# BlaineHeffron/WaveformML

Measured on AMD Instinct MI355X. Metric: waveforms/sec (LitPSD sparse-conv training step), higher is better.
Workload: dtype bf16; 1 GPU; SubMConv3d PSD net, 14x11 PMT grid x 256 samples, Cin=2 Cout=32, 256 events/rank/step, rulebook rebuilt every step; active_voxels_per_rank=84164, global_batch=256, parallelism=dp1, execution=hipgraph

## Files before the change

include/wfsparse.h:

```cpp
#ifndef WFSPARSE_H
#define WFSPARSE_H

#include <stddef.h>
#include <stdint.h>

#ifdef __cplusplus
extern "C" {
#endif

#define WFS_OK 0
#define WFS_EINVAL 1
#define WFS_EOVERFLOW 2
#define WFS_EHIP 3
#define WFS_EWORKSPACE 4

#define WFS_F32 0
#define WFS_BF16 1
#define WFS_F16 2

#define WFS_MAX_DIM 4

#define WFS_ABI_VERSION 6
int wfs_abi_version(void);
const char *wfs_last_error(void);
// ... 250 lines not shown
                   const float *momentum, const float *eps, const float *dropout_p, const int64_t *seed_dev,
                   int32_t training, float *saved, void *Y, int32_t dtype, void *stream);
int wfs_conv2d_bwd(const void *X, const void *dY, int64_t B, int32_t H, int32_t W, int32_t c0, const int32_t *channels,
                   const int32_t *fs, const int32_t *st, const int32_t *pd, const int32_t *dil, int32_t layers,
                   const void *param_ptrs, const float *dropout_p, const int64_t *seed_dev, int32_t training,
                   const float *saved, void *dX, float *workspace, int32_t dtype, void *stream);
int wfs_densify_rows(const void *rows, const int32_t *coords, int64_t n_cap, int32_t C, int64_t B, int32_t H, int32_t W,
                     const int64_t *n_valid_dev, void *out, int32_t dtype, void *stream);

#define WFS_RNN_MAX_INPUT 32
#define WFS_RNN_MAX_HIDDEN 32
#define WFS_RNN_MAX_LAYERS 8
#define WFS_RNN_MAX_T 4096
#define WFS_RNN_RELU 0
#define WFS_RNN_TANH 1
int wfs_rnn_ok(int32_t I, int32_t H, int32_t layers, int32_t dirs, int32_t nonlinearity, int32_t T, int32_t dtype);
int wfs_rnn_n_params(int32_t layers, int32_t dirs);
size_t wfs_rnn_saved_floats(int64_t N, int32_t T, int32_t I, int32_t H, int32_t layers, int32_t dirs);
size_t wfs_rnn_bwd_workspace_floats(int64_t N, int32_t T, int32_t I, int32_t H, int32_t layers, int32_t dirs);
int wfs_rnn_fwd(const void *X, int64_t N, int32_t T, int32_t I, int32_t H, int32_t layers, int32_t dirs,
                int32_t nonlinearity, const void *param_ptrs, float *saved, void *Y, void *hidden, int32_t dtype,
                float dropout_p, const int64_t *seed_dev, void *stream);
int wfs_rnn_bwd(const void *dY, int64_t N, int32_t T, int32_t I, int32_t H, int32_t layers, int32_t dirs,
                int32_t nonlinearity, const void *param_ptrs, const float *saved, void *dX, float *workspace,
                int32_t dtype, float dropout_p, const int64_t *seed_dev, void *stream);

#define WFS_VOXELIZE_MAX_SAMPLES 4096
size_t wfs_voxelize_offsets_ints(int64_t n_cap, int32_t T);
int wfs_voxelize_plan(const void *rows, const int32_t *coords, int64_t n_cap, int32_t T, const int64_t *n_dev,
                      float threshold, int32_t batch_size, int64_t V_cap, int32_t *row_offsets, int64_t *v_dev,
                      int32_t *event_offsets, int32_t *overflow_dev, int32_t dtype, void *stream);
int wfs_voxelize_emit(const void *rows, const void *values, const int32_t *coords, int64_t n_cap, int32_t T,
                      float threshold, const int32_t *row_offsets, int64_t V_cap, int32_t *indices, void *feats,
                      int32_t dtype, void *stream);
int wfs_voxelize_bwd(const void *dfeat, const int32_t *indices, const int32_t *row_offsets, int64_t n_cap, int32_t T,
                     int64_t V_cap, void *dY, int32_t dtype, void *stream);

int wfs_xent_mean_fwd_bwd(const float *logits, const int64_t *target, int64_t B, int32_t C,
                          int64_t ignore_index, float *loss, float *dlogits, void *stream);

int wfs_sgd_step(float *param, const float *grad, float *momentum_buf, int64_t n, const float *lr_dev,
                 float momentum, float dampening, float weight_decay, int32_t nesterov, int32_t first_step,
                 void *stream);

#define WFS_ADAM_COEF_FLOATS 16
int wfs_adam_step(float *param, const float *grad, float *exp_avg, float *exp_avg_sq, float *max_exp_avg_sq,
                  int64_t n, const double *hyper_dev, float *step_dev, float *coef_dev, int32_t amsgrad,
                  int32_t maximize, int32_t decoupled, void *stream);

int wfs_load_batch(const int32_t *coords, int64_t n, int32_t cols, const int32_t *perm_host, int32_t *coords_dst,
                   int32_t *indices_dst, const void *feats, void *feats_dst, int64_t feat_bytes,
                   const int64_t *labels, int64_t *labels_dst, int64_t B, int64_t *n_valid_dst,
                   int32_t *event_offsets, int32_t events, void *stream);

#define WFS_EVAL_MAX_SAMPLES 512
size_t wfs_eval_table_ints(int32_t n_bins, int32_t n_mult, int32_t n_confusion, int32_t n_se_max, int32_t nx,
                           int32_t ny, int32_t n_classes);
int wfs_event_pulse_stats(const int32_t *coords, const void *rows, int64_t n_cap, int32_t T, int32_t dtype,
                          const int64_t *n_dev, int32_t E, const double *gains, const float *seg_status, int32_t nx,
                          int32_t ny, int32_t fix_last_n_se, int32_t *offsets, double *rowstats, double *avg_coo,
                          float *summed, float *stats, int32_t *multiplicity, int32_t *n_se, float *psdl, float *psdr,
                          float *energy, float *features, int32_t *flags, void *stream);
int wfs_eval_accumulate(int32_t E, int32_t T, int32_t n_classes, const double *avg_coo, const float *summed,
                        const int32_t *multiplicity, const int32_t *n_se, const float *psdl, const float *psdr,
                        const float *energy, const int64_t *predictions, const int64_t *labels, int32_t n_bins,
                        int32_t n_mult, int32_t n_confusion, int32_t n_se_max, int32_t nx, int32_t ny, double emin,
                        double emax, double psd_min, double psd_max, int64_t *tables, double *sum_wf,
                        double *sum_labelled, int32_t *flags, void *stream);

size_t wfs_phys_table_ints(int32_t n_bins, int32_t n_mult, int32_t n_confusion, int32_t nx, int32_t ny,
                           int32_t n_classes);
size_t wfs_phys_spectra_ints(int32_t n_classes, const int32_t *spec_bins);
int wfs_phys_event_stats(const int32_t *coords, const void *rows, int64_t n_cap, int32_t dtype, const int64_t *n_dev,
                         int32_t E, int32_t *offsets, double *avg_coo, float *features, int32_t *multiplicity,
                         int32_t *flags, void *stream);
int wfs_phys_accumulate(int32_t E, int32_t n_classes, const double *avg_coo, const float *features,
                        const int32_t *multiplicity, const int64_t *predictions, const int64_t *labels, int32_t n_bins,
                        int32_t n_mult, int32_t n_confusion, int32_t nx, int32_t ny, double emin, double emax,
                        double psd_min, double psd_max, int64_t *tables, const double *spec_ranges,
                        const int32_t *spec_bins, int64_t *spectra, int32_t *flags, void *stream);

#define WFS_SEG_FIXED_ONE 4294967296.0
size_t wfs_seg_z_table_ints(int32_t nx, int32_t ny, int32_t nmult, int32_t nz, int32_t n_err, int32_t n_sample);
size_t wfs_seg_energy_table_ints(int32_t nx, int32_t ny, int32_t nmult, int32_t nE);
int wfs_seg_z_accumulate(const int32_t *coords, int64_t n_cap, const int64_t *n_dev, int32_t B, const void *pred,
                         int32_t pred_dtype, int64_t pred_bs, int64_t pred_ps, int32_t pred_plane, const void *targ,
                         int32_t targ_dtype, int64_t targ_bs, int64_t targ_ps, int32_t targ_plane, const void *energy,
                         int32_t e_dtype, int64_t e_bs, int64_t e_ps, int32_t e_plane, const float *seg_status,
                         int32_t nx, int32_t ny, const int32_t *sample_segs, int32_t n_sample, int32_t nmult,
                         int32_t nz, double zrange, int32_t n_err, double err_low, double err_high, double E_low,
                         double E_high, double E_scale, int32_t *offsets, int64_t *tables, int32_t *flags,
                         void *stream);
int wfs_seg_energy_accumulate(const int32_t *coords, int64_t n_cap, const int64_t *n_dev, int32_t B, const void *pred,
                              int32_t pred_dtype, int64_t pred_bs, int64_t pred_ps, int32_t pred_plane,
                              const void *targ, int32_t targ_dtype, int64_t targ_bs, int64_t targ_ps,
                              int32_t targ_plane, const float *seg_status, int32_t nx, int32_t ny, int32_t nmult,
                              int32_t nE, double E_low, double E_high, double E_scale, int32_t *offsets,
                              int64_t *tables, int32_t *flags, void *stream);

#define WFS_METRIC_PAIRS_MAX 16
#define WFS_PID_CLASSES 5
size_t wfs_metric_pairs_table_ints(int32_t P, const int32_t *nbins, int32_t n_classes);
int wfs_metric_pairs_accumulate(const float *params, const int32_t *result, const int32_t *category, int64_t M,
                                const int64_t *n_dev, int32_t P, const double *lo, const double *hi,
                                const int32_t *nbins, int32_t n_classes, int64_t *tables, int32_t *flags, void *stream);
int wfs_match_categories(const int64_t *predictions, const int64_t *labels, int64_t M, int32_t *result,
// ... 133 lines not shown
```

waveformml_amd/_lib.py:

```python
import ctypes
import os

import torch

_HERE = os.path.dirname(os.path.abspath(__file__))
LIB_PATH = os.environ.get("WFS_LIB") or os.path.join(_HERE, "lib", "libwfsparse.so")

WFS_OK, WFS_EINVAL, WFS_EOVERFLOW, WFS_EHIP, WFS_EWORKSPACE = 0, 1, 2, 3, 4
WFS_F32, WFS_BF16, WFS_F16 = 0, 1, 2
WFS_TENSOR_TARGET_I64 = 3
WFS_MAX_DIM = 4
WFS_RNN_RELU, WFS_RNN_TANH = 0, 1
WFS_LOSS_L1, WFS_LOSS_MSE = 0, 1
WFS_PREDICT_ROWS_PER_BLOCK = 256
WFS_PREDICT_WAVEFORM, WFS_PREDICT_PULSE = 0, 1
WFS_PREDICT_DENSE, WFS_PREDICT_EVENT, WFS_PREDICT_ROWS = 0, 1, 2
WFS_ABI_VERSION = 6
TIMER_GATHER_CONV, TIMER_GATHER_DW, TIMER_RULEBOOK, TIMER_CONV_BACKWARD = 0, 1, 2, 3

c_i32p = ctypes.POINTER(ctypes.c_int32)
c_i64p = ctypes.POINTER(ctypes.c_int64)
c_f32p = ctypes.POINTER(ctypes.c_float)
_vp, _i32, _i64, _sz = ctypes.c_void_p, ctypes.c_int32, ctypes.c_int64, ctypes.c_size_t
_dbl = ctypes.c_double


class Geometry(ctypes.Structure):
    _fields_ = [("ndim", _i32), ("batch_size", _i32), ("subm", _i32), ("K", _i32),
                ("spatial", _i32 * WFS_MAX_DIM), ("out_shape", _i32 * WFS_MAX_DIM),
                ("ksize", _i32 * WFS_MAX_DIM), ("stride", _i32 * WFS_MAX_DIM),
                ("padding", _i32 * WFS_MAX_DIM), ("dilation", _i32 * WFS_MAX_DIM),
                ("transposed", _i32), ("output_padding", _i32 * WFS_MAX_DIM)]


class DwJob(ctypes.Structure):
    _fields_ = [("part", _vp), ("nslabs", _i64), ("per", _i64), ("K", _i32), ("A", _i32), ("B", _i32),
                ("transpose", _i32), ("dW", _vp)]


SIGNATURES = {
    "wfs_abi_version": (ctypes.c_int, []),
    "wfs_last_error": (ctypes.c_char_p, []),
    "wfs_geometry_init": (ctypes.c_int, [ctypes.POINTER(Geometry)]),
    "wfs_rulebook_workspace_bytes": (_sz, [ctypes.POINTER(Geometry), _i64]),
    "wfs_rulebook_plan": (ctypes.c_int, [ctypes.POINTER(Geometry), _vp, _i64, _vp, _vp, _sz, c_i64p, _vp, _vp, _i64,
                                         _vp]),
    "wfs_rulebook_emit": (ctypes.c_int, [ctypes.POINTER(Geometry), _vp, _i64, _i64, _vp, _vp, _vp, _vp, _vp,
                                         _vp, _sz, _vp, _vp, _vp]),
    "wfs_indices_check": (ctypes.c_int, [ctypes.POINTER(Geometry), _vp, _i64, _vp, _sz, c_i64p, _vp]),
    "wfs_gather_conv": (ctypes.c_int, [_vp, c_i32p, _i32, _i32, _i64, _vp, _i64, _i32, _vp, _i32, _i32, _i32,
                                       _vp, _vp, _i32, _vp, _i32, _vp]),
    "wfs_gather_packed_ok": (ctypes.c_int, [_i32, _i32, _i32, _i32, _i32, _i32]),
    "wfs_unpack_table": (ctypes.c_int, [_vp, _i32, _i32, _i64, _vp, _vp, _vp]),
    "wfs_event_rulebook_conv_ok": (ctypes.c_int, [ctypes.POINTER(Geometry)]),
    "wfs_event_rulebook_conv_packed_kl": (ctypes.c_int, [ctypes.POINTER(Geometry)]),
    "wfs_event_rulebook_conv_state_bytes": (_sz, [_i32]),
    "wfs_event_rulebook_conv": (ctypes.c_int, [ctypes.POINTER(Geometry), _vp, _i64, _vp, _vp, _i64, _vp, _vp, _vp, _vp,
                                               _i32, _vp, _vp, _vp, _vp, _vp, _vp]),
    "wfs_wide_conv_ok": (ctypes.c_int, [_i32, _i64, _i64, _i32, _i32, _i32]),
    "wfs_wide_enable": (ctypes.c_int, [_i32]),
    "wfs_wide_conv_workspace_bytes": (_sz, [_i32, _i64, _i64, _i32, _i32, _i32, _i32]),
    "wfs_wide_filters_bytes": (_sz, [_i32, _i32, _i32, _i32]),
    "wfs_wide_filters": (ctypes.c_int, [_vp, _i32, _i32, _i32, _i32, _vp, _vp]),
    "wfs_wide_gather_conv": (ctypes.c_int, [_vp, c_i32p, _i32, _i32, _i64, _vp, _i64, _i32, _vp, _vp, _i32, _i32, _i32,
                                            _vp, _vp, _i32, _vp, _vp, _sz, _vp]),
    "wfs_wide_linear_ok": (ctypes.c_int, [_i64, _i32, _i32, _i32]),
    "wfs_wide_linear_workspace_bytes": (_sz, [_i64, _i32, _i32, _i32]),
    "wfs_wide_linear_fwd": (ctypes.c_int, [_vp, _i64, _i32, _vp, _vp, _i32, _vp, _i32, _vp, _sz, _vp]),
    "wfs_wide_linear_bwd": (ctypes.c_int, [_vp, _vp, _i64, _i32, _vp, _i32, _vp, _vp, _vp, _i32, _vp, _sz, _vp]),
    "wfs_event_offsets_ints": (_sz, [_i32]),
    "wfs_event_offsets": (ctypes.c_int, [_vp, _i64, _i32, _i32, _vp, _vp, _vp]),
    "wfs_event_rulebook_ok": (ctypes.c_int, [ctypes.POINTER(Geometry)]),
    "wfs_event_rulebook_flag_ints": (_sz, [_i32]),
    "wfs_event_rulebook_subm": (ctypes.c_int, [ctypes.POINTER(Geometry), _vp, _i64, _vp, _vp, _vp, _vp, _vp, _vp]),
    "wfs_gather_dw_workspace_bytes": (_sz, [_i32, _i64, _i32, _i32]),
    "wfs_gather_dw": (ctypes.c_int, [_vp, c_i32p, _i32, _i32, _i64, _vp, _i32, _vp, _i64, _i32, _i32, _vp, _i32, _vp,
                                     _sz, _vp, ctypes.POINTER(DwJob), _i32, _vp]),
    "wfs_conv_backward": (ctypes.c_int, [_vp, _i32, _i32, _i64, _vp, _vp, _i64, _i32, _i32, _vp, _vp, _vp, _i32, _vp, _sz,
                                         _vp, ctypes.POINTER(DwJob), _i32, _vp]),
    "wfs_dw_reduce_jobs": (ctypes.c_int, [ctypes.POINTER(DwJob), _i32, _vp]),
    "wfs_first_conv_bn_backward_workspace_bytes": (_sz, [_i32, _i64]),
    "wfs_first_conv_bn_backward": (ctypes.c_int, [_vp, c_i32p, _i32, _i32, _i64, _vp, _vp, _vp, _i64, _vp, _vp, _vp, _vp,
                                                  _i32, _vp, _vp, _vp, _i32, _vp, _sz, _vp, ctypes.POINTER(DwJob), _vp]),
    "wfs_scatter_conv": (ctypes.c_int, [_vp, _i32, _i32, _i64, _vp, _i32, _vp, _i32, _i32, _i32, _vp, _i32, _vp]),
    "wfs_maxpool_fwd": (ctypes.c_int, [_vp, c_i32p, _i32, _i64, _vp, _i64, _i32, _vp, _i32, _vp, _vp]),
    "wfs_maxpool_packed_ok": (ctypes.c_int, [_i32, _i32, _i32, _i32]),
    "wfs_maxpool_bwd": (ctypes.c_int, [_vp, _i32, _i32, _i64, _vp, _vp, _vp, _i64, _i32, _vp, _i32, _vp, _vp]),
    "wfs_bn_workspace_bytes": (_sz, [_i64, _i32]),
    "wfs_column_sum_workspace_bytes": (_sz, [_i32]),
    "wfs_column_sum": (ctypes.c_int, [_vp, _i64, _i32, _vp, _vp, _sz, _i32, _vp, _vp]),
    "wfs_bn_relu_fwd": (ctypes.c_int, [_vp, _i64, _i32, _vp, _vp, _vp, _vp, _vp, ctypes.c_float, ctypes.c_float, _i32,
# ... 18 lines not shown
    "wfs_head_bwd": (ctypes.c_int, [_vp, _vp, _i64, _i64, _vp, _i32, _vp, _vp, _vp, _i32, _vp, _sz, ctypes.POINTER(DwJob),
                                    _vp]),
    "wfs_tcn_lds_bytes": (_sz, [_i32, _i32, _i32]),
    "wfs_tcn_taps_fwd": (ctypes.c_int, [_vp, _i32, _i32, _vp, _vp, _vp]),
    "wfs_tcn_taps_bwd": (ctypes.c_int, [_vp, _i32, _i32, _vp, _i64, _vp]),
    "wfs_tcn_fwd": (ctypes.c_int, [_vp, _i64, _i32, _vp, _vp, _i32, _i32, _vp, _i32, ctypes.c_float, _vp, _vp]),
    "wfs_tcn_bwd": (ctypes.c_int, [_vp, _vp, _i64, _i32, _vp, _vp, _i32, _i32, _vp, _vp, _i32, ctypes.c_float, _vp,
                                    _vp]),
    "wfs_tcnc_ok": (ctypes.c_int, [_i32, c_i32p, _i32, _i32, _i32, _i32]),
    "wfs_tcnc_n_conv": (ctypes.c_int, [_i32, c_i32p, _i32, _i32]),
    "wfs_tcnc_weights_floats": (_sz, [_i32, c_i32p, _i32, _i32]),
    "wfs_tcnc_saved_floats": (_sz, [_i64, _i32, _i32, c_i32p, _i32]),
    "wfs_tcnc_bwd_workspace_floats": (_sz, [_i64, _i32, _i32, c_i32p, _i32, _i32]),
    "wfs_tcnc_taps_fwd": (ctypes.c_int, [_vp, _i32, c_i32p, _i32, _i32, _vp, _vp]),
    "wfs_tcnc_fwd": (ctypes.c_int, [_vp, _i64, _i32, _i32, c_i32p, _i32, _i32, _vp, _vp, _vp, _i32, ctypes.c_float, _vp,
                                    _vp]),
    "wfs_tcnc_bwd": (ctypes.c_int, [_vp, _vp, _i64, _i32, _i32, c_i32p, _i32, _i32, _vp, _vp, _vp, _vp, _vp, _i32,
                                    ctypes.c_float, _vp, _vp]),
    "wfs_conv1d_ok": (ctypes.c_int, [_i32, c_i32p, c_i32p, c_i32p, c_i32p, _i32, _i32, _i32]),
    "wfs_conv1d_saved_floats": (_sz, [_i64, _i32, _i32, c_i32p, c_i32p, c_i32p, c_i32p, _i32]),
    "wfs_conv1d_bwd_workspace_floats": (_sz, [_i64, _i32, _i32, c_i32p, c_i32p, c_i32p, c_i32p, _i32]),
    "wfs_conv1d_fwd": (ctypes.c_int, [_vp, _i64, _i32, _i32, c_i32p, c_i32p, c_i32p, c_i32p, _i32, _vp, c_f32p, c_f32p,
                                      _i32, _vp, _vp, _i32, _vp, _vp]),
    "wfs_conv1d_bwd": (ctypes.c_int, [_vp, _vp, _i64, _i32, _i32, c_i32p, c_i32p, c_i32p, c_i32p, _i32, _vp, _i32, _vp,
                                      _vp, _vp, _i32, _vp, _vp]),
    "wfs_conv2d_ok": (ctypes.c_int, [_i32, c_i32p, c_i32p, c_i32p, c_i32p, c_i32p, _i32, _i64, _i32, _i32, _i32, _i32]),
    "wfs_conv2d_saved_floats": (_sz, [_i64, _i32, _i32, _i32, c_i32p, c_i32p, c_i32p, c_i32p, c_i32p, _i32, _i32]),
    "wfs_conv2d_bwd_workspace_floats": (_sz, [_i64, _i32, _i32, _i32, c_i32p, c_i32p, c_i32p, c_i32p, c_i32p, _i32,
                                              _i32]),
    "wfs_conv2d_fwd": (ctypes.c_int, [_vp, _i64, _i32, _i32, _i32, c_i32p, c_i32p, c_i32p, c_i32p, c_i32p, _i32, _vp,
                                      c_f32p, c_f32p, c_f32p, _vp, _i32, _vp, _vp, _i32, _vp]),
    "wfs_conv2d_bwd": (ctypes.c_int, [_vp, _vp, _i64, _i32, _i32, _i32, c_i32p, c_i32p, c_i32p, c_i32p, c_i32p, _i32, _vp,
                                      c_f32p, _vp, _i32, _vp, _vp, _vp, _i32, _vp]),
    "wfs_densify_rows": (ctypes.c_int, [_vp, _vp, _i64, _i32, _i64, _i32, _i32, _vp, _vp, _i32, _vp]),
    "wfs_rnn_ok": (ctypes.c_int, [_i32, _i32, _i32, _i32, _i32, _i32, _i32]),
    "wfs_rnn_n_params": (ctypes.c_int, [_i32, _i32]),
    "wfs_rnn_saved_floats": (_sz, [_i64, _i32, _i32, _i32, _i32, _i32]),
    "wfs_rnn_bwd_workspace_floats": (_sz, [_i64, _i32, _i32, _i32, _i32, _i32]),
    "wfs_rnn_fwd": (ctypes.c_int, [_vp, _i64, _i32, _i32, _i32, _i32, _i32, _i32, _vp, _vp, _vp, _vp, _i32, ctypes.c_float,
                                   _vp, _vp]),
    "wfs_rnn_bwd": (ctypes.c_int, [_vp, _i64, _i32, _i32, _i32, _i32, _i32, _i32, _vp, _vp, _vp, _vp, _i32, ctypes.c_float,
                                   _vp, _vp]),
    "wfs_voxelize_offsets_ints": (_sz, [_i64, _i32]),
    "wfs_voxelize_plan": (ctypes.c_int, [_vp, _vp, _i64, _i32, _vp, ctypes.c_float, _i32, _i64, _vp, _vp, _vp, _vp, _i32,
                                         _vp]),
    "wfs_voxelize_emit": (ctypes.c_int, [_vp, _vp, _vp, _i64, _i32, ctypes.c_float, _vp, _i64, _vp, _vp, _i32, _vp]),
    "wfs_voxelize_bwd": (ctypes.c_int, [_vp, _vp, _vp, _i64, _i32, _i64, _vp, _i32, _vp]),
    "wfs_xent_mean_fwd_bwd": (ctypes.c_int, [_vp, _vp, _i64, _i32, _i64, _vp, _vp, _vp]),
    "wfs_sgd_step": (ctypes.c_int, [_vp, _vp, _vp, _i64, _vp, ctypes.c_float, ctypes.c_float, ctypes.c_float, _i32, _i32,
                                    _vp]),
    "wfs_adam_step": (ctypes.c_int, [_vp, _vp, _vp, _vp, _vp, _i64, _vp, _vp, _vp, _i32, _i32, _i32, _vp]),
    "wfs_load_batch": (ctypes.c_int, [_vp, _i64, _i32, c_i32p, _vp, _vp, _vp, _vp, _i64, _vp, _vp, _i64, _vp, _vp, _i32,
                                      _vp]),
    "wfs_eval_table_ints": (_sz, [_i32, _i32, _i32, _i32, _i32, _i32, _i32]),
    "wfs_event_pulse_stats": (ctypes.c_int, [_vp, _vp, _i64, _i32, _i32, _vp, _i32, _vp, _vp, _i32, _i32, _i32, _vp, _vp,
                                             _vp, _vp, _vp, _vp, _vp, _vp, _vp, _vp, _vp, _vp, _vp]),
    "wfs_eval_accumulate": (ctypes.c_int, [_i32, _i32, _i32, _vp, _vp, _vp, _vp, _vp, _vp, _vp, _vp, _vp, _i32, _i32,
                                           _i32, _i32, _i32, _i32, ctypes.c_double, ctypes.c_double, ctypes.c_double,
                                           ctypes.c_double, _vp, _vp, _vp, _vp, _vp]),
    "wfs_phys_table_ints": (_sz, [_i32, _i32, _i32, _i32, _i32, _i32]),
    "wfs_phys_spectra_ints": (_sz, [_i32, c_i32p]),
    "wfs_phys_event_stats": (ctypes.c_int, [_vp, _vp, _i64, _i32, _vp, _i32, _vp, _vp, _vp, _vp, _vp, _vp]),
    "wfs_phys_accumulate": (ctypes.c_int, [_i32, _i32, _vp, _vp, _vp, _vp, _vp, _i32, _i32, _i32, _i32, _i32, _dbl, _dbl,
                                           _dbl, _dbl, _vp, ctypes.POINTER(_dbl), c_i32p, _vp, _vp, _vp]),
    "wfs_seg_z_table_ints": (_sz, [_i32, _i32, _i32, _i32, _i32, _i32]),
    "wfs_seg_energy_table_ints": (_sz, [_i32, _i32, _i32, _i32]),
    "wfs_seg_z_accumulate": (ctypes.c_int, [_vp, _i64, _vp, _i32] + [_vp, _i32, _i64, _i64, _i32] * 3 +
                             [_vp, _i32, _i32, _vp, _i32, _i32, _i32, _dbl, _i32, _dbl, _dbl, _dbl, _dbl, _dbl, _vp, _vp,
                              _vp, _vp]),
    "wfs_seg_energy_accumulate": (ctypes.c_int, [_vp, _i64, _vp, _i32] + [_vp, _i32, _i64, _i64, _i32] * 2 +
                                  [_vp, _i32, _i32, _i32, _i32, _dbl, _dbl, _dbl, _vp, _vp, _vp, _vp]),
    "wfs_metric_pairs_table_ints": (_sz, [_i32, c_i32p, _i32]),
    "wfs_metric_pairs_accumulate": (ctypes.c_int, [_vp, _vp, _vp, _i64, _vp, _i32, ctypes.POINTER(_dbl),
                                                   ctypes.POINTER(_dbl), c_i32p, _i32, _vp, _vp, _vp]),
    "wfs_match_categories": (ctypes.c_int, [_vp, _vp, _i64, _vp, _vp, _vp]),
    "wfs_pid_table_ints": (_sz, [_i32, _i32]),
    "wfs_pid_row_stats": (ctypes.c_int, [_vp, _vp, _vp, _vp, _i32, _i32, _i64, _vp, _i32, _vp, _i32, _i32, _i32, _i32,
                                         _i32, _i32, _i32, _dbl] + [_vp] * 10),
    "wfs_metric_pairs_real_table_ints": (_sz, [_i32, c_i32p, _i32]),
    "wfs_metric_pairs_accumulate_real": (ctypes.c_int, [_vp, _vp, _vp, _i64, _vp, _i32, ctypes.POINTER(_dbl),
                                                        ctypes.POINTER(_dbl), c_i32p, _i32, _vp, _vp, _vp]),
    "wfs_tensor_rows": (ctypes.c_int, [_vp, _i32, _i32, _vp, _i32, _i32, _vp, _i64, _vp, _i32, _i32, _vp, _vp, _vp, _vp,
                                       _vp]),
    "wfs_masked_regression_loss_workspace_bytes": (_sz, [_i64]),
    "wfs_masked_regression_loss": (ctypes.c_int, [_vp, _i32, _vp, _i32, _i32, _i32, _vp, _vp, _i32, _i32, _i64, _vp, _i32,
                                                  _i32, _vp, _sz, _vp, _vp, _vp]),
    "wfs_masked_regression_loss_backward": (ctypes.c_int, [_vp, _i32, _vp, _i32, _i32, _i32, _vp, _vp, _i32, _i32, _i64,
                                                           _vp, _i32, _vp, _vp, _vp, _vp]),
    "wfs_error_edges": (ctypes.c_int, [_dbl, _i32, ctypes.POINTER(_dbl)]),
    "wfs_segq_row_stats": (ctypes.c_int, [_vp, _vp, _i32, _vp, _i32, _i32, _vp, _i32, _i64, _vp, _i32, _vp, _i32, _i32,
                                          _i32, _i32, _i32, _i32] + [_vp] * 11),
    "wfs_segq_error_accumulate": (ctypes.c_int, [_vp, _i32, _vp, _i32, _i32, _i32, _vp, _vp, _i64, _vp, _i32, _i32, _i32]
                                  + [_vp] * 7),
    "wfs_align_pulses": (ctypes.c_int, [_vp, _i32, _i64, _vp, _i32, _i32, _vp, _vp, _vp]),
    "wfs_zreal_row_stats": (ctypes.c_int, [_vp, _vp, _i32, _i64, _i64, _i32, _vp, _i32, _i64, _i64, _i32, _i32, _i32, _vp,
                                           _i32, _i64, _vp, _i32, _vp, _i32, _i32, _i32, _dbl] + [_vp] * 12),
    "wfs_zreal_baseline": (ctypes.c_int, [_vp, _i64, _vp, _i32, _vp, _vp, _vp, _i32, _i32, _vp, _vp]),
    "wfs_zreal_table_ints": (_sz, [_i32, _i32, _i32, _i32, _i32]),
    "wfs_zreal_accumulate": (ctypes.c_int, [_vp, _i64, _vp, _i32, _vp, _vp, _vp, _vp, _vp, _vp, _i32, _i32, _i32, _i32,
                                            _dbl, _dbl, _dbl, _i32, _vp, _vp, _vp]),
    "wfs_seg_z_accumulate_cal": (ctypes.c_int, [_vp, _i64, _vp, _i32] + [_vp, _i32, _i64, _i64, _i32] * 3 +
                                 [_vp, _vp, _i32, _vp, _vp, _i32, _i32, _vp, _i32, _i32, _i32, _dbl, _i32, _dbl, _dbl, _dbl, _dbl,
                                  _dbl, _vp, _vp, _vp, _vp]),
    "wfs_seg_energy_cal_table_ints": (_sz, [_i32, _i32, _i32, _i32, _i32]),
    "wfs_seg_energy_accumulate_cal": (ctypes.c_int, [_vp, _i64, _vp, _i32] + [_vp, _i32, _i64, _i64, _i32] * 2 +
                                      [_vp, _vp, _vp, _i32, _i32, _i32, _i32, _i32, _dbl, _dbl, _dbl, _dbl, _vp, _vp, _vp,
# ... 107 lines not shown
```

waveformml_amd/csrc/conv_mfma.hip:

```cpp
#include <stdlib.h>

#include "wfs_common.h"

namespace {

typedef float f32x16 __attribute__((ext_vector_type(16)));
typedef float f32x4 __attribute__((ext_vector_type(4)));
constexpr int F32_GROUP = 4;

struct KMap {
    int v[128];
};


__device__ __forceinline__ int packed_entry(int e, int o) { return (e >= 0 && (e & 7) == o) ? (e >> 3) : -1; }
__device__ __forceinline__ void table_row_of(int pk, int k, int *trow, int *osel) {
    const int kq = pk ? k / pk : k;
    *trow = kq;
    *osel = pk ? k - kq * pk : -1;
}
__device__ __forceinline__ int table_value(int e, int osel) { return osel < 0 ? e : packed_entry(e, osel); }

typedef __bf16 bf16x8e __attribute__((ext_vector_type(8)));
typedef float f32x2 __attribute__((ext_vector_type(2)));
// ... 286 lines not shown
                                                       const float *__restrict__ X, const float *__restrict__ W,
                                                       const float *__restrict__ bias, float *__restrict__ Y) {
    extern __shared__ __attribute__((aligned(16))) float sW_dyn[];
    __shared__ int sNext;
    gconv16_f32_body<TRANSPOSE_W, PK, true>(sW_dyn, &sNext, (int)blockIdx.x, (int)gridDim.x, (int)blockDim.x, table, mirror,
                                            K, identity_k, R, r_dev, X, W, bias, Y);
}

template <bool TRANSPOSE_W, int PK = 0>
__global__ void __launch_bounds__(1024) k_gconv16_f32(const int *__restrict__ table, int mirror, int K, int identity_k,
                                                      long long R, const long long *__restrict__ r_dev,
                                                      const float *__restrict__ X, const float *__restrict__ W,
                                                      const float *__restrict__ bias, float *__restrict__ Y) {
    extern __shared__ __attribute__((aligned(16))) float sW_dyn[];
    __shared__ int sNext;
    gconv16_f32_body<TRANSPOSE_W, PK>(sW_dyn, &sNext, (int)blockIdx.x, (int)gridDim.x, (int)blockDim.x, table, mirror, K,
                                      identity_k, R, r_dev, X, W, bias, Y);
}

typedef short s16x8 __attribute__((ext_vector_type(8)));
typedef __bf16 bf16x8 __attribute__((ext_vector_type(8)));
constexpr int BF_GROUP = 6;

typedef _Float16 f16x8 __attribute__((ext_vector_type(8)));

template <typename H, typename V>
__device__ __forceinline__ f32x16 mfma16(V a, V b, f32x16 acc) {
    static_assert(sizeof(V) == 16, "8 x 16-bit operands");
    if constexpr (sizeof(H) == 2 && __is_same(H, wfs_f16))
        return __builtin_amdgcn_mfma_f32_32x32x16_f16(__builtin_bit_cast(f16x8, a), __builtin_bit_cast(f16x8, b), acc, 0,
                                                      0, 0);
    else
        return __builtin_amdgcn_mfma_f32_32x32x16_bf16(__builtin_bit_cast(bf16x8, a), __builtin_bit_cast(bf16x8, b), acc,
                                                       0, 0, 0);
}

__device__ __forceinline__ uint4 keep_if(uint4 v, bool ok) {
    v.x = ok ? v.x : 0u;
    v.y = ok ? v.y : 0u;
    v.z = ok ? v.z : 0u;
    v.w = ok ? v.w : 0u;
    return v;
}

#ifndef WFS_KNOCK
#define WFS_KNOCK 0
#endif
template <typename H, bool TRANSPOSE_W, int PK = 0>
__device__ __forceinline__ void gconv32_bf16_body(unsigned char *smem, int vbid, int vgrid, int nthreads,
                                                  const int *__restrict__ table, int mirror, int K, int identity_k,
                                                  long long R, const long long *__restrict__ r_dev,
                                                  const H *__restrict__ X, const float *__restrict__ W,
                                                  const float *__restrict__ bias, H *__restrict__ Y, long long ntiles,
                                                  long long tiles_per_xcd) {
    uint4 *sWb = reinterpret_cast<uint4 *>(smem);
    int *sNb = reinterpret_cast<int *>(smem + (size_t)K * 2048);
    constexpr int WSB = 5;
    const int nfrag = K * 128;
    if (!(WFS_KNOCK & 1))
    for (int u0 = threadIdx.x; u0 < nfrag; u0 += nthreads * WSB) {
        float w[WSB][8];
#pragma unroll
        for (int b = 0; b < WSB; ++b) {
            int u = u0 + b * nthreads;
            u = u < nfrag ? u : nfrag - 1;
            int k = u >> 7, s = (u >> 6) & 1, h = (u >> 5) & 1, col = u & 31;
            int c0 = 16 * h + 8 * s;
            if (!TRANSPOSE_W) {
#pragma unroll
                for (int j = 0; j < 8; ++j) w[b][j] = W[((long long)k * 32 + c0 + j) * 32 + col];
            } else {
                const f32x4 *src = (const f32x4 *)(W + ((long long)k * 32 + col) * 32 + c0);
                f32x4 lo = src[0], hi = src[1];
                w[b][0] = lo.x; w[b][1] = lo.y; w[b][2] = lo.z; w[b][3] = lo.w;
                w[b][4] = hi.x; w[b][5] = hi.y; w[b][6] = hi.z; w[b][7] = hi.w;
            }
        }
#pragma unroll
        for (int b = 0; b < WSB; ++b) {
            int u = u0 + b * nthreads;
            uint4 v;
            v.x = wfs_pack2<H>(w[b][0], w[b][1]);
            v.y = wfs_pack2<H>(w[b][2], w[b][3]);
            v.z = wfs_pack2<H>(w[b][4], w[b][5]);
            v.w = wfs_pack2<H>(w[b][6], w[b][7]);
            if (u < nfrag) sWb[u] = v;
        }
    }
    __syncthreads();

    const int lane = threadIdx.x & 63, wid = threadIdx.x >> 6, nw = nthreads >> 6;
    const int r = lane & 31, h = lane >> 5;
    int *myNb = sNb + (size_t)wid * K * 32;
    const int xcd = vbid & 7, bi = vbid >> 3, bpx = vgrid >> 3;
    const long long Rv = wfs_valid_rows(R, r_dev);
    const long long nt_v = (Rv + 31) >> 5, tpx_v = (nt_v + 7) >> 3;
    (void)ntiles;
    (void)tiles_per_xcd;
    const long long t_begin = (long long)xcd * tpx_v;
    const long long t_end = t_begin + tpx_v < nt_v ? t_begin + tpx_v : nt_v;
    const float bj = bias ? bias[r] : 0.f;
    const __amdgpu_buffer_rsrc_t rsrcX = __builtin_amdgcn_make_buffer_rsrc((void *)X, 0, 0x7FFFFFFF, 0x00020000);
    for (long long tile = t_begin + (long long)wid * bpx + bi; tile < t_end; tile += (long long)bpx * nw) {
        if (tile * 32 >= Rv) break;
        const long long row = tile * 32 + r;
        const bool live = row < Rv;
        const long long rowc = live ? row : 0;
        int v[32];
        if constexpr (PK == 0) {
#pragma unroll
            for (int k = 0; k < 32; ++k) {
                int kk = k < K ? k : K - 1;
// ... 29 lines not shown
            int nbs[BF_GROUP];
#pragma unroll
            for (int g = 0; g < BF_GROUP; ++g) {
                ks[g] = mask ? __builtin_ctz(mask) : -1;
                mask = mask ? (mask & (mask - 1)) : 0u;
            }
#pragma unroll
            for (int g = 0; g < BF_GROUP; ++g)
                if (ks[g] >= 0) {
                    nbs[g] = myNb[ks[g] * 32 + r];
                    const int src = (WFS_KNOCK & 16) ? (int)rowc : nbs[g];
                    int voff = src >= 0 ? (int)((unsigned)src * 64u + (unsigned)h * 32u) : (int)0x80000000;
                    asm volatile("" : "+v"(voff));
                    if ((WFS_KNOCK & 32) && (ks[g] % 3) != 1) {
                        a_lo[g] = uint4{0x3f803f80u, 0x3f803f80u, 0x3f803f80u, 0x3f803f80u};
                        a_hi[g] = a_lo[g];
                    } else {
                        a_lo[g] = __builtin_bit_cast(uint4, __builtin_amdgcn_raw_buffer_load_b128(rsrcX, voff, 0, 0));
                        a_hi[g] = __builtin_bit_cast(uint4, __builtin_amdgcn_raw_buffer_load_b128(rsrcX, voff + 16, 0, 0));
                    }
                }
#pragma unroll
            for (int g = 0; g < BF_GROUP; ++g)
                if (ks[g] >= 0) {
                    const uint4 lo = a_lo[g], hi = a_hi[g];
                    const uint4 *bp = sWb + (size_t)ks[g] * 128 + h * 32 + r;
                    uint4 b0 = bp[0], b1 = bp[64];
                    acc = mfma16<H>(lo, b0, acc);
                    acc = mfma16<H>(hi, b1, acc);
                }
        }
        unsigned *Yw = reinterpret_cast<unsigned *>(Y);
#pragma unroll
        for (int i = 0; i < 16; i += 2) {
            float mine0 = acc[i], mine1 = acc[i + 1];
            float send = (lane & 1) ? mine0 : mine1;
            float got = __shfl_xor(send, 1, 64);
            unsigned packed = (lane & 1) ? wfs_pack2<H>(got, mine1) : wfs_pack2<H>(mine0, got);
            int ri = (lane & 1) ? i + 1 : i;
            long long orow = tile * 32 + (ri & 3) + 8 * (ri >> 2) + 4 * h;
            if (!(WFS_KNOCK & 8) || packed == 0x12345678u)
                if (orow < Rv) Yw[orow * 16 + (r >> 1)] = packed;
        }
    }
}

template <typename H, bool TRANSPOSE_W, int PK = 0>
__global__ void __launch_bounds__(1024) k_gconv32_bf16(const int *__restrict__ table, int mirror, int K,
                                                       int identity_k,
                                                       long long R, const long long *__restrict__ r_dev,
                                                       const H *__restrict__ X,
                                                       const float *__restrict__ W, const float *__restrict__ bias,
                                                       H *__restrict__ Y, long long ntiles,
                                                       long long tiles_per_xcd) {
    extern __shared__ __attribute__((aligned(16))) unsigned char smem[];
    gconv32_bf16_body<H, TRANSPOSE_W, PK>(smem, (int)blockIdx.x, (int)gridDim.x, (int)blockDim.x, table, mirror, K,
                                          identity_k, R, r_dev, X, W, bias, Y, ntiles, tiles_per_xcd);
}

template <typename T>
__global__ void __launch_bounds__(256) k_gconv_c2c32(const int *__restrict__ table, KMap kmap, int K, int identity_k,
                                                     long long R, const long long *__restrict__ r_dev,
                                                     const T *__restrict__ X,
                                                     const float *__restrict__ W, const float *__restrict__ bias,
                                                     T *__restrict__ Y) {
    __shared__ __attribute__((aligned(16))) float sW[128 * 64];
    for (int e = threadIdx.x; e < K * 64; e += 256) sW[e] = W[e];
    __syncthreads();
    const int rsub = threadIdx.x >> 3, cq = threadIdx.x & 7;
    f32x4 bv = {0.f, 0.f, 0.f, 0.f};
    if (bias) bv = *(const f32x4 *)(bias + cq * 4);
    const long long Rv = wfs_valid_rows(R, r_dev);
    for (long long row = (long long)blockIdx.x * 32 + rsub; row < Rv; row += (long long)gridDim.x * 32) {
        f32x4 acc = bv;
        for (int k = 0; k < K; ++k) {
            int nb = (k == identity_k) ? (int)row : table[(long long)kmap.v[k] * R + row];
            if (nb < 0) continue;
            float x0 = wfs_ld(X + (long long)nb * 2), x1 = wfs_ld(X + (long long)nb * 2 + 1);
            f32x4 w0 = *(const f32x4 *)(sW + k * 64 + cq * 4);
            f32x4 w1 = *(const f32x4 *)(sW + k * 64 + 32 + cq * 4);
            acc.x = fmaf(x0, w0.x, acc.x);
            acc.y = fmaf(x0, w0.y, acc.y);
            acc.z = fmaf(x0, w0.z, acc.z);
            acc.w = fmaf(x0, w0.w, acc.w);
            acc.x = fmaf(x1, w1.x, acc.x);
            acc.y = fmaf(x1, w1.y, acc.y);
            acc.z = fmaf(x1, w1.z, acc.z);
            acc.w = fmaf(x1, w1.w, acc.w);
        }
        T *y = Y + row * 32 + cq * 4;
        if constexpr (sizeof(T) == 4) {
            *reinterpret_cast<f32x4 *>(y) = acc;
        } else {
            uint2 pk;
            pk.x = wfs_pack2<T>(acc.x, acc.y);
            pk.y = wfs_pack2<T>(acc.z, acc.w);
            *reinterpret_cast<uint2 *>(y) = pk;
        }
    }
}

constexpr int DW_KG = 4;
constexpr int DW_WAVES = 8;

constexpr int DW_LDS = DW_WAVES * 1024 * 4;
template <typename T>
__device__ __forceinline__ void gdw32_body(float *sRed, int bx, int by, int nbx, const int *__restrict__ table, int pk, int K,
                                           int identity_k, long long Rcap, const long long *__restrict__ r_dev,
                                           const T *__restrict__ S, const T *__restrict__ G, float *__restrict__ part,
                                           int ngroups) {
// ... 459 lines not shown
#pragma unroll
    for (int q = 0; q < DWS_KG; ++q) {
        __syncthreads();
#pragma unroll
        for (int i = 0; i < 16; ++i) {
            int arow = (i & 3) + 8 * (i >> 2) + 4 * h;
            sRed[wid * 1024 + arow * 32 + c] = acc[q][i];
        }
        __syncthreads();
        const int k = g + q * ngroups;
        for (int e = threadIdx.x; e < 1024; e += DWS_WAVES * 64) {
            float v = 0.f;
#pragma unroll
            for (int w = 0; w < DWS_WAVES; ++w) v += sRed[w * 1024 + e];
            if (k < K) part[((long long)bx * K + k) * 1024 + e] = v;
        }
    }
}

__global__ void __launch_bounds__(DWS_WAVES * 64) k_gdw32_split(const int *__restrict__ table, int pk, int K, int identity_k,
                                                               long long Rcap, const long long *__restrict__ r_dev,
                                                               const float *__restrict__ S, const float *__restrict__ G,
                                                               float *__restrict__ part, int ngroups) {
    extern __shared__ __attribute__((aligned(16))) unsigned char smem[];
    gdw32_split_body(smem, (int)blockIdx.x, (int)blockIdx.y, (int)gridDim.x, table, pk, K, identity_k, Rcap, r_dev, S, G, part,
                     ngroups);
}

template <int PK>
__global__ void __launch_bounds__(DWS_WAVES * 64) k_bwd32_split(const int *__restrict__ table, int K, int identity_k,
                                                               long long Rcap, const long long *__restrict__ r_dev,
                                                               const float *__restrict__ S, const float *__restrict__ G,
                                                               const float *__restrict__ W, float *__restrict__ dX,
                                                               float *__restrict__ part, int ngroups, int nbx_dw,
                                                               int n_dw_pad, int n_dx, int dx_threads) {
    extern __shared__ __attribute__((aligned(16))) unsigned char smem[];
    __shared__ int sNext;
    const int bid = (int)blockIdx.x;
    if (bid < n_dw_pad) {
        if (bid >= nbx_dw * ngroups) return;
        gdw32_split_body(smem, bid % nbx_dw, bid / nbx_dw, nbx_dw, table, PK, K, identity_k, Rcap, r_dev, S, G, part, ngroups);
    } else {
        if ((int)threadIdx.x >= dx_threads) return;
        gconv16_f32_body<true, PK, true>(reinterpret_cast<float *>(smem), &sNext, bid - n_dw_pad, n_dx, dx_threads, table, 0,
                                         K, identity_k, Rcap, r_dev, G, W, nullptr, dX);
    }
}

template <typename H, int PK>
__global__ void __launch_bounds__(1024) k_bwd32_bf16(const int *__restrict__ table, int K, int identity_k, long long Rcap,
                                                     const long long *__restrict__ r_dev, const H *__restrict__ S,
                                                     const H *__restrict__ G, const float *__restrict__ W,
                                                     H *__restrict__ dX, float *__restrict__ part, int ngroups,
                                                     int nbx_dw, int n_dw_pad, int n_dx, int dx_threads) {
    extern __shared__ __attribute__((aligned(16))) unsigned char smem[];
    const int bid = (int)blockIdx.x;
    if (bid < n_dw_pad) {
        if (bid >= nbx_dw * ngroups) return;
        gdw32_bf16_body<H>(smem, bid % nbx_dw, bid / nbx_dw, nbx_dw, table, PK, K, identity_k, Rcap, r_dev, S, G, part,
                           ngroups);
    } else {
        if ((int)threadIdx.x >= dx_threads) return;
        gconv32_bf16_body<H, true, PK>(smem, bid - n_dw_pad, n_dx, dx_threads, table, 0, K, identity_k, Rcap, r_dev, G, W,
                                       nullptr, dX, 0, 0);
    }
}


constexpr int C2_WAVES = 8;

__device__ __forceinline__ void c2_fetch(const int *__restrict__ table, int mirror, int K, long long Rcap, long long trow,
                                         int h, int (&nb)[14]) {
#pragma unroll
    for (int t = 0; t < 14; ++t) {
        int k = 2 * t + h;
        int kk = k < K ? k : K - 1;
        nb[t] = table[(long long)(mirror ? K - 1 - kk : kk) * Rcap + trow];
    }
}

__device__ __forceinline__ void c2_resolve(int K, int identity_k, long long trow, bool tlive, int h, int (&nb)[14]) {
#pragma unroll
    for (int t = 0; t < 14; ++t) {
        int k = 2 * t + h;
        int n = (k == identity_k) ? (int)trow : nb[t];
        nb[t] = (tlive && k < K && n >= 0) ? n : -1;
    }
}

__device__ __forceinline__ void c2_fill_a(unsigned *myA, int c, int h, const int (&nb)[14], const unsigned (&xv)[14]) {
#pragma unroll
    for (int t = 0; t < 14; ++t) {
        int k = 2 * t + h;
        myA[c * 33 + k] = nb[t] >= 0 ? xv[t] : 0u;
    }
    if (h == 0) {
#pragma unroll
        for (int k = 28; k < 32; ++k) myA[c * 33 + k] = 0u;
    }
}

template <typename H>
__device__ __forceinline__ void c2_product(const unsigned *myA, const unsigned short *myB, int c, int h, f32x16 &acc0,
                                           f32x16 &acc1) {
    const unsigned short *A16 = reinterpret_cast<const unsigned short *>(myA);
    unsigned wa[2][2][4], wb[2][4];
#pragma unroll
    for (int st = 0; st < 2; ++st)
#pragma unroll
        for (int m = 0; m < 4; ++m) {
            int r0 = 16 * st + 8 * h + 2 * m;
            wa[0][st][m] = (unsigned)A16[r0 * 66 + c] | ((unsigned)A16[(r0 + 1) * 66 + c] << 16);
            wa[1][st][m] = (unsigned)A16[r0 * 66 + 32 + c] | ((unsigned)A16[(r0 + 1) * 66 + 32 + c] << 16);
            wb[st][m] = (unsigned)myB[r0 * 32 + c] | ((unsigned)myB[(r0 + 1) * 32 + c] << 16);
        }
#pragma unroll
    for (int st = 0; st < 2; ++st) {
// ... 401 lines not shown
    nb = (nb + 7) / 8 * 8;
    *wpb = w;
    *nblk = nb;
    *tiles_per_xcd = (*ntiles + 7) / 8;
}

int wfs_launch_gconv32_f32(const int *table, int mirror, int K, int identity_k, long long R, const long long *r_dev,
                           const float *X, const float *W, int transpose_w, const float *bias, float *Y,
                           hipStream_t stream, int packed_kl) {
    const size_t lds = (size_t)K * 4096;
    WFS_REQUIRE(packed_kl == 0 || (packed_kl == 3 && transpose_w && !mirror && identity_k < 0), WFS_EINVAL,
                "packed tables: kl = 3, dX products only");
    static bool attr16[2] = {false, false};
    const long long nt16 = (R + 15) >> 4;
    const long long expect = r_dev ? (nt16 * 7 + 7) / 8 : nt16;
    int w = (int)((expect + 255) / 256);
    w = w < 4 ? 4 : (w > 16 ? 16 : (w + 3) / 4 * 4);
    long long nb = (expect + w - 1) / w;
    nb = nb > 256 ? 256 : (nb + 7) / 8 * 8;
    if (nb < 8) nb = 8;
    if (wfs_split_bf16() && K <= 27) {
        int ws = w > 12 ? 12 : w;
        long long nbs = (expect + ws - 1) / ws;
        nbs = nbs > 256 ? 256 : (nbs + 7) / 8 * 8;
        if (nbs < 8) nbs = 8;
        const dim3 gs((unsigned)nbs), bs(ws * 64);
        const size_t lds_s = (size_t)(K - 1) * 6144;
        static bool attrs[3] = {false, false, false};
        if (packed_kl)
            return launch_big_lds(k_gconv16_split<true, 3>, &attrs[2], gs, bs, lds_s, stream, table, mirror, K, identity_k, R,
                                  r_dev, X, W, bias, Y);
        if (transpose_w)
            return launch_big_lds(k_gconv16_split<true>, &attrs[0], gs, bs, lds_s, stream, table, mirror, K, identity_k, R,
                                  r_dev, X, W, bias, Y);
        return launch_big_lds(k_gconv16_split<false>, &attrs[1], gs, bs, lds_s, stream, table, mirror, K, identity_k, R, r_dev,
                              X, W, bias, Y);
    }
    const dim3 g16((unsigned)nb), b16(w * 64);
    if (packed_kl) {
        static bool attr16p = false;
        return launch_big_lds(k_gconv16_f32<true, 3>, &attr16p, g16, b16, lds, stream, table, mirror, K, identity_k, R,
                              r_dev, X, W, bias, Y);
    }
    if (transpose_w)
        return launch_big_lds(k_gconv16_f32<true>, &attr16[0], g16, b16, lds, stream, table, mirror, K, identity_k, R,
                              r_dev, X, W, bias, Y);
    return launch_big_lds(k_gconv16_f32<false>, &attr16[1], g16, b16, lds, stream, table, mirror, K, identity_k, R,
                          r_dev, X, W, bias, Y);
}

template <typename H>
static int launch_gconv32_h16(const int *table, int mirror, int K, int identity_k, long long R, const long long *r_dev,
                              const H *Xb, const float *W, int transpose_w, const float *bias, H *Yb,
                              hipStream_t stream, int packed_kl) {
    long long ntiles, nblk, tiles_per_xcd;
    int wpb;
    gconv32_grid(R, r_dev != nullptr, &ntiles, &wpb, &nblk, &tiles_per_xcd, 16);
    const size_t lds = (size_t)K * 2048 + (size_t)wpb * K * 32 * sizeof(int);
    static bool attr[2] = {false, false};
    const dim3 grid((unsigned)nblk), block(wpb * 64);
    WFS_REQUIRE(packed_kl == 0 || (packed_kl == 3 && transpose_w && !mirror && identity_k < 0), WFS_EINVAL,
                "packed tables: kl = 3, dX products only");
    if (packed_kl) {
        static bool attr_p = false;
        return launch_big_lds(k_gconv32_bf16<H, true, 3>, &attr_p, grid, block, lds, stream, table, mirror, K, identity_k, R,
                              r_dev, Xb, W, bias, Yb, ntiles, tiles_per_xcd);
    }
    if (transpose_w)
        return launch_big_lds(k_gconv32_bf16<H, true>, &attr[0], grid, block, lds, stream, table, mirror, K, identity_k, R,
                              r_dev, Xb, W, bias, Yb, ntiles, tiles_per_xcd);
    return launch_big_lds(k_gconv32_bf16<H, false>, &attr[1], grid, block, lds, stream, table, mirror, K, identity_k, R,
                          r_dev, Xb, W, bias, Yb, ntiles, tiles_per_xcd);
}

int wfs_launch_gconv32_h16(const int *table, int mirror, int K, int identity_k, long long R, const long long *r_dev,
                           const void *X, const float *W, int transpose_w, const float *bias, void *Y, int dtype,
                           hipStream_t stream, int packed_kl) {
    if (dtype == WFS_F16)
        return launch_gconv32_h16<wfs_f16>(table, mirror, K, identity_k, R, r_dev, (const wfs_f16 *)X, W, transpose_w,
                                           bias, (wfs_f16 *)Y, stream, packed_kl);
    return launch_gconv32_h16<wfs_bf16>(table, mirror, K, identity_k, R, r_dev, (const wfs_bf16 *)X, W, transpose_w, bias,
                                        (wfs_bf16 *)Y, stream, packed_kl);
}

int wfs_launch_gconv_c2c32(const int *table, const int *kmap, int K, int identity_k, long long R,
                           const long long *r_dev, const void *X, const float *W, const float *bias, void *Y, int dtype,
                           hipStream_t stream) {
    KMap km;
    for (int k = 0; k < K; ++k) km.v[k] = kmap ? kmap[k] : k;
    const int kind = wfs_kmap_kind(kmap, K);
    const int mir = kind == WFS_KMAP_MIRROR;
    if (dtype != WFS_F32 && K <= 32 && kind != WFS_KMAP_OTHER) {
        long long nb = ((R + 31) / 32 + 3) / 4;
        if (nb > 4096) nb = 4096;
        const dim3 grid((unsigned)nb), block(256);
        if (dtype == WFS_F16)
            k_gconv_c2c32_bf16<wfs_f16><<<grid, block, 0, stream>>>(table, mir, K, identity_k, R, r_dev, (const wfs_f16 *)X, W,
                                                                    bias, (wfs_f16 *)Y);
        else
            k_gconv_c2c32_bf16<wfs_bf16><<<grid, block, 0, stream>>>(table, mir, K, identity_k, R, r_dev, (const wfs_bf16 *)X,
                                                                     W, bias, (wfs_bf16 *)Y);
        WFS_LAUNCH_CHECK();
        return WFS_OK;
    }
    if (dtype == WFS_F32 && K <= 27 && kind != WFS_KMAP_OTHER) {
        long long nb = ((R + 31) / 32 + 3) / 4;
        if (nb > 4096) nb = 4096;
        k_gconv_c2c32_f32<<<dim3((unsigned)nb), dim3(256), 0, stream>>>(table, mir, K, identity_k, R, r_dev, (const float *)X,
                                                                        W, bias, (float *)Y);
        WFS_LAUNCH_CHECK();
        return WFS_OK;
    }
    long long nblk = (R + 31) / 32;
    if (nblk > 8192) nblk = 8192;
    return wfs_with_dtype(dtype, [&](auto t) -> int {
        using T = decltype(t);
        k_gconv_c2c32<T><<<dim3((unsigned)nblk), dim3(256), 0, stream>>>(table, km, K, identity_k, R, r_dev, (const T *)X, W,
                                                                        bias, (T *)Y);
        WFS_LAUNCH_CHECK();
        return WFS_OK;
    });
}

static long long dw32_blocks(long long R, bool two_per_cu = false) {
    long long ntiles = (R + 31) >> 5;
    long long nblk = (ntiles + (two_per_cu ? 19 : 39)) / (two_per_cu ? 20 : 40);
    if (nblk < 1) nblk = 1;
    const long long cap = two_per_cu ? 72 : 36;
    if (nblk > cap) nblk = cap;
    return nblk;
}
static long long c2_slabs(long long R) {
    const long long ntiles = (R + 31) >> 5;
    const long long slabs = (ntiles + C2_WAVES - 1) / C2_WAVES;
    return slabs > 512 ? 512 : (slabs < 1 ? 1 : slabs);
// ... 3 lines not shown
    if (Cs == 32 && Cg == 32) return (size_t)dw32_blocks(R, true) * K * 1024 * sizeof(float);
    if (Cs == 32 && Cg == 2) {
        const long long bound = (R + 127) / 128;
        return (size_t)(bound > 512 ? 512 : (bound < 1 ? 1 : bound)) * K * 64 * sizeof(float);
    }
    return 0;
}

static int dw_reduce_or_defer(float *part, long long nslabs, long long per, int K, int A, int B, int transpose, float *dW,
                              wfs_dw_job *defer, hipStream_t stream) {
    if (defer) {
        *defer = wfs_dw_job{part, nslabs, per, K, A, B, transpose, dW};
        return WFS_OK;
    }
    k_slab_reduce<<<dim3((unsigned)((per + 31) / 32)), dim3(nslabs > 64 ? 1024 : 256), 0, stream>>>(part, nslabs, per, K, A, B,
                                                                                                  transpose, dW);
    WFS_LAUNCH_CHECK();
    return WFS_OK;
}

int wfs_launch_gdw32(const int *table, int K, int identity_k, long long R, const long long *r_dev, const void *S,
                     const void *G, int swap, float *dW, float *part, int dtype, wfs_dw_job *defer, hipStream_t stream,
                     int packed_kl) {
    WFS_REQUIRE(packed_kl == 0 || (packed_kl >= 1 && packed_kl <= 8 && K % packed_kl == 0 && identity_k < 0), WFS_EINVAL,
                "packed tables: K must be a multiple of kl <= 8, no identity offset");
    const long long nblk = dw32_blocks(R, dtype == WFS_F32 && !wfs_split_bf16());
    const long long ntiles = (R + 31) >> 5;
    const long long tiles_per_block = (ntiles + nblk - 1) / nblk;
    const int ngroups = (K + DW_KG - 1) / DW_KG;
    const dim3 grid((unsigned)nblk, (unsigned)ngroups);
    if (dtype == WFS_F32 && wfs_split_bf16()) {
        static bool attr = false;
        const int rc = launch_big_lds(k_gdw32_split, &attr, grid, dim3(DWS_WAVES * 64), DWS_LDS, stream, table, packed_kl, K, identity_k, R,
                                      r_dev, (const float *)S, (const float *)G, part, ngroups);
        if (rc != WFS_OK) return rc;
    } else if (dtype == WFS_F32) {
        k_gdw32<float><<<grid, dim3(512), 0, stream>>>(table, packed_kl, K, identity_k, R, r_dev, (const float *)S,
                                                       (const float *)G, part, ngroups, tiles_per_block);
        WFS_LAUNCH_CHECK();
    } else {
        const int rc = wfs_with_h16(dtype, [&](auto t) -> int {
            using H = decltype(t);
            static bool attr = false;
            return launch_big_lds(k_gdw32_bf16<H>, &attr, grid, dim3(1024), DWB_LDS, stream, table, packed_kl, K, identity_k,
                                  R, r_dev, (const H *)S, (const H *)G, part, ngroups, tiles_per_block);
        });
        if (rc != WFS_OK) return rc;
    }
    return dw_reduce_or_defer(part, nblk, (long long)K * 1024, K, 32, 32, swap, dW, defer, stream);
}

template <typename H>
static int launch_bwd32_h16(const int *table, int packed_kl, int K, int identity_k, long long R, const long long *r_dev,
                            const H *S, const H *G, const float *W, H *dX, float *part, hipStream_t stream) {
    const long long nbx_dw = dw32_blocks(R, false);
    const int ngroups = (K + DWB_KG - 1) / DWB_KG;
    const long long n_dw = nbx_dw * ngroups, n_dw_pad = (n_dw + 7) / 8 * 8;
    long long ntiles, n_dx, tiles_per_xcd;
    int wpb;
    gconv32_grid(R, r_dev != nullptr, &ntiles, &wpb, &n_dx, &tiles_per_xcd, 16);
    size_t lds = (size_t)K * 2048 + (size_t)wpb * K * 32 * sizeof(int);
    if (lds < (size_t)DWB_LDS) lds = DWB_LDS;
    const dim3 grid((unsigned)(n_dw_pad + n_dx)), block(1024);
    if (packed_kl) {
        static bool attr = false;
        return launch_big_lds(k_bwd32_bf16<H, 3>, &attr, grid, block, lds, stream, table, K, identity_k, R, r_dev, S, G, W, dX,
                              part, ngroups, (int)nbx_dw, (int)n_dw_pad, (int)n_dx, wpb * 64);
    }
    static bool attr0 = false;
    return launch_big_lds(k_bwd32_bf16<H, 0>, &attr0, grid, block, lds, stream, table, K, identity_k, R, r_dev, S, G, W, dX,
                          part, ngroups, (int)nbx_dw, (int)n_dw_pad, (int)n_dx, wpb * 64);
}

bool wfs_bwd32_fused_ok(int K, int packed_kl, int dtype) {
    const bool row_type = dtype == WFS_BF16 || dtype == WFS_F16 || (dtype == WFS_F32 && wfs_split_bf16());
    return row_type && K >= 1 && K <= 27 && (packed_kl == 0 || (packed_kl == 3 && K % 3 == 0));
}

static void gconv16_split_grid(long long R, bool padded, int *waves, long long *nblk) {
    const long long nt16 = (R + 15) >> 4;
    const long long expect = padded ? (nt16 * 7 + 7) / 8 : nt16;
    int w = (int)((expect + 255) / 256);
    w = w < 4 ? 4 : (w > 12 ? 12 : (w + 3) / 4 * 4);
    long long nb = (expect + w - 1) / w;
    nb = nb > 256 ? 256 : (nb + 7) / 8 * 8;
    if (nb < 8) nb = 8;
    *waves = w;
    *nblk = nb;
}

static int launch_bwd32_split(const int *table, int packed_kl, int K, int identity_k, long long R, const long long *r_dev,
                              const float *S, const float *G, const float *W, float *dX, float *part, hipStream_t stream) {
    const long long nbx_dw = dw32_blocks(R, false);
    const int ngroups = (K + DWS_KG - 1) / DWS_KG;
    const long long n_dw = nbx_dw * ngroups, n_dw_pad = (n_dw + 7) / 8 * 8;
    int ws;
    long long n_dx;
    gconv16_split_grid(R, r_dev != nullptr, &ws, &n_dx);
    size_t lds = (size_t)(K - 1) * 6144;
    if (lds < (size_t)DWS_LDS) lds = DWS_LDS;
    const dim3 grid((unsigned)(n_dw_pad + n_dx)), block(DWS_WAVES * 64);
    if (packed_kl) {
        static bool attr = false;
        return launch_big_lds(k_bwd32_split<3>, &attr, grid, block, lds, stream, table, K, identity_k, R, r_dev, S, G, W, dX,
                              part, ngroups, (int)nbx_dw, (int)n_dw_pad, (int)n_dx, ws * 64);
    }
    static bool attr0 = false;
    return launch_big_lds(k_bwd32_split<0>, &attr0, grid, block, lds, stream, table, K, identity_k, R, r_dev, S, G, W, dX,
                          part, ngroups, (int)nbx_dw, (int)n_dw_pad, (int)n_dx, ws * 64);
}

int wfs_launch_bwd32_h16(const int *table, int packed_kl, int K, int identity_k, long long R, const long long *r_dev,
                         const void *S, const void *G, const float *W, void *dX, int swap, float *dW, float *part, int dtype,
                         wfs_dw_job *defer, hipStream_t stream) {
    int rc;
    if (dtype == WFS_F32)
        rc = launch_bwd32_split(table, packed_kl, K, identity_k, R, r_dev, (const float *)S, (const float *)G, W, (float *)dX,
                                part, stream);
    else if (dtype == WFS_F16)
        rc = launch_bwd32_h16<wfs_f16>(table, packed_kl, K, identity_k, R, r_dev, (const wfs_f16 *)S, (const wfs_f16 *)G, W,
                                       (wfs_f16 *)dX, part, stream);
    else
        rc = launch_bwd32_h16<wfs_bf16>(table, packed_kl, K, identity_k, R, r_dev, (const wfs_bf16 *)S, (const wfs_bf16 *)G,
                                        W, (wfs_bf16 *)dX, part, stream);
    if (rc != WFS_OK) return rc;
    return dw_reduce_or_defer(part, dw32_blocks(R, false), (long long)K * 1024, K, 32, 32, swap, dW, defer, stream);
}

int wfs_launch_gdw_c32c2(const int *table, int mirror, int K, int identity_k, long long R, const long long *r_dev,
                         const void *S, const void *G, int swap, float *dW, float *part, int dtype,
                         wfs_dw_job *defer, hipStream_t stream) {
    const long long slabs = c2_slabs(R);
    if (dtype == WFS_F32)
        k_gdw_c32c2_f32<<<dim3((unsigned)slabs), dim3(512), 0, stream>>>(table, mirror, K, identity_k, R, r_dev,
                                                                         (const float *)S, (const float *)G, part);
    else
        wfs_with_h16(dtype, [&](auto t) -> int {
            using H = decltype(t);
            k_gdw_c32c2_bf16<H><<<dim3((unsigned)slabs), dim3(512), 0, stream>>>(table, mirror, K, identity_k, R, r_dev,
                                                                                (const H *)S, (const H *)G, part);
            return WFS_OK;
        });
    WFS_LAUNCH_CHECK();
    return dw_reduce_or_defer(part, slabs, (long long)K * 64, K, 2, 32, swap ? 0 : 1, dW, defer, stream);
}

long long wfs_first_bn_slabs(long long R) { return c2_slabs(R); }

int wfs_launch_first_bn_bwd(const int *table, int mirror, int K, int identity_k, long long R, const long long *r_dev,
                            const void *Z, const void *dY, const void *X, const float *gamma, const float *beta,
                            const float *mean, const float *invstd, int relu, const float *partial, int nblk, float *dW,
                            float *dgamma, float *dbeta, float *part, int dtype, wfs_dw_job *defer, hipStream_t stream) {
    const long long slabs = c2_slabs(R);
    const int rc = wfs_with_h16(dtype, [&](auto t) -> int {
        using H = decltype(t);
        k_gdw_bnapply_c32c2<H><<<dim3((unsigned)slabs), dim3(512), 0, stream>>>(
            table, mirror, K, identity_k, R, r_dev, (const H *)Z, (const H *)dY, (const H *)X, partial, nblk, mean, invstd,
            gamma, beta, relu, dgamma, dbeta, part);
        WFS_LAUNCH_CHECK();
        return WFS_OK;
    });
    if (rc != WFS_OK) return rc;
    return dw_reduce_or_defer(part, slabs, (long long)K * 64, K, 2, 32, 0, dW, defer, stream);
}
```

waveformml_amd/csrc/gather_conv.hip:

```cpp
#include "wfs_common.h"

namespace {

constexpr int TB = 256;
constexpr int CT = 8;

struct KMap {
    int v[128];
};


template <typename T, bool TRANSPOSE_W>
__global__ void __launch_bounds__(TB) k_gather_conv(const int *__restrict__ table, KMap kmap, int K, int identity_k,
                                                    long long R, const long long *__restrict__ r_dev,
                                                    const T *__restrict__ X, int Cx,
                                                    const float *__restrict__ W, int Cw_in, int Cw_out,
                                                    const float *__restrict__ bias, T *__restrict__ Y, int Cy) {
    const int lane = threadIdx.x & 63;
    const int wid = __builtin_amdgcn_readfirstlane(threadIdx.x >> 6);
    const long long r = (long long)blockIdx.x * 64 + lane;
    const int c0 = blockIdx.y * (4 * CT) + wid * CT;
    if (c0 >= Cy) return;
    const bool live = r < wfs_valid_rows(R, r_dev);
    float acc[CT];
// ... 273 lines not shown
            const int nb = h ? n1 : n0;
            const long long rr = base + 2 * s + h;
            const float a = wfs_ld(S + (nb >= 0 ? rr : r_begin) * Cs + ac);
            const float b = wfs_ld(G + (long long)(nb >= 0 ? nb : 0) * Cg + bc);
            A[s] = (nb >= 0 && a_ok) ? a : 0.f;
            B[s] = (nb >= 0 && b_ok) ? b : 0.f;
        }
    };
    if (r_begin < r_end) fetch(r_begin, av, bv);
    for (long long base = r_begin; base < r_end; base += 64) {
        const bool more = base + 64 < r_end;
        if (more) fetch(base + 64, an, bn);
#pragma unroll
        for (int s = 0; s < 32; ++s) acc = __builtin_amdgcn_mfma_f32_32x32x2f32(av[s], bv[s], acc, 0, 0, 0);
        if (more) {
#pragma unroll
            for (int s = 0; s < 32; ++s) {
                av[s] = an[s];
                bv[s] = bn[s];
            }
        }
    }
    float *p = part + ((long long)chunk * K + k) * Cs * Cg;
#pragma unroll
    for (int i = 0; i < 16; ++i) {
        const int a = a0 + (i & 3) + 8 * (i >> 2) + 4 * h;
        if (a < Cs && b_ok) p[(long long)a * Cg + b0 + j] = acc[i];
    }
}

inline bool gm_shape(int Ca, int Cb) { return Ca >= 8 && Cb >= 8 && (long long)Ca * Cb >= 256; }

long long dw_chunks(long long R) {
    long long chunks = wfs_cdiv(R, 4096);
    if (chunks < 1) chunks = 1;
    if (chunks > 512) chunks = 512;
    return chunks;
}
long long dw_chunks_mfma(long long R, int K, int Cs, int Cg) {
    long long chunks = wfs_cdiv(R, 256);
    const long long per = (long long)K * Cs * Cg * 4;
    const long long cap = per > 0 ? (32ll << 20) / per : 1;
    if (chunks > 64) chunks = 64;
    if (chunks > cap) chunks = cap;
    const long long base = dw_chunks(R);
    return chunks < base ? base : chunks;
}

}

static int gather_conv_impl(const int32_t *table, const int32_t *kmap_host, int32_t K, int32_t identity_k,
                            int64_t R, const void *X, int64_t X_rows, int32_t Cx, const float *W, int32_t Cw_in,
                            int32_t Cw_out, int32_t transpose_w, const float *bias, void *Y, int32_t dtype,
                            const int64_t *r_dev_, void *stream_, int packed_kl = 0) {
    hipStream_t stream = (hipStream_t)stream_;
    WFS_REQUIRE(packed_kl == 0 || wfs_gather_packed_ok(packed_kl, K, Cx, transpose_w ? Cw_in : Cw_out, dtype, transpose_w ? 1 : 2),
                WFS_EINVAL, "a packed table (kl %d) is not taken by this product (wfs_gather_packed_ok): expand it with "
                "wfs_unpack_table", packed_kl);
    const long long *r_dev = (const long long *)r_dev_;
    (void)X_rows;
    WFS_REQUIRE(K >= 1 && K <= 128, WFS_EINVAL, "kernel volume %d not in [1,128]", K);
    WFS_REQUIRE(wfs_dtype_ok(dtype), WFS_EINVAL, "bad dtype %d", dtype);
    const int Cy = transpose_w ? Cw_in : Cw_out;
    WFS_REQUIRE(Cx == (transpose_w ? Cw_out : Cw_in), WFS_EINVAL, "channel mismatch: X has %d, filter wants %d", Cx,
                transpose_w ? Cw_out : Cw_in);
    if (R == 0) return WFS_OK;
    WFS_REQUIRE((table || (K == 1 && identity_k == 0)) && X && W && Y, WFS_EINVAL, "NULL device pointer");
    KMap km;
    for (int k = 0; k < K; ++k) {
        km.v[k] = kmap_host ? kmap_host[k] : k;
        WFS_REQUIRE(km.v[k] >= 0 && km.v[k] < K, WFS_EINVAL, "kmap[%d] out of range", k);
    }
    WfsTimerScope timer(WFS_TIMER_GATHER_CONV, stream);
    const int kind = wfs_kmap_kind(kmap_host, K);
    const int mirror = kind == WFS_KMAP_MIRROR;
    if (dtype == WFS_F32 && Cx == 32 && Cy == 32 && wfs_mfma_gconv32_ok(K) && table && kind != WFS_KMAP_OTHER &&
        X_rows < (1ll << 24)) {
        return wfs_launch_gconv32_f32(table, mirror, K, identity_k, R, r_dev, (const float *)X, W, transpose_w, bias,
                                      (float *)Y, stream, packed_kl);
    }
    if (dtype != WFS_F32 && Cx == 32 && Cy == 32 && K <= 27 && table && kind != WFS_KMAP_OTHER && X_rows < (1ll << 25)) {
        return wfs_launch_gconv32_h16(table, mirror, K, identity_k, R, r_dev, X, W, transpose_w, bias, Y, dtype, stream,
                                      packed_kl);
    }
    WFS_REQUIRE(packed_kl == 0, WFS_EINVAL, "a packed table reached a kernel that reads dense ones");
    if (Cx == 2 && Cy == 32 && !transpose_w && table)
        return wfs_launch_gconv_c2c32(table, kmap_host, K, identity_k, R, r_dev, X, W, bias, Y, dtype, stream);
    if (gm_shape(Cx, Cy) && table) {
        const dim3 g((unsigned)wfs_cdiv(R, 32), (unsigned)wfs_cdiv(Cy, 32)), b(64 * GM_WAVES);
        return wfs_with_dtype(dtype, [&](auto t) -> int {
            using T = decltype(t);
            if (transpose_w)
                k_gconv_mfma<T, true><<<g, b, 0, stream>>>(table, km, K, identity_k, R, r_dev, (const T *)X, Cx, W, Cw_in,
                                                           Cw_out, bias, (T *)Y, Cy);
            else
                k_gconv_mfma<T, false><<<g, b, 0, stream>>>(table, km, K, identity_k, R, r_dev, (const T *)X, Cx, W, Cw_in,
                                                            Cw_out, bias, (T *)Y, Cy);
            WFS_LAUNCH_CHECK();
            return WFS_OK;
        });
    }
    dim3 grid((unsigned)wfs_cdiv(R, 64), (unsigned)wfs_cdiv(Cy, 4 * CT)), block(TB);
    return wfs_with_dtype(dtype, [&](auto t) -> int {
        using T = decltype(t);
        if (transpose_w)
            k_gather_conv<T, true><<<grid, block, 0, stream>>>(table, km, K, identity_k, R, r_dev, (const T *)X, Cx, W, Cw_in,
                                                               Cw_out, bias, (T *)Y, Cy);
        else
            k_gather_conv<T, false><<<grid, block, 0, stream>>>(table, km, K, identity_k, R, r_dev, (const T *)X, Cx, W, Cw_in,
                                                                Cw_out, bias, (T *)Y, Cy);
        WFS_LAUNCH_CHECK();
        return WFS_OK;
    });
}

extern "C" int wfs_gather_conv(const int32_t *table, const int32_t *kmap_host, int32_t K, int32_t identity_k,
                               int64_t R, const void *X, int64_t X_rows, int32_t Cx, const float *W, int32_t Cw_in,
                               int32_t Cw_out, int32_t transpose_w, const float *bias, void *Y, int32_t dtype,
                               const int64_t *r_dev, int32_t packed_kl, void *stream) {
    WFS_REQUIRE(packed_kl == 0 || !kmap_host, WFS_EINVAL, "a packed table takes no column map");
    return gather_conv_impl(table, kmap_host, K, identity_k, R, X, X_rows, Cx, W, Cw_in, Cw_out, transpose_w, bias, Y,
                            dtype, r_dev, stream, packed_kl);
}

extern "C" int wfs_gather_packed_ok(int32_t packed_kl, int32_t K, int32_t Ca, int32_t Cb, int32_t dtype, int32_t which) {
    if (packed_kl < 1 || packed_kl > 8 || K < 1 || K > 32 || K % packed_kl != 0 || Ca != 32 || Cb != 32 || !wfs_dtype_ok(dtype))
        return 0;
    if (which == 3) return 1;
    return which == 1 && packed_kl == 3 && K <= 27;
}

extern "C" int wfs_scatter_conv(const int32_t *table, int32_t K, int32_t identity_k, int64_t R, const void *X,
                                int32_t Cx, const float *W, int32_t Cw_in, int32_t Cw_out, int32_t transpose_w,
                                float *Y_accum, int32_t dtype, void *stream_) {
    hipStream_t stream = (hipStream_t)stream_;
    WFS_REQUIRE(K >= 1, WFS_EINVAL, "bad K");
    WFS_REQUIRE(wfs_dtype_ok(dtype), WFS_EINVAL, "bad dtype %d", dtype);
    const int Cy = transpose_w ? Cw_in : Cw_out;
    WFS_REQUIRE(Cx == (transpose_w ? Cw_out : Cw_in), WFS_EINVAL, "channel mismatch");
    if (R == 0) return WFS_OK;
    WFS_REQUIRE(table && X && W && Y_accum, WFS_EINVAL, "NULL device pointer");
    dim3 grid((unsigned)wfs_cdiv(R, 64), (unsigned)wfs_cdiv(Cy, 4 * CT)), block(TB);
    return wfs_with_dtype(dtype, [&](auto t) -> int {
        using T = decltype(t);
        if (transpose_w)
            k_scatter_conv<T, true><<<grid, block, 0, stream>>>(table, K, identity_k, R, (const T *)X, Cx, W, Cw_in, Cw_out,
                                                                Y_accum, Cy);
        else
            k_scatter_conv<T, false><<<grid, block, 0, stream>>>(table, K, identity_k, R, (const T *)X, Cx, W, Cw_in, Cw_out,
                                                                 Y_accum, Cy);
        WFS_LAUNCH_CHECK();
        return WFS_OK;
    });
}

extern "C" size_t wfs_gather_dw_workspace_bytes(int32_t K, int64_t R, int32_t Cs, int32_t Cg) {
    size_t generic = (size_t)(gm_shape(Cs, Cg) ? dw_chunks_mfma(R, K, Cs, Cg) : dw_chunks(R)) * K * Cs * Cg * sizeof(float);
    size_t fast = wfs_dw_fast_workspace(K, R, Cs, Cg);
    if (wfs_wide_dw_ok(K, R, Cs, Cg, WFS_F32)) {
        size_t wide = wfs_wide_dw_workspace(K, R, Cs, Cg, WFS_F32);
        generic = generic > wide ? generic : wide;
    }
    return generic > fast ? generic : fast;
}

static int gather_dw_impl(const int32_t *table, const int32_t *kmap_host, int32_t K, int32_t identity_k, int64_t R,
                          const void *S, int32_t Cs, const void *G, int64_t G_rows, int32_t Cg, int32_t swap, float *dW,
                          int32_t dtype, void *workspace, size_t workspace_bytes, const int64_t *r_dev_,
                          wfs_dw_job *defer, void *stream_, int packed_kl = 0) {
    hipStream_t stream = (hipStream_t)stream_;
    WFS_REQUIRE(packed_kl == 0 || (wfs_gather_packed_ok(packed_kl, K, Cs, Cg, dtype, 3) && !kmap_host), WFS_EINVAL,
                "a packed table (kl %d) is not taken by this product (wfs_gather_packed_ok): expand it with wfs_unpack_table",
                packed_kl);
    const long long *r_dev = (const long long *)r_dev_;
    WFS_REQUIRE(K >= 1 && K <= 65535, WFS_EINVAL, "bad K");
// ... 16 lines not shown
    }
    const bool rows_fit = dtype != WFS_F32 || (R < (1ll << 24) && G_rows < (1ll << 24));
    if (Cs == 32 && Cg == 32 && table && !kmap_host && rows_fit)
        return wfs_launch_gdw32(table, K, identity_k, R, r_dev, S, G, swap, dW, (float *)workspace, dtype, defer, stream,
                                packed_kl);
    WFS_REQUIRE(packed_kl == 0, WFS_EINVAL, "a packed table reached a kernel that reads dense ones");
    const int kind = wfs_kmap_kind(kmap_host, K);
    if (Cs == 32 && Cg == 2 && K <= 27 && table && kind != WFS_KMAP_OTHER)
        return wfs_launch_gdw_c32c2(table, kind == WFS_KMAP_MIRROR, K, identity_k, R, r_dev, S, G, swap, dW,
                                    (float *)workspace, dtype, defer, stream);
    WFS_REQUIRE(kind == WFS_KMAP_IDENTITY, WFS_EINVAL, "a column map is only supported by the 32 x 2 dW kernel");
    long long chunks = gm_shape(Cs, Cg) ? dw_chunks_mfma(R, K, Cs, Cg) : dw_chunks(R);
    long long rows_per_chunk = wfs_cdiv(wfs_cdiv(R, chunks), DW_ROWS) * DW_ROWS;
    int tiles_a = (int)wfs_cdiv(Cs, DW_TA), tiles_b = (int)wfs_cdiv(Cg, DW_TBB);
    WFS_REQUIRE((long long)tiles_a * tiles_b <= 65535, WFS_EINVAL, "channel tile grid too large");
    dim3 grid((unsigned)chunks, (unsigned)K, (unsigned)(tiles_a * tiles_b)), block(TB);
    float *part = (float *)workspace;
    int rc;
    if (gm_shape(Cs, Cg) && table)
        rc = wfs_with_dtype(dtype, [&](auto t) -> int {
            using T = decltype(t);
            k_gdw_mfma<T><<<grid, dim3(64), 0, stream>>>(table, K, identity_k, R, r_dev, rows_per_chunk, (const T *)S, Cs,
                                                         (const T *)G, Cg, part, tiles_b);
            WFS_LAUNCH_CHECK();
            return WFS_OK;
        });
    else
        rc = wfs_with_dtype(dtype, [&](auto t) -> int {
            using T = decltype(t);
            k_gather_dw<T><<<grid, block, 0, stream>>>(table, K, identity_k, R, r_dev, rows_per_chunk, (const T *)S, Cs,
                                                       (const T *)G, Cg, part, tiles_a, tiles_b);
            WFS_LAUNCH_CHECK();
            return WFS_OK;
        });
    if (rc != WFS_OK) return rc;
    long long per = (long long)K * Cs * Cg;
    k_dw_reduce<<<dim3((unsigned)wfs_cdiv(per, TB)), block, 0, stream>>>(part, chunks, K, Cs, Cg, swap, dW);
    WFS_LAUNCH_CHECK();
    return WFS_OK;
}

extern "C" int wfs_gather_dw(const int32_t *table, const int32_t *kmap_host, int32_t K, int32_t identity_k, int64_t R,
                             const void *S, int32_t Cs, const void *G, int64_t G_rows, int32_t Cg, int32_t swap, float *dW,
                             int32_t dtype, void *workspace, size_t workspace_bytes, const int64_t *r_dev,
                             wfs_dw_job *defer, int32_t packed_kl, void *stream) {
    return gather_dw_impl(table, kmap_host, K, identity_k, R, S, Cs, G, G_rows, Cg, swap, dW, dtype, workspace,
                          workspace_bytes, r_dev, defer, stream, packed_kl);
}

extern "C" int wfs_conv_backward(const int32_t *table, int32_t K, int32_t identity_k, int64_t R, const void *X,
                                 const void *dY, int64_t dY_rows, int32_t Cin, int32_t Cout, const float *W, void *dX,
                                 float *dW, int32_t dtype, void *workspace, size_t workspace_bytes, const int64_t *r_dev,
                                 wfs_dw_job *defer, int32_t packed_kl, void *stream_) {
    hipStream_t stream = (hipStream_t)stream_;
    WFS_REQUIRE(dX && dW, WFS_EINVAL, "wfs_conv_backward computes both gradients (use wfs_gather_conv / wfs_gather_dw for one)");
    const long long row_lim = dtype == WFS_F32 ? (1ll << 24) : (1ll << 25);
    const bool fused = Cin == 32 && Cout == 32 && table && wfs_bwd32_fused_ok(K, packed_kl, dtype) && R > 0 &&
                       R < row_lim && dY_rows < row_lim && (packed_kl == 0 || identity_k < 0);
    if (!fused) {
        int rc = gather_dw_impl(table, nullptr, K, identity_k, R, X, Cin, dY, dY_rows, Cout, 0, dW, dtype, workspace,
                                workspace_bytes, r_dev, defer, stream_, packed_kl);
        if (rc != WFS_OK) return rc;
        return gather_conv_impl(table, nullptr, K, identity_k, R, dY, dY_rows, Cout, W, Cin, Cout, 1, nullptr, dX, dtype, r_dev,
                                stream_, packed_kl);
    }
    WFS_REQUIRE(X && dY && W && workspace, WFS_EINVAL, "NULL device pointer");
    const size_t need = wfs_gather_dw_workspace_bytes(K, R, Cin, Cout);
    WFS_REQUIRE(workspace_bytes >= need, WFS_EWORKSPACE, "workspace %zu < %zu", workspace_bytes, need);
    if (defer) *defer = wfs_dw_job_none();
    WfsTimerScope timer(WFS_TIMER_CONV_BACKWARD, stream);
    return wfs_launch_bwd32_h16(table, packed_kl, K, identity_k, R, (const long long *)r_dev, X, dY, W, dX, 0, dW,
                                (float *)workspace, dtype, defer, stream);
}

static size_t first_bn_slab_bytes(int32_t K, int64_t R) {
    return wfs_align_up((size_t)wfs_first_bn_slabs(R) * (size_t)K * 64 * sizeof(float), 256);
}
extern "C" size_t wfs_first_conv_bn_backward_workspace_bytes(int32_t K, int64_t R) {
    return first_bn_slab_bytes(K, R) + wfs_bn_workspace_bytes(R, 32);
}

extern "C" int wfs_first_conv_bn_backward(const int32_t *table, const int32_t *kmap_host, int32_t K, int32_t identity_k,
                                          int64_t R, const void *Z, const void *dY, const void *X, int64_t X_rows,
                                          const float *gamma, const float *beta, const float *save_mean,
                                          const float *save_invstd, int32_t relu, float *dW, float *dgamma, float *dbeta,
                                          int32_t dtype, void *workspace, size_t workspace_bytes, const int64_t *r_dev,
                                          wfs_dw_job *defer, void *stream_) {
    hipStream_t stream = (hipStream_t)stream_;
    WFS_REQUIRE(K >= 1 && K <= 27, WFS_EINVAL, "K = %d (1 .. 27)", K);
    WFS_REQUIRE(dtype == WFS_BF16 || dtype == WFS_F16, WFS_EINVAL, "16-bit rows only (dtype %d)", dtype);
    WFS_REQUIRE(dW, WFS_EINVAL, "NULL dW");
    WFS_REQUIRE(R >= 0 && R < (1ll << 31) && X_rows < (1ll << 31), WFS_EINVAL, "too many rows");
    if (defer) *defer = wfs_dw_job_none();
    if (R == 0) {
        WFS_HIP_CHECK(hipMemsetAsync(dW, 0, (size_t)K * 64 * sizeof(float), stream));
        if (dgamma) WFS_HIP_CHECK(hipMemsetAsync(dgamma, 0, 32 * sizeof(float), stream));
        if (dbeta) WFS_HIP_CHECK(hipMemsetAsync(dbeta, 0, 32 * sizeof(float), stream));
        return WFS_OK;
    }
    WFS_REQUIRE(table && Z && dY && X && save_mean && save_invstd && workspace, WFS_EINVAL, "NULL device pointer");
    WFS_REQUIRE(((uintptr_t)workspace & 15) == 0, WFS_EINVAL, "the workspace must be 16-byte aligned");
    WFS_REQUIRE(workspace_bytes >= wfs_first_conv_bn_backward_workspace_bytes(K, R), WFS_EWORKSPACE, "workspace too small");
    const int kind = wfs_kmap_kind(kmap_host, K);
    WFS_REQUIRE(kind != WFS_KMAP_OTHER, WFS_EINVAL, "the column map must be the identity or the SubM mirror");
    float *part = (float *)workspace;
    float *partial = (float *)((char *)workspace + first_bn_slab_bytes(K, R));
    int nblk = 0;
    int rc = wfs_launch_bn_bwd_reduce(Z, dY, R, 32, gamma, beta, save_mean, save_invstd, relu ? 1 : 0, partial, dtype,
                                      (const long long *)r_dev, stream, &nblk);
    if (rc != WFS_OK) return rc;
    WfsTimerScope timer(WFS_TIMER_GATHER_DW, stream);
    return wfs_launch_first_bn_bwd(table, kind == WFS_KMAP_MIRROR, K, identity_k, R, (const long long *)r_dev, Z, dY, X, gamma,
                                   beta, save_mean, save_invstd, relu ? 1 : 0, partial, nblk, dW, dgamma, dbeta, part, dtype,
                                   defer, stream);
}

extern "C" int wfs_dw_reduce_jobs(const wfs_dw_job *jobs, int32_t n, void *stream) {
    WFS_REQUIRE(n >= 0 && n <= 16 && (n == 0 || jobs), WFS_EINVAL, "%d jobs (0 .. 16)", n);
    wfs_dw_job live[16];
    int m = 0;
    for (int i = 0; i < n; ++i) {
        if (jobs[i].nslabs <= 0) continue;
        WFS_REQUIRE(jobs[i].part && jobs[i].dW && jobs[i].per > 0 && jobs[i].A > 0 && jobs[i].B > 0, WFS_EINVAL,
                    "job %d is incomplete", i);
        live[m++] = jobs[i];
// ... 64 lines not shown
```

waveformml_amd/csrc/optim.hip:

```cpp
#include "wfs_common.h"

namespace {

__global__ void __launch_bounds__(256) k_sgd_step(float *__restrict__ P, const float *__restrict__ G,
                                                  float *__restrict__ M, long long n, const float *__restrict__ lr_dev,
                                                  float momentum, float dampening, float weight_decay, int nesterov,
                                                  int first_step) {
    const float lr = *lr_dev;
    for (long long i = (long long)blockIdx.x * 256 + threadIdx.x; i < n; i += (long long)gridDim.x * 256) {
        float p = P[i];
        float g = G[i];
        if (weight_decay != 0.f) g = fmaf(weight_decay, p, g);
        if (M) {
            float b = first_step ? g : fmaf(1.f - dampening, g, M[i] * momentum);
            M[i] = b;
            g = nesterov ? fmaf(momentum, b, g) : b;
        }
        P[i] = fmaf(-lr, g, p);
    }
}

}

extern "C" int wfs_sgd_step(float *param, const float *grad, float *momentum_buf, int64_t n, const float *lr_dev,
                            float momentum, float dampening, float weight_decay, int32_t nesterov, int32_t first_step,
                            void *stream_) {
    hipStream_t stream = (hipStream_t)stream_;
    if (n == 0) return WFS_OK;
    WFS_REQUIRE(param && grad && lr_dev, WFS_EINVAL, "NULL device pointer");
    WFS_REQUIRE(momentum_buf || momentum == 0.f, WFS_EINVAL, "momentum needs a buffer");
    long long blocks = wfs_cdiv(n, 256);
    if (blocks > 2048) blocks = 2048;
    k_sgd_step<<<dim3((unsigned)blocks), dim3(256), 0, stream>>>(param, grad, momentum != 0.f ? momentum_buf : nullptr, n,
                                                                 lr_dev, momentum, dampening, weight_decay, nesterov,
                                                                 first_step);
    WFS_LAUNCH_CHECK();
    return WFS_OK;
}

namespace {

struct AdamCoef {
    float decay, wd, w1, omw1, b2, omb2, bc2s, eps, neg_step;
    int has_wd;
};
static_assert(sizeof(AdamCoef) <= WFS_ADAM_COEF_FLOATS * sizeof(float), "coefficient workspace");

__global__ void __launch_bounds__(64) k_adam_prologue(const double *__restrict__ hp, float *__restrict__ step,
                                                      AdamCoef *__restrict__ coef) {
    if (threadIdx.x != 0) return;
    const float t = *step + 1.f;
    *step = t;
    const double lr = hp[0], beta1 = hp[1], beta2 = hp[2], eps = hp[3], wd = hp[4];
// ... 63 lines not shown
    for (long long i = done + tid; i < n; i += nth) {
        float p = P[i], m = M[i], v = V[i], vm = AMS ? VM[i] : 0.f;
        adam1<AMS>(p, G[i], m, v, vm, c, maximize, decoupled);
        P[i] = p;
        M[i] = m;
        V[i] = v;
        if (AMS) VM[i] = vm;
    }
}

}

extern "C" int wfs_adam_step(float *param, const float *grad, float *exp_avg, float *exp_avg_sq, float *max_exp_avg_sq,
                             int64_t n, const double *hyper_dev, float *step_dev, float *coef_dev, int32_t amsgrad,
                             int32_t maximize, int32_t decoupled, void *stream_) {
    hipStream_t stream = (hipStream_t)stream_;
    WFS_REQUIRE(n >= 0, WFS_EINVAL, "negative size");
    WFS_REQUIRE(param && grad && exp_avg && exp_avg_sq && hyper_dev && step_dev && coef_dev, WFS_EINVAL,
                "NULL device pointer");
    WFS_REQUIRE(max_exp_avg_sq || !amsgrad, WFS_EINVAL, "amsgrad needs max_exp_avg_sq");
    WFS_REQUIRE((uintptr_t)coef_dev % 4 == 0, WFS_EINVAL, "unaligned coefficient workspace");
    AdamCoef *coef = reinterpret_cast<AdamCoef *>(coef_dev);
    k_adam_prologue<<<dim3(1), dim3(64), 0, stream>>>(hyper_dev, step_dev, coef);
    WFS_LAUNCH_CHECK();
    if (n == 0) return WFS_OK;
    float *vm = amsgrad ? max_exp_avg_sq : nullptr;
    const bool vec4 = (((uintptr_t)param | (uintptr_t)grad | (uintptr_t)exp_avg | (uintptr_t)exp_avg_sq |
                        (uintptr_t)vm) & 15) == 0;
    long long blocks = wfs_cdiv(vec4 ? wfs_cdiv(n, 4) : n, 256);
    if (blocks > 512) blocks = 512;
    if (amsgrad)
        k_adam_step<true><<<dim3((unsigned)blocks), dim3(256), 0, stream>>>(param, grad, exp_avg, exp_avg_sq, vm, n,
                                                                            vec4 ? 1 : 0, coef, maximize, decoupled);
    else
        k_adam_step<false><<<dim3((unsigned)blocks), dim3(256), 0, stream>>>(param, grad, exp_avg, exp_avg_sq, nullptr, n,
                                                                             vec4 ? 1 : 0, coef, maximize, decoupled);
    WFS_LAUNCH_CHECK();
    return WFS_OK;
}

namespace {

struct Perm {
    int v[8];
};

__global__ void __launch_bounds__(256) k_load_batch(const int *__restrict__ coords, long long n, int cols, Perm perm,
                                                    int *__restrict__ coords_dst, int *__restrict__ indices_dst,
                                                    const uint4 *__restrict__ feats, uint4 *__restrict__ feats_dst,
                                                    long long feat_words, const unsigned char *__restrict__ feats_tail,
                                                    unsigned char *__restrict__ feats_tail_dst, int tail_bytes,
                                                    const long long *__restrict__ labels, long long *__restrict__ labels_dst,
                                                    long long B, long long *__restrict__ n_valid_dst,
                                                    int *__restrict__ ev_off, int ev_B, int ev_col) {
    const long long tid = (long long)blockIdx.x * 256 + threadIdx.x, nth = (long long)gridDim.x * 256;
    if (tid == 0 && n_valid_dst) *n_valid_dst = n;
    if (ev_off && blockIdx.x < WFS_EVENT_FLAG_WORDS) {
        int bad = 0;
        if (n == 0)
            for (int e = blockIdx.x * 256 + threadIdx.x; e <= ev_B; e += WFS_EVENT_FLAG_WORDS * 256) ev_off[e] = 0;
        for (long long j = (long long)blockIdx.x * 256 + threadIdx.x; j < n; j += (long long)WFS_EVENT_FLAG_WORDS * 256) {
            const int b = coords[j * cols + ev_col];
            const int bp = j > 0 ? coords[(j - 1) * cols + ev_col] : -1;
            const bool ok = b >= 0 && b < ev_B && b >= bp && bp >= -1 && bp < ev_B;
            bad |= ok ? 0 : 1;
            if (ok) {
                for (int e = bp + 1; e <= b; ++e) ev_off[e] = (int)j;
                if (j == n - 1)
                    for (int e = b + 1; e <= ev_B; ++e) ev_off[e] = (int)n;
            }
        }
        bad = __syncthreads_or(bad);
        if (threadIdx.x == 0) ev_off[ev_B + 1 + blockIdx.x] = bad;
    }
    if (cols == 4 && ((reinterpret_cast<uintptr_t>(coords) | reinterpret_cast<uintptr_t>(coords_dst) |
                       reinterpret_cast<uintptr_t>(indices_dst)) & 15) == 0) {
        const int4 *src = reinterpret_cast<const int4 *>(coords);
        int4 *dst = reinterpret_cast<int4 *>(coords_dst), *idx = reinterpret_cast<int4 *>(indices_dst);
        const int p0 = perm.v[0], p1 = perm.v[1], p2 = perm.v[2], p3 = perm.v[3];
        auto pick = [](const int4 &r, int p) { return p == 0 ? r.x : (p == 1 ? r.y : (p == 2 ? r.z : r.w)); };
        for (long long row = tid; row < n; row += nth) {
            const int4 r = src[row];
            if (dst) dst[row] = r;
            if (idx) idx[row] = int4{pick(r, p0), pick(r, p1), pick(r, p2), pick(r, p3)};
        }
    } else {
        for (long long i = tid; i < n * cols; i += nth) {
            const long long row = i / cols;
            const int col = (int)(i - row * cols);
            if (coords_dst) coords_dst[i] = coords[i];
            if (indices_dst) indices_dst[i] = coords[row * cols + perm.v[col]];
        }
    }
    for (long long i = tid; i < feat_words; i += nth) feats_dst[i] = feats[i];
    for (long long i = tid; i < tail_bytes; i += nth) feats_tail_dst[i] = feats_tail[i];
    for (long long i = tid; i < B; i += nth) labels_dst[i] = labels[i];
}

}

extern "C" int wfs_load_batch(const int32_t *coords, int64_t n, int32_t cols, const int32_t *perm_host,
                              int32_t *coords_dst, int32_t *indices_dst, const void *feats, void *feats_dst,
                              int64_t feat_bytes, const int64_t *labels, int64_t *labels_dst, int64_t B,
                              int64_t *n_valid_dst, int32_t *event_offsets, int32_t events, void *stream_) {
    hipStream_t stream = (hipStream_t)stream_;
    WFS_REQUIRE(cols >= 1 && cols <= 8, WFS_EINVAL, "bad coordinate width %d", cols);
    WFS_REQUIRE(n >= 0 && B >= 0 && feat_bytes >= 0, WFS_EINVAL, "negative size");
    WFS_REQUIRE((n == 0 || coords) && (feat_bytes == 0 || (feats && feats_dst)) && (B == 0 || (labels && labels_dst)),
                WFS_EINVAL, "NULL device pointer");
    Perm pm;
    for (int c = 0; c < 8; ++c) {
        pm.v[c] = (perm_host && c < cols) ? perm_host[c] : c;
        WFS_REQUIRE(pm.v[c] >= 0 && pm.v[c] < (c < cols ? cols : 8), WFS_EINVAL, "bad column permutation");
    }
    const bool aligned = ((uintptr_t)feats % 16 == 0) && ((uintptr_t)feats_dst % 16 == 0);
    const long long words = aligned ? feat_bytes / 16 : 0;
    const int tail = (int)(feat_bytes - words * 16 > (1 << 30) ? 0 : feat_bytes - words * 16);
    WFS_REQUIRE(aligned || feat_bytes < (1 << 30), WFS_EINVAL, "unaligned feature buffers");
    long long work = n * cols > words ? n * cols : words;
    long long blocks = wfs_cdiv(work > 0 ? work : 1, 256);
    if (blocks > 1024) blocks = 1024;
    WFS_REQUIRE(!event_offsets || events >= 1, WFS_EINVAL, "event offsets of %d events", events);
    if (event_offsets && blocks < WFS_EVENT_FLAG_WORDS) blocks = WFS_EVENT_FLAG_WORDS;
    k_load_batch<<<dim3((unsigned)blocks), dim3(256), 0, stream>>>(
        coords, n, cols, pm, coords_dst, indices_dst, (const uint4 *)feats, (uint4 *)feats_dst, words,
        (const unsigned char *)feats + words * 16, (unsigned char *)feats_dst + words * 16, tail, (const long long *)labels,
        (long long *)labels_dst, B, (long long *)n_valid_dst, event_offsets, events, pm.v[0]);
    WFS_LAUNCH_CHECK();
    return WFS_OK;
}
```

waveformml_amd/csrc/wfs_common.h:

```cpp
#pragma once
#include <hip/hip_runtime.h>
#include <stdint.h>
#include <stdio.h>

#include <type_traits>

#include "../../include/wfsparse.h"

#define WFS_WAVE 64

void wfs_set_error(const char *fmt, ...);

#define WFS_HIP_CHECK(expr)                                                                  \
    do {                                                                                     \
        hipError_t _e = (expr);                                                              \
        if (_e != hipSuccess) {                                                              \
            wfs_set_error("%s failed: %s (%s:%d)", #expr, hipGetErrorString(_e), __FILE__,   \
                          __LINE__);                                                         \
            return WFS_EHIP;                                                                 \
        }                                                                                    \
    } while (0)

#define WFS_LAUNCH_CHECK() WFS_HIP_CHECK(hipGetLastError())

// ... 71 lines not shown
    bool is_ident = true, is_mirror = true;
    for (int k = 0; k < K && kmap_host; ++k) {
        is_ident = is_ident && kmap_host[k] == k;
        is_mirror = is_mirror && kmap_host[k] == K - 1 - k;
    }
    return is_ident ? WFS_KMAP_IDENTITY : (is_mirror ? WFS_KMAP_MIRROR : WFS_KMAP_OTHER);
}

template <typename F>
static inline int wfs_with_dtype(int dtype, F &&f) {
    if (dtype == WFS_F32) return f(float{});
    if (dtype == WFS_BF16) return f(wfs_bf16{});
    return f(wfs_f16{});
}
template <typename F>
static inline int wfs_with_h16(int dtype, F &&f) {
    if (dtype == WFS_BF16) return f(wfs_bf16{});
    return f(wfs_f16{});
}
template <int V0, int... Vs, typename F>
static inline int wfs_with_int(int v, F &&f) {
    if constexpr (sizeof...(Vs) == 0) {
        return f(std::integral_constant<int, V0>{});
    } else {
        if (v == V0) return f(std::integral_constant<int, V0>{});
        return wfs_with_int<Vs...>(v, f);
    }
}

__device__ __forceinline__ long long wfs_valid_rows(long long cap, const long long *dev) {
    long long v = dev ? *dev : cap;
    return v < cap ? v : cap;
}
__device__ __forceinline__ long long wfs_valid_rows_nonneg(long long cap, const long long *dev) {
    long long v = dev ? *dev : cap;
    v = v < cap ? v : cap;
    return v > 0 ? v : 0;
}

struct WfsTimerScope {
    int timer;
    hipStream_t stream;
    void *rec;
    WfsTimerScope(int timer, hipStream_t stream);
    ~WfsTimerScope();
};

bool wfs_mfma_gconv32_ok(int K);
int wfs_launch_gconv32_f32(const int *table, int mirror, int K, int identity_k, long long R, const long long *r_dev,
                           const float *X, const float *W, int transpose_w, const float *bias, float *Y,
                           hipStream_t stream, int packed_kl = 0);
int wfs_launch_gconv32_h16(const int *table, int mirror, int K, int identity_k, long long R, const long long *r_dev,
                           const void *X, const float *W, int transpose_w, const float *bias, void *Y, int dtype,
                           hipStream_t stream, int packed_kl = 0);
int wfs_launch_gconv_c2c32(const int *table, const int *kmap, int K, int identity_k, long long R,
                           const long long *r_dev, const void *X, const float *W, const float *bias, void *Y, int dtype,
                           hipStream_t stream);
bool wfs_wide_dw_ok(int K, long long R, int Cs, int Cg, int dtype);
size_t wfs_wide_dw_workspace(int K, long long R, int Cs, int Cg, int dtype);
int wfs_launch_wide_dw(const int *table, const int *kmap_host, int K, int identity_k, long long R, const long long *r_dev,
                       const void *S, int Cs, const void *G, long long G_rows, int Cg, int swap, float *dW, int dtype,
                       void *workspace, size_t workspace_bytes, hipStream_t stream);
size_t wfs_dw_fast_workspace(int K, long long R, int Cs, int Cg);
int wfs_launch_gdw32(const int *table, int K, int identity_k, long long R, const long long *r_dev, const void *S,
                     const void *G, int swap, float *dW, float *part, int dtype, wfs_dw_job *defer, hipStream_t stream,
                     int packed_kl = 0);
bool wfs_bwd32_fused_ok(int K, int packed_kl, int dtype);
int wfs_launch_bwd32_h16(const int *table, int packed_kl, int K, int identity_k, long long R, const long long *r_dev,
                         const void *S, const void *G, const float *W, void *dX, int swap, float *dW, float *part, int dtype,
                         wfs_dw_job *defer, hipStream_t stream);
int wfs_launch_gdw_c32c2(const int *table, int mirror, int K, int identity_k, long long R, const long long *r_dev,
                         const void *S, const void *G, int swap, float *dW, float *part, int dtype,
                         wfs_dw_job *defer, hipStream_t stream);
int wfs_launch_dw_jobs(const wfs_dw_job *jobs, int n, hipStream_t stream);
int wfs_launch_bn_bwd_reduce(const void *X, const void *dY, long long N, int C, const float *gamma, const float *beta,
                             const float *save_mean, const float *save_invstd, int relu, float *partial, int dtype,
                             const long long *n_dev, hipStream_t stream, int *nblk_out);
long long wfs_first_bn_slabs(long long R);
int wfs_launch_first_bn_bwd(const int *table, int mirror, int K, int identity_k, long long R, const long long *r_dev,
                            const void *Z, const void *dY, const void *X, const float *gamma, const float *beta,
                            const float *mean, const float *invstd, int relu, const float *partial, int nblk, float *dW,
                            float *dgamma, float *dbeta, float *part, int dtype, wfs_dw_job *defer, hipStream_t stream);
```

waveformml_amd/psd/graph.py:

```python
import contextlib
import gc
import os
import sys

import torch
import torch.distributed as dist

from .. import _lib
from ..spconv import ops
from .voxel import Voxelizer


@contextlib.contextmanager
def _no_gc():
    was = gc.isenabled()
    gc.disable()
    try:
        yield
    finally:
        if was:
            gc.enable()


def _round_up(v, m):
    return int((int(v) + m - 1) // m * m)


def steps_in_graph(optimizer):
    if getattr(optimizer, "flat_device_step", False):
        return True
    return all(g.get("capturable", True) for g in optimizer.param_groups)


class _CapturedRunner(object):

    @staticmethod
    def _headroom_granule(rows, labels, headroom=None, granule=None):
        if headroom is None and os.environ.get("WFS_CAPTURE_HEADROOM"):
            headroom = float(os.environ["WFS_CAPTURE_HEADROOM"])
        if headroom is None:
            headroom = max(1.1, 1.0 + 3.0 / max(1.0, float(labels)) ** 0.5)
        if granule is None:
            granule = 512 if rows >= 32768 else (256 if rows >= 2048 else 64)
        return headroom, granule

    @classmethod
    def capacity_for(cls, rows, labels):
        headroom, granule = cls._headroom_granule(int(rows), int(labels))
        return _round_up(headroom * int(rows), granule)

    def _static_buffers(self, module, example_batch, headroom, granule, min_rows=0, per_row=False):
        (coords, feats), labels = example_batch
        assert coords.is_cuda and feats.is_cuda
        dev = coords.device
        self.module, self.per_row = module, per_row
        self.graph, self._graphs = None, []
        self.n_cap = max(_round_up(headroom * coords.shape[0], granule), _round_up(min_rows, granule))
        self.coords = torch.zeros((self.n_cap, coords.shape[1]), dtype=coords.dtype, device=dev)
        self.feats = torch.zeros((self.n_cap, feats.shape[1]), dtype=feats.dtype, device=dev)
        if per_row:
            self.labels = torch.full((self.n_cap,) + tuple(labels.shape[1:]), self.ignore_index, dtype=labels.dtype,
                                     device=dev)
        else:
            self.labels = torch.zeros_like(labels)
        self.n_valid = torch.zeros((1,), dtype=torch.int64, device=dev)
        self.n_events = int(self.n_cap if per_row else labels.shape[0])
        net = getattr(module, "model", None)
        perm = getattr(net, "permute_tensor", None)
        self._perm = [int(v) for v in perm.tolist()] if perm is not None else None
        self.indices = torch.zeros_like(self.coords) if self._perm is not None else None
        self.events = None
        return net

    def _own_stream(self, dev):
        if torch.cuda.current_stream(dev) == torch.cuda.default_stream(dev):
            st = torch.cuda.Stream(dev)
            st.wait_stream(torch.cuda.default_stream(dev))
            torch.cuda.set_stream(st)
        self.stream = torch.cuda.current_stream(dev)

    def _fresh_flags(self):
        self._owners = [m for m in self.module.modules() if isinstance(m, ops.StickyFlags)]
        for m in self._owners:
            m.fresh_sticky_flags()

    def _calibrate(self, factor, slack, granule):
        for m in self._owners:
            count = m.calibration_count()
            if count is not None:
                m.out_capacity = _round_up(slack * factor * count, granule)

    def _capture(self, fn):
        graph = torch.cuda.CUDAGraph()
        mode = "thread_local" if (dist.is_available() and dist.is_initialized()) else "global"
        with _no_gc(), torch.cuda.graph(graph, stream=self.stream, capture_error_mode=mode):
            out = fn()
        self._graphs.append(graph)
        return graph, out

    def _collect_flags(self):
        self._stores = [m._sticky_flags() for m in self._owners]
        self._overflow, self._voxel_overflow, self._event_flags = [], [], []
        for m, store in zip(self._owners, self._stores):
            if "overflow" in store:
                (self._voxel_overflow if isinstance(m, Voxelizer) else self._overflow).append(store["overflow"])
            self._event_flags += [store[k] for k in ("events", "conv_events") if k in store]
        for t in self._overflow + self._voxel_overflow + self._event_flags:
            t.zero_()

    def check(self):
        _check_flags(self._overflow, self._voxel_overflow, self._event_flags, self.coords.device)

    def close(self):
        if self.graph is None:
            return
        torch.cuda.synchronize(self.coords.device)
        for g in self._graphs:
            g.reset()
        self.graph, self._graphs = None, []
        net = getattr(self.module, "model", None)
        if net is not None:
            if getattr(net, "batch_events", None) is not None and net.batch_events[0] is self.coords:
                net.batch_events = None
            if getattr(net, "batch_first_indices", None) is not None and net.batch_first_indices[0] is self.coords:
                net.batch_first_indices = None
        torch.cuda.synchronize(self.coords.device)

    def fits(self, batch):
        (coords, _f), labels = batch
        if self.per_row:
            return coords.shape[0] <= self.n_cap and labels.shape[0] == coords.shape[0]
        return coords.shape[0] <= self.n_cap and tuple(labels.shape) == tuple(self.labels.shape)

    def _load(self, batch):
        if torch.cuda.current_stream(self.coords.device) == torch.cuda.default_stream(self.coords.device):
            torch.cuda.set_stream(self.stream)
        (coords, feats), labels = batch
        n = coords.shape[0]
        if n > self.n_cap:
            raise RuntimeError("batch has %d voxels, the captured step holds %d" % (n, self.n_cap))
        if self.per_row:
            self.coords[:n].copy_(coords, non_blocking=True)
            self.feats[:n].copy_(feats, non_blocking=True)
            self.labels.fill_(self.ignore_index)
            self.labels[:n].copy_(labels, non_blocking=True)
            self.n_valid.fill_(n)
            if self.indices is not None:
                self.indices[:n].copy_(coords[:, self._perm], non_blocking=True)
            self._event_offsets()
            return
        if (coords.is_cuda and coords.dtype == torch.int32 and coords.is_contiguous() and feats.is_cuda
                and feats.is_contiguous() and feats.dtype == self.feats.dtype and labels.is_cuda
                and labels.dtype == torch.int64 and labels.is_contiguous() and labels.shape == self.labels.shape):
            lib = _lib.load()
            perm = _lib.i32_array(self._perm) if self._perm is not None else None
            ev = self.events if (self.events is not None and perm is not None) else None
            _lib.check(lib.wfs_load_batch(_lib.ptr(coords), n, coords.shape[1], perm, _lib.ptr(self.coords),
                                          _lib.ptr(self.indices), _lib.ptr(feats), _lib.ptr(self.feats),
                                          feats.numel() * feats.element_size(), _lib.ptr(labels), _lib.ptr(self.labels),
                                          labels.numel(), _lib.ptr(self.n_valid), _lib.ptr(ev), self.n_events,
                                          _lib.stream_ptr()))
            if ev is None:
                self._event_offsets()
            return
        self.coords[:n].copy_(coords, non_blocking=True)
        self.feats[:n].copy_(feats, non_blocking=True)
        self.labels.copy_(labels, non_blocking=True)
        self.n_valid.fill_(n)
        if self.indices is not None:
            self.indices[:n].copy_(coords[:, self._perm], non_blocking=True)
        self._event_offsets()

    def _event_offsets(self):
        if self.events is None:
            return
        _lib.check(_lib.load().wfs_event_offsets(_lib.ptr(self.indices), self.indices.shape[0], self.indices.shape[1] - 1,
                                                 self.n_events, _lib.ptr(self.n_valid), _lib.ptr(self.events),
                                                 _lib.stream_ptr()))


class GraphedTrainStep(_CapturedRunner):
    def __init__(self, module, optimizer, reducer, example_batch, headroom=None, granule=None, warmup=2, min_rows=0):
        (coords, feats), labels = example_batch
        headroom, granule = self._headroom_granule(int(coords.shape[0]), int(labels.shape[0]), headroom, granule)
        assert labels.is_cuda
        per_row = bool(getattr(module, "per_row_targets", False)) and labels.shape[0] == coords.shape[0]
        if per_row:
            self.ignore_index = int(getattr(getattr(module, "criterion", None), "ignore_index", -100))
        net = self._static_buffers(module, example_batch, headroom, granule, min_rows, per_row)
        self.optimizer, self.reducer = optimizer, reducer
        dev = coords.device
        if per_row and net is not None and hasattr(net, "batch_size_hint"):
            net.batch_size_hint = self.n_cap
        if (ops.EVENT_LOCAL and self.indices is not None and 1 <= self.n_events <= ops.EVENT_LOCAL_MAX_BATCH
                and hasattr(net, "batch_events")):
            self.events = torch.zeros((int(_lib.load().wfs_event_offsets_ints(self.n_events)),), dtype=torch.int32,
                                      device=dev)
            net.batch_events = (self.coords, self.events)
        self.world = reducer.world
        exchange = bool(getattr(reducer, "exchange", self.world > 1))
        self.in_graph_exchange = (exchange and dist.is_available() and dist.is_initialized()
                                  and dist.get_backend(reducer.group) == "nccl"
                                  and os.environ.get("WFS_GRAPH_EXCHANGE", "1") != "0")
        if self.in_graph_exchange:
            self.in_graph_exchange = _collective_capture_works(reducer.group, dev)
        self.exchange_after = exchange and not self.in_graph_exchange
        self.in_graph_optimizer = not self.exchange_after and steps_in_graph(optimizer)
        self._own_stream(dev)
        self._fresh_flags()
        reducer.reset()
        loss = module.training_step(([coords, feats], labels), 0)
        loss.backward()
        reducer.finish()
        optimizer.step()
        del loss
        own = _round_up(headroom * coords.shape[0], granule)
        factor = headroom if self.n_cap <= own else self.n_cap / max(1.0, float(coords.shape[0]))
        slack = 1.06 if headroom < 1.05 else 1.0
        self._calibrate(factor, slack, granule)
        if self.exchange_after:
            reducer.remove()
        if self.indices is not None:
            net.batch_first_indices = (self.coords, self.indices)
        self._load(example_batch)
        failed, err = 0, None
        try:
            self._warm_and_capture(warmup)
        except Exception as e:
            if not self.in_graph_exchange:
                raise
            failed, err = 1, e
        if self.in_graph_exchange and self.world > 1:
            failed = _agree_max(failed, reducer.group)
        if failed:
            print("[waveformml_amd] in-graph gradient exchange could not be captured on some rank (%s); exchanging "
                  "after the replay" % (("%s: %s" % (type(err).__name__, err)) if err is not None else "another rank"),
                  file=sys.stderr, flush=True)
            torch.cuda.synchronize()
            self.in_graph_exchange, self.exchange_after, self.in_graph_optimizer = False, True, False
            reducer.remove()
            self._warm_and_capture(warmup)
        self._collect_flags()

    def _warm_and_capture(self, warmup):
        for _ in range(warmup):
            self._body()
            if not self.in_graph_optimizer:
                self._after()
        torch.cuda.synchronize()
        self.graph, self.loss = self._capture(self._body)

    def close(self, remove_hooks=True):
        if self.graph is not None and remove_hooks:
            self.reducer.remove()
        super().close()
        self.loss = None

    def _static_batch(self):
        return ([self.coords, self.feats, self.n_valid], self.labels)

    def _body(self):
        self.reducer.reset()
        from ..spconv import functional as Fsp
        loss = self.module.training_step(self._static_batch(), 0)
        Fsp.defer_dw(self.reducer.flat_param is not None)
        try:
            if loss.dtype == torch.float32 and loss.dim() == 0:
                torch.autograd.backward(loss, grad_tensors=Fsp.unit_loss_grad(loss.device))
            else:
                loss.backward()
            if self.in_graph_exchange:
                self.reducer.finish()
            else:
                self.reducer.pack_all()
        finally:
            Fsp.defer_dw(False)
        if self.in_graph_optimizer:
            self.optimizer.step()
        return loss.detach()

    def _after(self):
        if self.exchange_after:
            self.reducer.exchange_packed()
        self.optimizer.step()

    def eager_step(self, batch):
        self.reducer.reset()
        net = getattr(self.module, "model", None)
        hint = getattr(net, "batch_size_hint", None)
        if self.per_row and hint is not None:
            net.batch_size_hint = None
        try:
            loss = self.module.training_step(batch, 0)
        finally:
            if self.per_row and hint is not None:
                net.batch_size_hint = hint
        loss.backward()
        if self.exchange_after:
            self.reducer.pack_all()
            self.reducer.exchange_packed()
        else:
            self.reducer.finish()
        self.optimizer.step()
        return loss.detach()

    def fits_counts(self, rows_max, labels_min, labels_max, rows_ne_labels):
        if self.per_row:
            return rows_max <= self.n_cap and not rows_ne_labels
        return rows_max <= self.n_cap and labels_min == labels_max == int(self.labels.shape[0])

    def __call__(self, batch):
        self._load(batch)
        if hasattr(self.optimizer, "sync_hyperparameters"):
            self.optimizer.sync_hyperparameters()
# ... 86 lines not shown
        work.wait()
        r = t[self.FIELDS * i: self.FIELDS * (i + 1)].tolist()
        return int(r[0]), -int(r[2]), int(r[1]), bool(r[3])


_EVENTS_MESSAGE = ("a batch was not grouped by event (or an event exceeded the LDS tables of the event-local rulebook "
                   "build, or held duplicate coordinates); set WFS_EVENT_LOCAL=0 and re-capture")


def _check_flags(conv, voxels, events, dev, reduce=None):
    def any_set(flags):
        if not flags:
            return torch.zeros((), dtype=torch.bool, device=dev)
        return torch.stack([f.any() for f in flags]).any()
    words = torch.stack([any_set([f[: 2 * (f.numel() // 3)] for f in events]), any_set(conv),
                         any_set(voxels)]).to(torch.int32)
    if reduce is not None:
        reduce(words)
    bad_events, conv_over, voxel_over = (bool(w) for w in words.tolist())
    for t in conv + voxels + events:
        t.zero_()
    if bad_events:
        raise RuntimeError(_EVENTS_MESSAGE)
    if conv_over and voxel_over:
        raise RuntimeError("a batch exceeded the captured voxel capacity AND a sparse conv output exceeded its captured "
                           "capacity; re-capture with more headroom")
    if voxel_over:
        raise RuntimeError("a batch had more voxels than the captured voxel capacity (psd/voxel.Voxelizer); re-capture "
                           "with more headroom or on a busier batch")
    if conv_over:
        raise RuntimeError("a sparse conv output exceeded its captured capacity; re-capture with more headroom")


class GraphedEvalStep(_CapturedRunner):

    def __init__(self, module, example_batch, headroom=None, granule=None, sweep=False, min_rows=0):
        (coords, feats), labels = example_batch
        headroom, granule = self._headroom_granule(int(coords.shape[0]), int(labels.shape[0]), headroom, granule)
        net = self._static_buffers(module, example_batch, headroom, granule, min_rows=min_rows)
        self.feats_loaded = torch.zeros_like(self.feats) if sweep else None
        self._own_stream(coords.device)
        self._reuse, self.graph_fwd = None, None
        was_training = module.training
        module.eval()
        try:
            with torch.no_grad():
                self._fresh_flags()
                if hasattr(net, "batch_size_hint"):
                    net.batch_size_hint = self.n_events
                net([coords, feats])
                self._calibrate(headroom, 1.0, granule)
                if self.indices is not None:
                    net.batch_first_indices = (self.coords, self.indices)
                self._load(example_batch)
                if sweep:
                    self._reuse = ops.reuse_rulebooks()
                    self._reuse.__enter__()
                for _ in range(2):
                    self._forward()
                torch.cuda.synchronize()
                self.graph, self.logits = self._capture(self._forward)
                self._collect_flags()
                if sweep:
                    before = ops.BUILD_COUNT
                    self.graph_fwd, self.logits_fwd = self._capture(self._forward)
                    assert ops.BUILD_COUNT == before, "the forward-only capture rebuilt a rulebook"
        finally:
            module.train(was_training)

    def _forward(self):
        net = self.module.model
        if hasattr(net, "batch_size_hint"):
            net.batch_size_hint = self.n_events
        return net([self.coords, self.feats, self.n_valid]).float()

    def __call__(self, batch, occlude_index=None):
        self._load(batch)
        if self.feats_loaded is not None:
            self.feats_loaded.copy_(self.feats)
        if occlude_index:
            self.feats[:, occlude_index] = 0
        self.graph.replay()
        return self.logits

    def rerun(self, occlude_index=None):
        if self.graph_fwd is None:
            raise RuntimeError("GraphedEvalStep(..., sweep=True) captures the forward-only graph that rerun() replays")
        self.feats.copy_(self.feats_loaded)
        if occlude_index:
            self.feats[:, occlude_index] = 0
        self.graph_fwd.replay()
        return self.logits_fwd

    def close(self):
        if self._reuse is not None:
            self._reuse.__exit__(None, None, None)
            self._reuse = None
        super().close()
        self.graph_fwd = None
```

waveformml_amd/spconv/conv.py:

```python
import math

import numpy as np
import torch
from torch import nn
from torch.nn import init

from . import functional as Fsp
from . import ops
from .modules import SparseModule
from .tensor import IndiceData, SparseConvTensor


class SparseConvolution(SparseModule, ops.StickyFlags):
    def __init__(self, ndim, in_channels, out_channels, kernel_size=3, stride=1, padding=0, dilation=1,
                 groups=1, bias=True, subm=False, output_padding=0, transposed=False, inverse=False,
                 indice_key=None, fused_bn=False, use_hash=False, algo=None):
        super(SparseConvolution, self).__init__()
        assert groups == 1
        self.ndim = ndim
        self.in_channels = in_channels
        self.out_channels = out_channels
        self.kernel_size = ops._listify(kernel_size, ndim)
        self.conv1x1 = int(np.prod(self.kernel_size)) == 1
        self.stride = ops._listify(stride, ndim)
        self.padding = ops._listify(padding, ndim)
        self.dilation = ops._listify(dilation, ndim)
        self.transposed = transposed
        self.inverse = inverse
        self.output_padding = ops._listify(output_padding, ndim)
        self.groups = groups
        self.subm = subm
        self.indice_key = indice_key
        self.fused_bn = fused_bn
        self.use_hash = use_hash
        self.algo = algo
        for d, s in zip(self.dilation, self.stride):
            assert any([s == 1, d == 1]), "don't support this."
        self.weight = nn.Parameter(torch.Tensor(*self.kernel_size, in_channels, out_channels))
        if bias:
            self.bias = nn.Parameter(torch.Tensor(out_channels))
        else:
            self.register_parameter('bias', None)
        self.reset_parameters()

    def calibration_count(self):
        if self.subm or self.conv1x1 or self.inverse:
            return None
        return self.last_rulebook.M

    def reset_parameters(self):
        init.kaiming_uniform_(self.weight, a=math.sqrt(5))
        if self.bias is not None:
            fan_in, _ = init._calculate_fan_in_and_fan_out(self.weight)
            bound = 1 / math.sqrt(fan_in)
            init.uniform_(self.bias, -bound, bound)

    def forward(self, input, bn_tail=None):
        assert isinstance(input, SparseConvTensor)
        features = input.features
        indices = input.indices
        spatial_shape = input.spatial_shape
        batch_size = input.batch_size
        if self.transposed:
            out_spatial_shape = ops.get_deconv_output_size(spatial_shape, self.kernel_size, self.stride,
                                                           self.padding, self.dilation, self.output_padding)
        elif not self.subm:
            out_spatial_shape = ops.get_conv_output_size(spatial_shape, self.kernel_size, self.stride,
                                                         self.padding, self.dilation)
        else:
            out_spatial_shape = spatial_shape
        if self.conv1x1:
            features = Fsp.pointwise_conv(features, self.weight, self.bias, input.n_valid)
            out_tensor = SparseConvTensor(features, input.indices, input.spatial_shape, input.batch_size)
            out_tensor.indice_dict = input.indice_dict
            out_tensor.grid = input.grid
            out_tensor.unique = input.unique
            out_tensor.n_valid = input.n_valid
            out_tensor.prefetched = getattr(input, "prefetched", None)
            return out_tensor
        datas = input.find_indice_pair(self.indice_key)
        fused = False
        if self.inverse:
            assert datas is not None and self.indice_key is not None
            rb = datas.rulebook
            out_spatial_shape = datas.spatial_shape
            assert rb.K == np.prod(self.kernel_size), "inverse conv must have same kernel size as its couple conv"
            out_indices = rb.indices
            out_features = Fsp.indice_inverse_conv(features, self.weight, self.bias, rb)
            out_unique = None if rb.has_dup else True
            out_n_valid = rb.n_dev
        else:
            pre = getattr(input, "prefetched", None)
            if pre is not None and id(self) in pre:
                rb = pre[id(self)]
                if rb.ready is not None:
                    rb.ready.wait()
                self.last_rulebook = rb
                input.unique = not rb.has_dup
                if datas is None:
                    input.indice_dict[self.indice_key] = IndiceData(rb, spatial_shape)
            elif self.indice_key is not None and datas is not None:
                rb = datas.rulebook
            else:
                rb = ops.build_rulebook(indices, batch_size, spatial_shape, self.kernel_size, self.stride,
                                        self.padding, self.dilation, self.subm, known_unique=input.unique,
                                        n_dev=input.n_valid, out_capacity=getattr(self, "out_capacity", None),
                                        transposed=self.transposed, output_padding=self.output_padding,
                                        events=getattr(input, "events", None), flags=self._sticky_flags(),
                                        want_cell_map=getattr(input, "dense_follows", True))
                if getattr(rb, "events_in", None) is not None:
                    input.events = rb.events_in
                self.last_rulebook = rb
                input.unique = not rb.has_dup
                input.indice_dict[self.indice_key] = IndiceData(rb, spatial_shape)
            out_indices = rb.out_indices
            fused = (bn_tail is not None and not self.transposed
                     and Fsp.first_conv_bn_ok(features, self.weight, self.bias, rb, bn_tail[0]))
            if fused:
                out_features = features
                out_unique = input.unique if self.subm else True
            elif self.subm:
                out_features = Fsp.indice_subm_conv(features, self.weight, self.bias, rb)
                out_unique = input.unique
            else:
                out_features = Fsp.indice_conv(features, self.weight, self.bias, rb)
                out_unique = True
            out_n_valid = rb.m_dev
        out_tensor = SparseConvTensor(out_features, out_indices, out_spatial_shape, batch_size)
        out_tensor.indice_dict = input.indice_dict
        out_tensor.grid = input.grid
        out_tensor.unique = out_unique
        out_tensor.n_valid = out_n_valid
        out_tensor.prefetched = getattr(input, "prefetched", None)
        if self.subm:
            out_tensor.events = getattr(input, "events", None)
        elif not self.inverse and getattr(rb, "events_out", None) is not None:
            out_tensor.events = rb.events_out
        if not self.subm and not self.inverse:
            out_tensor.cell_map = getattr(rb, "cell_map", None)
        if not self.inverse and fused:
            bn, relu, between = bn_tail
            out_tensor.features = Fsp.first_conv_bn_relu(features, self.weight, rb, bn, relu,
                                                         None if between is None else (lambda: between(out_tensor)))
            out_tensor.bn_applied = True
        return out_tensor


def _conv_class(name, ndim, **fixed):
    def __init__(self, in_channels, out_channels, kernel_size, stride=1, padding=0, dilation=1, groups=1,
                 bias=True, indice_key=None, use_hash=False, algo=None):
        SparseConvolution.__init__(self, ndim, in_channels, out_channels, kernel_size, stride, padding, dilation,
                                   groups, bias, indice_key=indice_key, use_hash=use_hash, algo=algo, **fixed)
    return type(name, (SparseConvolution,), {"__init__": __init__, "__module__": __name__})


def _inverse_class(name, ndim):
    def __init__(self, in_channels, out_channels, kernel_size, indice_key=None, bias=True, algo=None):
        SparseConvolution.__init__(self, ndim, in_channels, out_channels, kernel_size, bias=bias, inverse=True,
                                   indice_key=indice_key, algo=algo)
    return type(name, (SparseConvolution,), {"__init__": __init__, "__module__": __name__})


def _transpose_class(name, ndim):
    def __init__(self, in_channels, out_channels, kernel_size, stride=1, padding=0, dilation=1, groups=1,
                 bias=True, indice_key=None, algo=None):
        SparseConvolution.__init__(self, ndim, in_channels, out_channels, kernel_size, stride, padding, dilation,
                                   groups, bias, transposed=True, indice_key=indice_key, algo=algo)
    return type(name, (SparseConvolution,), {"__init__": __init__, "__module__": __name__})


SparseConv1d = _conv_class("SparseConv1d", 1)
SparseConv2d = _conv_class("SparseConv2d", 2)
SparseConv3d = _conv_class("SparseConv3d", 3)
SparseConv4d = _conv_class("SparseConv4d", 4)
SubMConv1d = _conv_class("SubMConv1d", 1, subm=True)
SubMConv2d = _conv_class("SubMConv2d", 2, subm=True)
SubMConv3d = _conv_class("SubMConv3d", 3, subm=True)
SubMConv4d = _conv_class("SubMConv4d", 4, subm=True)
# ... 5 lines not shown
```

waveformml_amd/spconv/functional.py:

```python
import ctypes

import torch
from torch.autograd import Function

from .. import _lib

CONV, SUBM, INVERSE = 0, 1, 2

ACCOUNT = None


def _account(kind, table, R, rows_in, c_in, rows_out, c_out, K, cw_in, cw_out, esize):
    if ACCOUNT is None:
        return
    pairs = int((table >= 0).sum().item()) if table is not None else int(R)
    ACCOUNT.append(dict(kind=kind, pairs=pairs,
                        bytes=rows_in * c_in * esize + rows_out * c_out * esize + pairs * 8 + K * cw_in * cw_out * 4,
                        flops=2 * pairs * cw_in * cw_out))


def _features_ok(t):
    if not t.is_cuda:
        raise RuntimeError("waveformml_amd.spconv: features must be on the GPU (there is no CPU path)")
    return t.contiguous()
# ... 8 lines not shown
    return torch.empty(shape, dtype=like.dtype, device=like.device)


def _masked_column_sum(t, r_dev):
    lib = _lib.load()
    t = t.contiguous()
    R, C = int(t.shape[0]), int(t.shape[1])
    out = torch.empty((C,), dtype=torch.float32, device=t.device)
    ws = torch.empty((int(lib.wfs_column_sum_workspace_bytes(C)),), dtype=torch.uint8, device=t.device)
    _lib.check(lib.wfs_column_sum(_lib.ptr(t), R, C, _lib.ptr(out), _lib.ptr(ws), ws.numel(), _lib.dtype_code(t),
                                  _lib.ptr(r_dev), _lib.stream_ptr()))
    return out




def _fast_shape(Cx, Cy):
    return (Cx == 32 and Cy == 32) or (Cx == 2 and Cy == 32) or (Cx == 32 and Cy == 2)


def filters16(W, like):
    lib = _lib.load()
    K, Cw_in, Cw_out = int(W.shape[0]), int(W.shape[1]), int(W.shape[2])
    if like.dtype == torch.float32 and Cw_out % 4 == 0:
        return None
    code = _lib.dtype_code(like)
    out = torch.empty((int(lib.wfs_wide_filters_bytes(K, Cw_in, Cw_out, code)),), dtype=torch.uint8, device=W.device)
    _lib.check(lib.wfs_wide_filters(_lib.ptr(W), K, Cw_in, Cw_out, code, _lib.ptr(out), _lib.stream_ptr()))
    return out


def takes_wide_path(K, R, X, Cy):
    return bool(X.is_cuda and X.dtype in (torch.float32, torch.bfloat16, torch.float16)
                and _lib.load().wfs_wide_conv_ok(K, R, X.shape[0], int(X.shape[1]), int(Cy), _lib.dtype_code(X)))


def _wide_gather_conv(lib, table, kmap, K, identity_k, R, X, W, transpose_w, bias, r_dev, w16=None):
    Cw_in, Cw_out = int(W.shape[-2]), int(W.shape[-1])
    Cx, Cy = int(X.shape[1]), (Cw_in if transpose_w else Cw_out)
    assert W.dtype == torch.float32 and W.is_contiguous() and X.is_contiguous()
    assert Cx == (Cw_out if transpose_w else Cw_in), (X.shape, W.shape, transpose_w)
    assert table is None or (table.dtype == torch.int32 and table.shape == (K, R)), (None if table is None else table.shape, K, R)
    assert bias is None or (bias.dtype == torch.float32 and bias.numel() == Cy)
    Y = _rows((R, Cy), X, r_dev)
    nbytes = lib.wfs_wide_conv_workspace_bytes(K, R, X.shape[0], Cx, Cy, 0 if table is None else 1, _lib.dtype_code(X))
    ws = torch.empty((int(nbytes),), dtype=torch.uint8, device=X.device)
    _lib.check(lib.wfs_wide_gather_conv(_lib.ptr(table), kmap, K, identity_k, R, _lib.ptr(X), X.shape[0], Cx, _lib.ptr(W),
                                        _lib.ptr(w16), Cw_in, Cw_out, 1 if transpose_w else 0, _lib.ptr(bias), _lib.ptr(Y),
                                        _lib.dtype_code(X), _lib.ptr(r_dev), _lib.ptr(ws), ws.numel(), _lib.stream_ptr()))
    _account("gather_conv", table, R, X.shape[0], Cx, R, Cy, K, Cw_in, Cw_out, X.element_size())
    return Y


def gather_conv(table, kmap, K, identity_k, R, X, W, transpose_w, bias, r_dev=None, w16=None, packed_kl=0):
    lib = _lib.load()
    Cw_in, Cw_out = int(W.shape[-2]), int(W.shape[-1])
    if packed_kl:
        assert transpose_w and kmap is None and table.shape == (K // packed_kl, R), (table.shape, K, packed_kl, R)
        Y = _rows((R, Cw_in), X, r_dev)
        _lib.check(lib.wfs_gather_conv(_lib.ptr(table), None, K, identity_k, R, _lib.ptr(X), X.shape[0], X.shape[1],
                                       _lib.ptr(W), Cw_in, Cw_out, 1, None, _lib.ptr(Y), _lib.dtype_code(X),
                                       _lib.ptr(r_dev), packed_kl, _lib.stream_ptr()))
        if ACCOUNT is not None:
            _account("gather_conv", (table >> 3).clamp_(min=-1), R, X.shape[0], X.shape[1], R, Cw_in, K, Cw_in, Cw_out,
                     X.element_size())
        return Y
    if X.is_cuda and lib.wfs_wide_conv_ok(K, R, X.shape[0], int(X.shape[1]), Cw_in if transpose_w else Cw_out, _lib.dtype_code(X)):
        return _wide_gather_conv(lib, table, kmap, K, identity_k, R, X, W, transpose_w, bias, r_dev, w16)
    if transpose_w and not _fast_shape(Cw_out, Cw_in):
        W, transpose_w = W.transpose(1, 2).contiguous(), False
        Cw_in, Cw_out = Cw_out, Cw_in
    Cy = Cw_in if transpose_w else Cw_out
    Y = _rows((R, Cy), X, r_dev)
    assert W.dtype == torch.float32 and W.is_contiguous()
    assert X.dim() == 2 and X.shape[1] == (Cw_out if transpose_w else Cw_in), (X.shape, W.shape, transpose_w)
    assert table is None or (table.dtype == torch.int32 and table.shape == (K, R)), (None if table is None else table.shape, K, R)
    assert bias is None or (bias.dtype == torch.float32 and bias.numel() == Cy)
    _lib.check(lib.wfs_gather_conv(_lib.ptr(table), kmap, K, identity_k, R, _lib.ptr(X), X.shape[0], X.shape[1],
                                   _lib.ptr(W), Cw_in, Cw_out, 1 if transpose_w else 0, _lib.ptr(bias),
                                   _lib.ptr(Y), _lib.dtype_code(X), _lib.ptr(r_dev), 0, _lib.stream_ptr()))
    _account("gather_conv", table, R, X.shape[0], X.shape[1], R, Cy, K, Cw_in, Cw_out, X.element_size())
    return Y


def scatter_conv(table, K, identity_k, R, X, W, transpose_w, n_out, bias):
    lib = _lib.load()
    Cw_in, Cw_out = int(W.shape[-2]), int(W.shape[-1])
    Cy = Cw_in if transpose_w else Cw_out
    Y = torch.zeros((n_out, Cy), dtype=torch.float32, device=X.device)
    if bias is not None:
        Y += bias
    assert table.dtype == torch.int32 and table.shape == (K, R)
    _lib.check(lib.wfs_scatter_conv(_lib.ptr(table), K, identity_k, R, _lib.ptr(X), X.shape[1], _lib.ptr(W), Cw_in,
                                    Cw_out, 1 if transpose_w else 0, _lib.ptr(Y), _lib.dtype_code(X),
                                    _lib.stream_ptr()))
    return Y.to(X.dtype)


_GRAD_SLOTS = []


def register_grad_slots(flat_param, flat_grad):
    import weakref
    _GRAD_SLOTS[:] = [(p, g) for (p, g) in _GRAD_SLOTS if p() is not None and g() is not None]
    _GRAD_SLOTS.append((weakref.ref(flat_param), weakref.ref(flat_grad)))


_SLOTS_WRITTEN = set()


def reset_grad_slots():
    _SLOTS_WRITTEN.clear()


def grad_like(param, shape=None):
    shape = tuple(param.shape) if shape is None else tuple(shape)
    if (param is not None and param.is_cuda and param.dtype == torch.float32 and param.is_contiguous()
            and param.grad is None):
        for pref, gref in _GRAD_SLOTS:
            fp, fg = pref(), gref()
            if fp is None or fg is None or fp.device != param.device or fg.dtype != torch.float32:
                continue
            off = param.data_ptr() - fp.data_ptr()
            if 0 <= off and off + 4 * param.numel() <= 4 * fp.numel() and off % 4 == 0:
                slot = fg.data_ptr() + off
                if slot in _SLOTS_WRITTEN:
                    flush_deferred_dw()
                    _SHARED_SLOTS.add(slot)
                    break
                if not _SLOTS_WRITTEN:
                    try:
                        torch.autograd.Variable._execution_engine.queue_callback(reset_grad_slots)
                    except RuntimeError:
# ... 17 lines not shown

def was_deferred(slot_ptr):
    return slot_ptr in _DEFERRED_SLOTS and slot_ptr not in _SHARED_SLOTS


def flush_deferred_dw():
    if not _DEFERRED_DW:
        return
    lib = _lib.load()
    jobs = (_lib.DwJob * len(_DEFERRED_DW))(*[j for (j, _ws) in _DEFERRED_DW])
    for at in range(0, len(_DEFERRED_DW), 16):
        n = min(16, len(_DEFERRED_DW) - at)
        _lib.check(lib.wfs_dw_reduce_jobs(ctypes.cast(ctypes.byref(jobs, at * ctypes.sizeof(_lib.DwJob)),
                                                      ctypes.POINTER(_lib.DwJob)), n, _lib.stream_ptr()))
    for j, _ws in _DEFERRED_DW:
        _DEFERRED_SLOTS.add(int(j.dW))
    del _DEFERRED_DW[:]


def _dw_job(grad):
    if _DEFERRED_DW is not None and grad is not None and grad._base is not None:
        return _lib.DwJob()
    return None


def _queue_dw_job(job, ws):
    if job is not None and job.nslabs > 0:
        _DEFERRED_DW.append((job, ws))


def gather_dw(table, K, identity_k, R, S, G, swap, kmap=None, r_dev=None, like=None, packed_kl=0):
    lib = _lib.load()
    Cs, Cg = int(S.shape[1]), int(G.shape[1])
    shape = (K, Cg, Cs) if swap else (K, Cs, Cg)
    if like is not None and like.numel() == K * Cs * Cg:
        dW = grad_like(like, shape)
    else:
        dW = torch.empty(shape, dtype=torch.float32, device=S.device)
    assert S.dtype == G.dtype and S.shape[0] == R
    assert table is None or (table.dtype == torch.int32 and table.shape == ((K // packed_kl if packed_kl else K), R))
    nbytes = lib.wfs_gather_dw_workspace_bytes(K, R, Cs, Cg)
    ws = torch.empty((max(int(nbytes), 1),), dtype=torch.uint8, device=S.device)
    job = _dw_job(dW)
    _lib.check(lib.wfs_gather_dw(_lib.ptr(table), kmap, K, identity_k, R, _lib.ptr(S), Cs, _lib.ptr(G), G.shape[0],
                                 Cg, 1 if swap else 0, _lib.ptr(dW), _lib.dtype_code(S), _lib.ptr(ws), ws.numel(),
                                 _lib.ptr(r_dev), job, packed_kl, _lib.stream_ptr()))
    _queue_dw_job(job, ws)
    if ACCOUNT is not None:
        _account("gather_dw", (table >> 3).clamp_(min=-1) if packed_kl else table, R, R, Cs, G.shape[0], Cg, K, Cs, Cg,
                 S.element_size())
    return dW


def conv_backward(table, K, identity_k, R, X, dY, W, r_dev=None, like=None, packed_kl=0):
    lib = _lib.load()
    Cin, Cout = int(X.shape[1]), int(dY.shape[1])
    if like is not None and like.numel() == K * Cin * Cout:
        dW = grad_like(like, (K, Cin, Cout))
    else:
        dW = torch.empty((K, Cin, Cout), dtype=torch.float32, device=X.device)
    dX = _rows((R, Cin), dY, r_dev)
    ws = torch.empty((max(int(lib.wfs_gather_dw_workspace_bytes(K, R, Cin, Cout)), 1),), dtype=torch.uint8, device=X.device)
    job = _dw_job(dW)
    _lib.check(lib.wfs_conv_backward(_lib.ptr(table), K, identity_k, R, _lib.ptr(X), _lib.ptr(dY), dY.shape[0], Cin, Cout,
                                     _lib.ptr(W), _lib.ptr(dX), _lib.ptr(dW), _lib.dtype_code(X), _lib.ptr(ws), ws.numel(),
                                     _lib.ptr(r_dev), job, packed_kl, _lib.stream_ptr()))
    _queue_dw_job(job, ws)
    if ACCOUNT is not None:
        dense = (table >> 3).clamp_(min=-1) if packed_kl else table
        pairs = int((dense >= 0).sum().item())
        es = X.element_size()
        fused = Cin == 32 and Cout == 32 and _one_launch_rows(X.dtype) and K <= 27
        if fused:
            ACCOUNT.append(dict(kind="conv_backward", pairs=pairs,
                                bytes=2 * R * Cin * es + dY.shape[0] * Cout * es + 2 * pairs * 8 + 2 * K * Cin * Cout * 4,
                                flops=4 * pairs * Cin * Cout))
        else:
            _account("gather_dw", dense, R, R, Cin, dY.shape[0], Cout, K, Cin, Cout, es)
            _account("gather_conv", dense, R, dY.shape[0], Cout, R, Cin, K, Cin, Cout, es)
    return dX, dW


SPLIT_BF16 = __import__("os").environ.get("WFS_SPLIT_BF16", "1") != "0"


def _one_launch_rows(dtype):
    return dtype in (torch.bfloat16, torch.float16) or (dtype == torch.float32 and SPLIT_BF16)


class SparseConvFunction(Function):

    @staticmethod
    def forward(ctx, features, filters, bias, rulebook, mode):
        rb = rulebook
        features = _features_ok(features)
        K = rb.K
        W = filters.detach().reshape(K, filters.shape[-2], filters.shape[-1]).float().contiguous()
        b = None if bias is None else bias.detach().float().contiguous()
        ident = rb.centre_k if rb.subm else -1
        w16 = None
        if mode == INVERSE:
            assert features.shape[0] == rb.M, "inverse conv input must be the coupled conv's output set"
            w16 = filters16(W, features) if takes_wide_path(K, rb.N, features, W.shape[2]) else None
            out = gather_conv(rb.nbr_out, None, K, ident, rb.N, features, W, False, b, rb.n_dev, w16)
        elif rb.has_dup:
            out = scatter_conv(rb.nbr_out, K, ident, rb.N, features, W, False, rb.M, b)
        else:
            assert features.shape[0] == rb.N
            table, kmap = rb.table_by_out()
            w16 = filters16(W, features) if takes_wide_path(K, rb.M, features, W.shape[2]) else None
            out = gather_conv(table, kmap, K, ident, rb.M, features, W, False, b, rb.m_dev, w16)
        ctx.save_for_backward(features, filters, bias)
        ctx.rb, ctx.mode = rb, mode
        ctx.w16 = w16 if ctx.needs_input_grad[0] else None
        return out

    @staticmethod
    def backward(ctx, grad_output):
        features, filters, bias = ctx.saved_tensors
        rb, mode = ctx.rb, ctx.mode
        K = rb.K
        dY = as_grad(grad_output, features.dtype)
        W = filters.detach().reshape(K, filters.shape[-2], filters.shape[-1]).float().contiguous()
        ident = rb.centre_k if rb.subm else -1
        dX = dW = db = None
        if mode == INVERSE:
            if ctx.needs_input_grad[0]:
                if rb.has_dup:
                    dX = scatter_conv(rb.nbr_out, K, ident, rb.N, dY, W, True, rb.M, None)
                else:
                    dX = gather_conv(rb.nbr_in, None, K, ident, rb.M, dY, W, True, None, rb.m_dev, ctx.w16)
            if ctx.needs_input_grad[1]:
                dW = gather_dw(rb.nbr_out, K, ident, rb.N, dY, features, True, None, rb.n_dev, filters)
        elif (ctx.needs_input_grad[0] and ctx.needs_input_grad[1] and not rb.has_dup and features.shape[1] == 32
              and dY.shape[1] == 32 and features.is_cuda and _one_launch_rows(features.dtype)):
            table, pk = rb.table_by_in(32, 32, features, 3)
            if pk and rb.table_by_in(32, 32, dY, 1)[1] != pk:
                table, pk = rb.nbr_out, 0
            dX, dW = conv_backward(table, K, ident, rb.N, features, dY, W, rb.n_dev, filters, pk)
        else:
            if ctx.needs_input_grad[1]:
                if features.shape[1] == 2 and dY.shape[1] == 32 and K <= 27 and not rb.has_dup:
                    table, kmap = rb.table_by_out()
                    dW = gather_dw(table, K, ident, rb.M, dY, features, True, kmap, rb.m_dev, filters)
                else:
                    table, pk = rb.table_by_in(features.shape[1], dY.shape[1], features, 3)
                    dW = gather_dw(table, K, ident, rb.N, features, dY, False, None, rb.n_dev, filters, pk)
            if ctx.needs_input_grad[0]:
                table, pk = rb.table_by_in(dY.shape[1], W.shape[1], dY, 1)
                dX = gather_conv(table, None, K, ident, rb.N, dY, W, True, None, rb.n_dev, ctx.w16, pk)
        if dW is not None:
            dW = dW.reshape(filters.shape).to(filters.dtype)
        if bias is not None and ctx.needs_input_grad[2]:
            db = _masked_column_sum(dY, rb.n_dev if mode == INVERSE else rb.m_dev).to(bias.dtype)
        return dX, dW, db, None, None


def maxpool_fwd(table, kmap, K, R, X, r_dev=None):
    lib = _lib.load()
    C = int(X.shape[1])
    assert X.dim() == 2 and table.dtype == torch.int32 and table.shape == (K, R), (X.shape, table.shape, K, R)
    Y = _rows((R, C), X, r_dev)
    _lib.check(lib.wfs_maxpool_fwd(_lib.ptr(table), kmap, K, R, _lib.ptr(X), X.shape[0], C, _lib.ptr(Y),
                                   _lib.dtype_code(X), _lib.ptr(r_dev), _lib.stream_ptr()))
    _account("maxpool_fwd", table, R, X.shape[0], C, R, C, K, 0, 0, X.element_size())
    return Y


def maxpool_bwd(table, K, packed_kl, N, X, Y, dY, n_dev=None):
    lib = _lib.load()
    C = int(X.shape[1])
    assert X.shape[0] == N and Y.shape == dY.shape and Y.shape[1] == C and X.dtype == Y.dtype == dY.dtype
    assert table.dtype == torch.int32 and table.shape == ((K // packed_kl if packed_kl else K), N), (table.shape, K, N)
    dX = _rows((N, C), X, n_dev)
    _lib.check(lib.wfs_maxpool_bwd(_lib.ptr(table), K, packed_kl, N, _lib.ptr(X), _lib.ptr(Y), _lib.ptr(dY), Y.shape[0], C,
                                   _lib.ptr(dX), _lib.dtype_code(X), _lib.ptr(n_dev), _lib.stream_ptr()))
    if ACCOUNT is not None:
        pairs = int(((table >> 3).clamp_(min=-1) if packed_kl else table).ge(0).sum().item())
        ACCOUNT.append(dict(kind="maxpool_bwd", pairs=pairs, flops=0,
                            bytes=(2 * N + 2 * Y.shape[0]) * C * X.element_size() + pairs * 8))
    return dX


class SparseMaxPoolFunction(Function):

    @staticmethod
    def forward(ctx, features, rulebook):
        rb = rulebook
        features = _features_ok(features)
        if rb.has_dup:
            raise RuntimeError("waveformml_amd.spconv: SparseMaxPool needs distinct input coordinates")
        assert features.shape[0] == rb.N
        table, kmap = rb.table_by_out()
        out = maxpool_fwd(table, kmap, rb.K, rb.M, features, rb.m_dev)
        ctx.save_for_backward(features, out)
        ctx.rb = rb
        return out

    @staticmethod
    def backward(ctx, grad_output):
        features, out = ctx.saved_tensors
        rb = ctx.rb
        if not ctx.needs_input_grad[0]:
            return None, None
        dY = as_grad(grad_output, features.dtype)
        table, pk = rb.nbr_out_packed, rb.packed_kl
        if table is None or not _lib.load().wfs_maxpool_packed_ok(pk, rb.K, int(features.shape[1]), _lib.dtype_code(features)):
            table, pk = rb.nbr_out, 0
# ... 518 lines not shown
        grad = grad_loss if grad_loss.dtype == torch.float32 else grad_loss.float()
        dpred = torch.empty_like(pred)
        p = _lib.ptr
        _lib.check(_lib.load().wfs_masked_regression_loss_backward(
            p(pred), _lib.dtype_code(pred), p(target), _lib.dtype_code(target), n_cols, col, p(coords), p(se_mask), nx, ny,
            n_cap, p(n_valid), kind, p(count), p(grad.contiguous()), p(dpred), _lib.stream_ptr()))
        return dpred, None, None, None, None, None, None, None


def regression_loss_kind(criterion):
    if getattr(criterion, "reduction", None) != "mean":
        return None
    if type(criterion) is torch.nn.L1Loss:
        return _lib.WFS_LOSS_L1
    if type(criterion) is torch.nn.MSELoss:
        return _lib.WFS_LOSS_MSE
    return None


def can_fuse_regression_loss(criterion, pred, target):
    return (regression_loss_kind(criterion) is not None and pred.is_cuda and target.is_cuda and pred.dim() == 1
            and target.dim() in (1, 2) and target.shape[0] == pred.shape[0]
            and pred.dtype in (torch.float32, torch.bfloat16, torch.float16)
            and target.dtype in (torch.float32, torch.bfloat16, torch.float16))


def masked_regression_loss(pred, target, kind, col=0, coords=None, se_mask=None, n_valid=None, max_blocks=0):
    return MaskedRegressionLossFunction.apply(pred, target, col, coords, se_mask, n_valid, kind, max_blocks)


_UNIT_LOSS_GRAD = {}


def unit_loss_grad(device):
    device = torch.device(device)
    if device.type == "cuda" and device.index is None:
        device = torch.device("cuda", torch.cuda.current_device())
    if device not in _UNIT_LOSS_GRAD:
        _UNIT_LOSS_GRAD[device] = torch.ones((), dtype=torch.float32, device=device)
    return _UNIT_LOSS_GRAD[device]


def can_fuse_cross_entropy(criterion, logits, target):
    return (type(criterion) is torch.nn.CrossEntropyLoss and criterion.reduction == "mean" and criterion.weight is None
            and getattr(criterion, "label_smoothing", 0.0) == 0.0 and logits.is_cuda and logits.dim() == 2
            and logits.dtype == torch.float32 and target.dtype == torch.int64 and target.dim() == 1
            and logits.shape[0] >= 1 and logits.shape[1] <= 4096)


def cross_entropy_mean(logits, target, ignore_index=-100):
    return CrossEntropyMeanFunction.apply(logits, target, ignore_index)


def indice_conv(features, filters, bias, rulebook):
    return SparseConvFunction.apply(features, filters, bias, rulebook, CONV)


def indice_subm_conv(features, filters, bias, rulebook):
    return SparseConvFunction.apply(features, filters, bias, rulebook, SUBM)


def indice_inverse_conv(features, filters, bias, rulebook):
    return SparseConvFunction.apply(features, filters, bias, rulebook, INVERSE)


def to_dense(features, indices, spatial_shape, batch_size, unique, m_dev=None, cell_map=None):
    return ToDenseFunction.apply(features, indices, spatial_shape, batch_size, unique, m_dev, cell_map)
```

waveformml_amd/spconv/ops.py:

```python
import ctypes

import os

import numpy as np
import torch

from .. import _lib


ASSUME_VALID_UNIQUE_INDICES = False


PREFETCH_RULEBOOKS = False

EVENT_LOCAL = os.environ.get("WFS_EVENT_LOCAL", "1") != "0"
EVENT_LOCAL_MAX_BATCH = 16384

EVENT_LOCAL_CONV = os.environ.get("WFS_EVENT_LOCAL_CONV", "1") != "0"
PACKED_TABLES = os.environ.get("WFS_PACKED_TABLES", "1") != "0"

_SIDE_STREAMS = {}


def side_stream(device):
    key = torch.device(device).index if torch.device(device).index is not None else torch.cuda.current_device()
    if key not in _SIDE_STREAMS:
        _SIDE_STREAMS[key] = torch.cuda.Stream(device)
    return _SIDE_STREAMS[key]


def _listify(v, ndim):
    if isinstance(v, (list, tuple, np.ndarray)):
        v = [int(x) for x in v]
        assert len(v) == ndim, "expected %d values, got %s" % (ndim, v)
        return v
    if torch.is_tensor(v):
        return _listify(v.tolist(), ndim)
    return [int(v)] * ndim


def get_conv_output_size(input_size, kernel_size, stride, padding, dilation):
    ndim = len(input_size)
    out = []
    for i in range(ndim):
        size = (int(input_size[i]) + 2 * padding[i] - dilation[i] * (kernel_size[i] - 1) - 1) // stride[i] + 1
        out.append(int(input_size[i]) if kernel_size[i] == -1 else size)
    return out


def get_deconv_output_size(input_size, kernel_size, stride, padding, dilation, output_padding):
    ndim = len(input_size)
    out = []
    for i in range(ndim):
        if kernel_size[i] == -1:
            raise ValueError("deconv don't support kernel_size < 0")
        out.append((int(input_size[i]) - 1) * stride[i] - 2 * padding[i] + kernel_size[i] + output_padding[i])
    return out


class Rulebook(object):

    def __init__(self):
        self.geometry = None
        self.N = self.M = self.K = 0
        self.subm = False
        self.has_dup = False
        self.indices = None
        self.out_indices = None
        self._nbr_out = None
        self.nbr_out_packed = None
        self.packed_kl = 0
        self.nbr_in = None
# ... 340 lines not shown
```

Measured before the change: 562,800 events/s.

## Precompute bf16 filter images once per step and feed them to 32-channel conv kernels

Adds a prepared bf16 fragment image of each 32x32 conv filter, plus a transposed copy, built alongside batch loading. The forward gather-conv and fused backward kernels then copy these images straight into LDS instead of converting fp32 weights to bf16 fragments in every block. This removes redundant per-block weight conversion work, at the cost of an extra image-building pass and extra memory per layer. Correctness depends on the images being rebuilt after every optimizer step.

```diff
diff --git a/include/wfsparse.h b/include/wfsparse.h
--- a/include/wfsparse.h
+++ b/include/wfsparse.h
@@ -326,6 +326,30 @@
                    int32_t *indices_dst, const void *feats, void *feats_dst, int64_t feat_bytes,
                    const int64_t *labels, int64_t *labels_dst, int64_t B, int64_t *n_valid_dst,
                    int32_t *event_offsets, int32_t events, void *stream);
+
+#define WFS_FILTER_IMAGE_JOBS_MAX 16
+typedef struct wfs_filter_image_job {
+    const float *W;
+    void *img_fwd;
+    void *img_t;
+    int32_t K;
+    int32_t dtype;
+} wfs_filter_image_job;
+size_t wfs_filter_image_bytes(int32_t K);
+int wfs_conv_filter_images(const float *W, int32_t K, int32_t dtype, void *img_fwd, void *img_t, void *stream);
+int wfs_load_batch_images(const int32_t *coords, int64_t n, int32_t cols, const int32_t *perm_host, int32_t *coords_dst,
+                          int32_t *indices_dst, const void *feats, void *feats_dst, int64_t feat_bytes,
+                          const int64_t *labels, int64_t *labels_dst, int64_t B, int64_t *n_valid_dst,
+                          int32_t *event_offsets, int32_t events, const wfs_filter_image_job *jobs, int32_t njobs,
+                          void *stream);
+int wfs_gather_conv_image(const int32_t *table, const int32_t *kmap_host, int32_t K, int32_t identity_k,
+                          int64_t R, const void *X, int64_t X_rows, int32_t Cx, const float *W,
+                          int32_t Cw_in, int32_t Cw_out, int32_t transpose_w, const float *bias, void *Y,
+                          int32_t dtype, const int64_t *r_dev, int32_t packed_kl, const void *image, void *stream);
+int wfs_conv_backward_image(const int32_t *table, int32_t K, int32_t identity_k, int64_t R, const void *X, const void *dY,
+                            int64_t dY_rows, int32_t Cin, int32_t Cout, const float *W, void *dX, float *dW, int32_t dtype,
+                            void *workspace, size_t workspace_bytes, const int64_t *r_dev, wfs_dw_job *defer,
+                            int32_t packed_kl, const void *image_t, void *stream);
 
 #define WFS_EVAL_MAX_SAMPLES 512
 size_t wfs_eval_table_ints(int32_t n_bins, int32_t n_mult, int32_t n_confusion, int32_t n_se_max, int32_t nx,
diff --git a/waveformml_amd/_lib.py b/waveformml_amd/_lib.py
--- a/waveformml_amd/_lib.py
+++ b/waveformml_amd/_lib.py
@@ -37,6 +37,12 @@
     _fields_ = [("part", _vp), ("nslabs", _i64), ("per", _i64), ("K", _i32), ("A", _i32), ("B", _i32),
                 ("transpose", _i32), ("dW", _vp)]
 
+
+class FilterImageJob(ctypes.Structure):
+    _fields_ = [("W", _vp), ("img_fwd", _vp), ("img_t", _vp), ("K", _i32), ("dtype", _i32)]
+
+
+FILTER_IMAGE_JOBS_MAX = 16
 
 SIGNATURES = {
     "wfs_abi_version": (ctypes.c_int, []),
@@ -161,6 +167,14 @@
     "wfs_adam_step": (ctypes.c_int, [_vp, _vp, _vp, _vp, _vp, _i64, _vp, _vp, _vp, _i32, _i32, _i32, _vp]),
     "wfs_load_batch": (ctypes.c_int, [_vp, _i64, _i32, c_i32p, _vp, _vp, _vp, _vp, _i64, _vp, _vp, _i64, _vp, _vp, _i32,
                                       _vp]),
+    "wfs_filter_image_bytes": (_sz, [_i32]),
+    "wfs_conv_filter_images": (ctypes.c_int, [_vp, _i32, _i32, _vp, _vp, _vp]),
+    "wfs_load_batch_images": (ctypes.c_int, [_vp, _i64, _i32, c_i32p, _vp, _vp, _vp, _vp, _i64, _vp, _vp, _i64, _vp, _vp,
+                                             _i32, ctypes.POINTER(FilterImageJob), _i32, _vp]),
+    "wfs_gather_conv_image": (ctypes.c_int, [_vp, c_i32p, _i32, _i32, _i64, _vp, _i64, _i32, _vp, _i32, _i32, _i32,
+                                             _vp, _vp, _i32, _vp, _i32, _vp, _vp]),
+    "wfs_conv_backward_image": (ctypes.c_int, [_vp, _i32, _i32, _i64, _vp, _vp, _i64, _i32, _i32, _vp, _vp, _vp, _i32, _vp,
+                                               _sz, _vp, ctypes.POINTER(DwJob), _i32, _vp, _vp]),
     "wfs_eval_table_ints": (_sz, [_i32, _i32, _i32, _i32, _i32, _i32, _i32]),
     "wfs_event_pulse_stats": (ctypes.c_int, [_vp, _vp, _i64, _i32, _i32, _vp, _i32, _vp, _vp, _i32, _i32, _i32, _vp, _vp,
                                              _vp, _vp, _vp, _vp, _vp, _vp, _vp, _vp, _vp, _vp, _vp]),
diff --git a/waveformml_amd/csrc/conv_mfma.hip b/waveformml_amd/csrc/conv_mfma.hip
--- a/waveformml_amd/csrc/conv_mfma.hip
+++ b/waveformml_amd/csrc/conv_mfma.hip
@@ -362,12 +362,24 @@
                                                   long long R, const long long *__restrict__ r_dev,
                                                   const H *__restrict__ X, const float *__restrict__ W,
                                                   const float *__restrict__ bias, H *__restrict__ Y, long long ntiles,
-                                                  long long tiles_per_xcd) {
+                                                  long long tiles_per_xcd, const uint4 *__restrict__ img) {
     uint4 *sWb = reinterpret_cast<uint4 *>(smem);
     int *sNb = reinterpret_cast<int *>(smem + (size_t)K * 2048);
     constexpr int WSB = 5;
     const int nfrag = K * 128;
-    if (!(WFS_KNOCK & 1))
+    if (!(WFS_KNOCK & 1) && img != nullptr) {
+        for (int u0 = threadIdx.x; u0 < nfrag; u0 += nthreads * WSB) {
+            uint4 f[WSB];
+#pragma unroll
+            for (int b = 0; b < WSB; ++b) {
+                const int u = u0 + b * nthreads;
+                f[b] = img[u < nfrag ? u : nfrag - 1];
+            }
+#pragma unroll
+            for (int b = 0; b < WSB; ++b)
+                if (u0 + b * nthreads < nfrag) sWb[u0 + b * nthreads] = f[b];
+        }
+    } else if (!(WFS_KNOCK & 1))
     for (int u0 = threadIdx.x; u0 < nfrag; u0 += nthreads * WSB) {
         float w[WSB][8];
 #pragma unroll
@@ -503,10 +515,10 @@
                                                        const H *__restrict__ X,
                                                        const float *__restrict__ W, const float *__restrict__ bias,
                                                        H *__restrict__ Y, long long ntiles,
-                                                       long long tiles_per_xcd) {
+                                                       long long tiles_per_xcd, const uint4 *__restrict__ img) {
     extern __shared__ __attribute__((aligned(16))) unsigned char smem[];
     gconv32_bf16_body<H, TRANSPOSE_W, PK>(smem, (int)blockIdx.x, (int)gridDim.x, (int)blockDim.x, table, mirror, K,
-                                          identity_k, R, r_dev, X, W, bias, Y, ntiles, tiles_per_xcd);
+                                          identity_k, R, r_dev, X, W, bias, Y, ntiles, tiles_per_xcd, img);
 }
 
 template <typename T>
@@ -1072,7 +1084,8 @@
                                                      const long long *__restrict__ r_dev, const H *__restrict__ S,
                                                      const H *__restrict__ G, const float *__restrict__ W,
                                                      H *__restrict__ dX, float *__restrict__ part, int ngroups,
-                                                     int nbx_dw, int n_dw_pad, int n_dx, int dx_threads) {
+                                                     int nbx_dw, int n_dw_pad, int n_dx, int dx_threads,
+                                                     const uint4 *__restrict__ img_t) {
     extern __shared__ __attribute__((aligned(16))) unsigned char smem[];
     const int bid = (int)blockIdx.x;
     if (bid < n_dw_pad) {
@@ -1082,7 +1095,7 @@
     } else {
         if ((int)threadIdx.x >= dx_threads) return;
         gconv32_bf16_body<H, true, PK>(smem, bid - n_dw_pad, n_dx, dx_threads, table, 0, K, identity_k, Rcap, r_dev, G, W,
-                                       nullptr, dX, 0, 0);
+                                       nullptr, dX, 0, 0, img_t);
     }
 }
 
@@ -1590,7 +1603,7 @@
 template <typename H>
 static int launch_gconv32_h16(const int *table, int mirror, int K, int identity_k, long long R, const long long *r_dev,
                               const H *Xb, const float *W, int transpose_w, const float *bias, H *Yb,
-                              hipStream_t stream, int packed_kl) {
+                              hipStream_t stream, int packed_kl, const uint4 *img) {
     long long ntiles, nblk, tiles_per_xcd;
     int wpb;
     gconv32_grid(R, r_dev != nullptr, &ntiles, &wpb, &nblk, &tiles_per_xcd, 16);
@@ -1602,23 +1615,23 @@
     if (packed_kl) {
         static bool attr_p = false;
         return launch_big_lds(k_gconv32_bf16<H, true, 3>, &attr_p, grid, block, lds, stream, table, mirror, K, identity_k, R,
-                              r_dev, Xb, W, bias, Yb, ntiles, tiles_per_xcd);
+                              r_dev, Xb, W, bias, Yb, ntiles, tiles_per_xcd, img);
     }
     if (transpose_w)
         return launch_big_lds(k_gconv32_bf16<H, true>, &attr[0], grid, block, lds, stream, table, mirror, K, identity_k, R,
-                              r_dev, Xb, W, bias, Yb, ntiles, tiles_per_xcd);
+                              r_dev, Xb, W, bias, Yb, ntiles, tiles_per_xcd, img);
     return launch_big_lds(k_gconv32_bf16<H, false>, &attr[1], grid, block, lds, stream, table, mirror, K, identity_k, R,
-                          r_dev, Xb, W, bias, Yb, ntiles, tiles_per_xcd);
+                          r_dev, Xb, W, bias, Yb, ntiles, tiles_per_xcd, img);
 }
 
 int wfs_launch_gconv32_h16(const int *table, int mirror, int K, int identity_k, long long R, const long long *r_dev,
                            const void *X, const float *W, int transpose_w, const float *bias, void *Y, int dtype,
-                           hipStream_t stream, int packed_kl) {
+                           hipStream_t stream, int packed_kl, const void *image) {
     if (dtype == WFS_F16)
         return launch_gconv32_h16<wfs_f16>(table, mirror, K, identity_k, R, r_dev, (const wfs_f16 *)X, W, transpose_w,
-                                           bias, (wfs_f16 *)Y, stream, packed_kl);
+                                           bias, (wfs_f16 *)Y, stream, packed_kl, (const uint4 *)image);
     return launch_gconv32_h16<wfs_bf16>(table, mirror, K, identity_k, R, r_dev, (const wfs_bf16 *)X, W, transpose_w, bias,
-                                        (wfs_bf16 *)Y, stream, packed_kl);
+                                        (wfs_bf16 *)Y, stream, packed_kl, (const uint4 *)image);
 }
 
 int wfs_launch_gconv_c2c32(const int *table, const int *kmap, int K, int identity_k, long long R,
@@ -1728,7 +1741,8 @@
 
 template <typename H>
 static int launch_bwd32_h16(const int *table, int packed_kl, int K, int identity_k, long long R, const long long *r_dev,
-                            const H *S, const H *G, const float *W, H *dX, float *part, hipStream_t stream) {
+                            const H *S, const H *G, const float *W, H *dX, float *part, hipStream_t stream,
+                            const uint4 *img_t) {
     const long long nbx_dw = dw32_blocks(R, false);
     const int ngroups = (K + DWB_KG - 1) / DWB_KG;
     const long long n_dw = nbx_dw * ngroups, n_dw_pad = (n_dw + 7) / 8 * 8;
@@ -1741,11 +1755,11 @@
     if (packed_kl) {
         static bool attr = false;
         return launch_big_lds(k_bwd32_bf16<H, 3>, &attr, grid, block, lds, stream, table, K, identity_k, R, r_dev, S, G, W, dX,
-                              part, ngroups, (int)nbx_dw, (int)n_dw_pad, (int)n_dx, wpb * 64);
+                              part, ngroups, (int)nbx_dw, (int)n_dw_pad, (int)n_dx, wpb * 64, img_t);
     }
     static bool attr0 = false;
     return launch_big_lds(k_bwd32_bf16<H, 0>, &attr0, grid, block, lds, stream, table, K, identity_k, R, r_dev, S, G, W, dX,
-                          part, ngroups, (int)nbx_dw, (int)n_dw_pad, (int)n_dx, wpb * 64);
+                          part, ngroups, (int)nbx_dw, (int)n_dw_pad, (int)n_dx, wpb * 64, img_t);
 }
 
 bool wfs_bwd32_fused_ok(int K, int packed_kl, int dtype) {
@@ -1788,17 +1802,17 @@
 
 int wfs_launch_bwd32_h16(const int *table, int packed_kl, int K, int identity_k, long long R, const long long *r_dev,
                          const void *S, const void *G, const float *W, void *dX, int swap, float *dW, float *part, int dtype,
-                         wfs_dw_job *defer, hipStream_t stream) {
+                         wfs_dw_job *defer, hipStream_t stream, const void *image_t) {
     int rc;
     if (dtype == WFS_F32)
         rc = launch_bwd32_split(table, packed_kl, K, identity_k, R, r_dev, (const float *)S, (const float *)G, W, (float *)dX,
                                 part, stream);
     else if (dtype == WFS_F16)
         rc = launch_bwd32_h16<wfs_f16>(table, packed_kl, K, identity_k, R, r_dev, (const wfs_f16 *)S, (const wfs_f16 *)G, W,
-                                       (wfs_f16 *)dX, part, stream);
+                                       (wfs_f16 *)dX, part, stream, (const uint4 *)image_t);
     else
         rc = launch_bwd32_h16<wfs_bf16>(table, packed_kl, K, identity_k, R, r_dev, (const wfs_bf16 *)S, (const wfs_bf16 *)G,
-                                        W, (wfs_bf16 *)dX, part, stream);
+                                        W, (wfs_bf16 *)dX, part, stream, (const uint4 *)image_t);
     if (rc != WFS_OK) return rc;
     return dw_reduce_or_defer(part, dw32_blocks(R, false), (long long)K * 1024, K, 32, 32, swap, dW, defer, stream);
 }
diff --git a/waveformml_amd/csrc/gather_conv.hip b/waveformml_amd/csrc/gather_conv.hip
--- a/waveformml_amd/csrc/gather_conv.hip
+++ b/waveformml_amd/csrc/gather_conv.hip
@@ -349,8 +349,9 @@
 static int gather_conv_impl(const int32_t *table, const int32_t *kmap_host, int32_t K, int32_t identity_k,
                             int64_t R, const void *X, int64_t X_rows, int32_t Cx, const float *W, int32_t Cw_in,
                             int32_t Cw_out, int32_t transpose_w, const float *bias, void *Y, int32_t dtype,
-                            const int64_t *r_dev_, void *stream_, int packed_kl = 0) {
+                            const int64_t *r_dev_, void *stream_, int packed_kl = 0, const void *image = nullptr) {
     hipStream_t stream = (hipStream_t)stream_;
+    WFS_REQUIRE(((uintptr_t)image & 15) == 0, WFS_EINVAL, "the filter image must be 16-byte aligned");
     WFS_REQUIRE(packed_kl == 0 || wfs_gather_packed_ok(packed_kl, K, Cx, transpose_w ? Cw_in : Cw_out, dtype, transpose_w ? 1 : 2),
                 WFS_EINVAL, "a packed table (kl %d) is not taken by this product (wfs_gather_packed_ok): expand it with "
                 "wfs_unpack_table", packed_kl);
@@ -378,7 +379,7 @@
     }
     if (dtype != WFS_F32 && Cx == 32 && Cy == 32 && K <= 27 && table && kind != WFS_KMAP_OTHER && X_rows < (1ll << 25)) {
         return wfs_launch_gconv32_h16(table, mirror, K, identity_k, R, r_dev, X, W, transpose_w, bias, Y, dtype, stream,
-                                      packed_kl);
+                                      packed_kl, image);
     }
     WFS_REQUIRE(packed_kl == 0, WFS_EINVAL, "a packed table reached a kernel that reads dense ones");
     if (Cx == 2 && Cy == 32 && !transpose_w && table)
@@ -418,6 +419,15 @@
     WFS_REQUIRE(packed_kl == 0 || !kmap_host, WFS_EINVAL, "a packed table takes no column map");
     return gather_conv_impl(table, kmap_host, K, identity_k, R, X, X_rows, Cx, W, Cw_in, Cw_out, transpose_w, bias, Y,
                             dtype, r_dev, stream, packed_kl);
+}
+
+extern "C" int wfs_gather_conv_image(const int32_t *table, const int32_t *kmap_host, int32_t K, int32_t identity_k,
+                                     int64_t R, const void *X, int64_t X_rows, int32_t Cx, const float *W, int32_t Cw_in,
+                                     int32_t Cw_out, int32_t transpose_w, const float *bias, void *Y, int32_t dtype,
+                                     const int64_t *r_dev, int32_t packed_kl, const void *image, void *stream) {
+    WFS_REQUIRE(packed_kl == 0 || !kmap_host, WFS_EINVAL, "a packed table takes no column map");
+    return gather_conv_impl(table, kmap_host, K, identity_k, R, X, X_rows, Cx, W, Cw_in, Cw_out, transpose_w, bias, Y,
+                            dtype, r_dev, stream, packed_kl, image);
 }
 
 extern "C" int wfs_gather_packed_ok(int32_t packed_kl, int32_t K, int32_t Ca, int32_t Cb, int32_t dtype, int32_t which) {
@@ -540,7 +550,17 @@
                                  const void *dY, int64_t dY_rows, int32_t Cin, int32_t Cout, const float *W, void *dX,
                                  float *dW, int32_t dtype, void *workspace, size_t workspace_bytes, const int64_t *r_dev,
                                  wfs_dw_job *defer, int32_t packed_kl, void *stream_) {
+    return wfs_conv_backward_image(table, K, identity_k, R, X, dY, dY_rows, Cin, Cout, W, dX, dW, dtype, workspace,
+                                   workspace_bytes, r_dev, defer, packed_kl, nullptr, stream_);
+}
+
+extern "C" int wfs_conv_backward_image(const int32_t *table, int32_t K, int32_t identity_k, int64_t R, const void *X,
+                                       const void *dY, int64_t dY_rows, int32_t Cin, int32_t Cout, const float *W,
+                                       void *dX, float *dW, int32_t dtype, void *workspace, size_t workspace_bytes,
+                                       const int64_t *r_dev, wfs_dw_job *defer, int32_t packed_kl, const void *image_t,
+                                       void *stream_) {
     hipStream_t stream = (hipStream_t)stream_;
+    WFS_REQUIRE(((uintptr_t)image_t & 15) == 0, WFS_EINVAL, "the filter image must be 16-byte aligned");
     WFS_REQUIRE(dX && dW, WFS_EINVAL, "wfs_conv_backward computes both gradients (use wfs_gather_conv / wfs_gather_dw for one)");
     const long long row_lim = dtype == WFS_F32 ? (1ll << 24) : (1ll << 25);
     const bool fused = Cin == 32 && Cout == 32 && table && wfs_bwd32_fused_ok(K, packed_kl, dtype) && R > 0 &&
@@ -550,7 +570,7 @@
                                 workspace_bytes, r_dev, defer, stream_, packed_kl);
         if (rc != WFS_OK) return rc;
         return gather_conv_impl(table, nullptr, K, identity_k, R, dY, dY_rows, Cout, W, Cin, Cout, 1, nullptr, dX, dtype, r_dev,
-                                stream_, packed_kl);
+                                stream_, packed_kl, image_t);
     }
     WFS_REQUIRE(X && dY && W && workspace, WFS_EINVAL, "NULL device pointer");
     const size_t need = wfs_gather_dw_workspace_bytes(K, R, Cin, Cout);
@@ -558,7 +578,7 @@
     if (defer) *defer = wfs_dw_job_none();
     WfsTimerScope timer(WFS_TIMER_CONV_BACKWARD, stream);
     return wfs_launch_bwd32_h16(table, packed_kl, K, identity_k, R, (const long long *)r_dev, X, dY, W, dX, 0, dW,
-                                (float *)workspace, dtype, defer, stream);
+                                (float *)workspace, dtype, defer, stream, image_t);
 }
 
 static size_t first_bn_slab_bytes(int32_t K, int64_t R) {
diff --git a/waveformml_amd/csrc/optim.hip b/waveformml_amd/csrc/optim.hip
--- a/waveformml_amd/csrc/optim.hip
+++ b/waveformml_amd/csrc/optim.hip
@@ -1,4 +1,5 @@
 #include "wfs_common.h"
+#include "wfs_filterimg.h"
 
 namespace {
 
@@ -168,8 +169,16 @@
                                                     unsigned char *__restrict__ feats_tail_dst, int tail_bytes,
                                                     const long long *__restrict__ labels, long long *__restrict__ labels_dst,
                                                     long long B, long long *__restrict__ n_valid_dst,
-                                                    int *__restrict__ ev_off, int ev_B, int ev_col) {
-    const long long tid = (long long)blockIdx.x * 256 + threadIdx.x, nth = (long long)gridDim.x * 256;
+                                                    int *__restrict__ ev_off, int ev_B, int ev_col, int copy_blocks,
+                                                    WfsFilterImageJobs images) {
+    if ((int)blockIdx.x >= copy_blocks) {
+        const int b = (int)blockIdx.x - copy_blocks;
+        for (int i = 0; i < images.n; ++i)
+            if (b >= images.first_block[i] && b < images.first_block[i + 1])
+                wfs_filter_images_block(images.j[i], b - images.first_block[i]);
+        return;
+    }
+    const long long tid = (long long)blockIdx.x * 256 + threadIdx.x, nth = (long long)copy_blocks * 256;
     if (tid == 0 && n_valid_dst) *n_valid_dst = n;
     if (ev_off && blockIdx.x < WFS_EVENT_FLAG_WORDS) {
         int bad = 0;
@@ -213,13 +222,57 @@
     for (long long i = tid; i < B; i += nth) labels_dst[i] = labels[i];
 }
 
+__global__ void __launch_bounds__(256) k_filter_images(wfs_filter_image_job job) {
+    wfs_filter_images_block(job, (int)blockIdx.x);
+}
+
+int filter_image_job_ok(const wfs_filter_image_job &j) {
+    WFS_REQUIRE(j.K >= 1 && j.K <= 32, WFS_EINVAL, "filter image of K = %d (1 .. 32)", j.K);
+    WFS_REQUIRE(j.dtype == WFS_BF16 || j.dtype == WFS_F16, WFS_EINVAL, "filter images are 16-bit (dtype %d)", j.dtype);
+    WFS_REQUIRE(j.W && ((uintptr_t)j.W & 3) == 0, WFS_EINVAL, "NULL or misaligned filter");
+    WFS_REQUIRE((((uintptr_t)j.img_fwd | (uintptr_t)j.img_t) & 15) == 0, WFS_EINVAL, "images must be 16-byte aligned");
+    return WFS_OK;
+}
+
+}
+
+extern "C" size_t wfs_filter_image_bytes(int32_t K) { return K > 0 ? (size_t)K * 2048 : 0; }
+
+extern "C" int wfs_conv_filter_images(const float *W, int32_t K, int32_t dtype, void *img_fwd, void *img_t,
+                                      void *stream_) {
+    const wfs_filter_image_job job{W, img_fwd, img_t, K, dtype};
+    const int rc = filter_image_job_ok(job);
+    if (rc != WFS_OK) return rc;
+    if (!img_fwd && !img_t) return WFS_OK;
+    k_filter_images<<<dim3((unsigned)K), dim3(256), 0, (hipStream_t)stream_>>>(job);
+    WFS_LAUNCH_CHECK();
+    return WFS_OK;
 }
 
 extern "C" int wfs_load_batch(const int32_t *coords, int64_t n, int32_t cols, const int32_t *perm_host,
                               int32_t *coords_dst, int32_t *indices_dst, const void *feats, void *feats_dst,
                               int64_t feat_bytes, const int64_t *labels, int64_t *labels_dst, int64_t B,
                               int64_t *n_valid_dst, int32_t *event_offsets, int32_t events, void *stream_) {
+    return wfs_load_batch_images(coords, n, cols, perm_host, coords_dst, indices_dst, feats, feats_dst, feat_bytes, labels,
+                                 labels_dst, B, n_valid_dst, event_offsets, events, nullptr, 0, stream_);
+}
+
+extern "C" int wfs_load_batch_images(const int32_t *coords, int64_t n, int32_t cols, const int32_t *perm_host,
+                                     int32_t *coords_dst, int32_t *indices_dst, const void *feats, void *feats_dst,
+                                     int64_t feat_bytes, const int64_t *labels, int64_t *labels_dst, int64_t B,
+                                     int64_t *n_valid_dst, int32_t *event_offsets, int32_t events,
+                                     const wfs_filter_image_job *jobs, int32_t njobs, void *stream_) {
     hipStream_t stream = (hipStream_t)stream_;
+    WFS_REQUIRE(njobs >= 0 && njobs <= WFS_FILTER_IMAGE_JOBS_MAX && (njobs == 0 || jobs), WFS_EINVAL,
+                "%d filter image jobs (0 .. %d)", njobs, WFS_FILTER_IMAGE_JOBS_MAX);
+    WfsFilterImageJobs images = {};
+    for (int i = 0; i < njobs; ++i) {
+        const int rc = filter_image_job_ok(jobs[i]);
+        if (rc != WFS_OK) return rc;
+        images.j[i] = jobs[i];
+        images.first_block[i + 1] = images.first_block[i] + jobs[i].K;
+    }
+    images.n = njobs;
     WFS_REQUIRE(cols >= 1 && cols <= 8, WFS_EINVAL, "bad coordinate width %d", cols);
     WFS_REQUIRE(n >= 0 && B >= 0 && feat_bytes >= 0, WFS_EINVAL, "negative size");
     WFS_REQUIRE((n == 0 || coords) && (feat_bytes == 0 || (feats && feats_dst)) && (B == 0 || (labels && labels_dst)),
@@ -238,10 +291,10 @@
     if (blocks > 1024) blocks = 1024;
     WFS_REQUIRE(!event_offsets || events >= 1, WFS_EINVAL, "event offsets of %d events", events);
     if (event_offsets && blocks < WFS_EVENT_FLAG_WORDS) blocks = WFS_EVENT_FLAG_WORDS;
-    k_load_batch<<<dim3((unsigned)blocks), dim3(256), 0, stream>>>(
+    k_load_batch<<<dim3((unsigned)(blocks + images.first_block[njobs])), dim3(256), 0, stream>>>(
         coords, n, cols, pm, coords_dst, indices_dst, (const uint4 *)feats, (uint4 *)feats_dst, words,
         (const unsigned char *)feats + words * 16, (unsigned char *)feats_dst + words * 16, tail, (const long long *)labels,
-        (long long *)labels_dst, B, (long long *)n_valid_dst, event_offsets, events, pm.v[0]);
-    WFS_LAUNCH_CHECK();
-    return WFS_OK;
-}
+        (long long *)labels_dst, B, (long long *)n_valid_dst, event_offsets, events, pm.v[0], (int)blocks, images);
+    WFS_LAUNCH_CHECK();
+    return WFS_OK;
+}
diff --git a/waveformml_amd/csrc/wfs_common.h b/waveformml_amd/csrc/wfs_common.h
--- a/waveformml_amd/csrc/wfs_common.h
+++ b/waveformml_amd/csrc/wfs_common.h
@@ -147,7 +147,7 @@
                            hipStream_t stream, int packed_kl = 0);
 int wfs_launch_gconv32_h16(const int *table, int mirror, int K, int identity_k, long long R, const long long *r_dev,
                            const void *X, const float *W, int transpose_w, const float *bias, void *Y, int dtype,
-                           hipStream_t stream, int packed_kl = 0);
+                           hipStream_t stream, int packed_kl = 0, const void *image = nullptr);
 int wfs_launch_gconv_c2c32(const int *table, const int *kmap, int K, int identity_k, long long R,
                            const long long *r_dev, const void *X, const float *W, const float *bias, void *Y, int dtype,
                            hipStream_t stream);
@@ -163,7 +163,7 @@
 bool wfs_bwd32_fused_ok(int K, int packed_kl, int dtype);
 int wfs_launch_bwd32_h16(const int *table, int packed_kl, int K, int identity_k, long long R, const long long *r_dev,
                          const void *S, const void *G, const float *W, void *dX, int swap, float *dW, float *part, int dtype,
-                         wfs_dw_job *defer, hipStream_t stream);
+                         wfs_dw_job *defer, hipStream_t stream, const void *image_t = nullptr);
 int wfs_launch_gdw_c32c2(const int *table, int mirror, int K, int identity_k, long long R, const long long *r_dev,
                          const void *S, const void *G, int swap, float *dW, float *part, int dtype,
                          wfs_dw_job *defer, hipStream_t stream);
diff --git a/waveformml_amd/csrc/wfs_filterimg.h b/waveformml_amd/csrc/wfs_filterimg.h
--- /dev/null
+++ b/waveformml_amd/csrc/wfs_filterimg.h
@@ -0,0 +1,41 @@
+#pragma once
+#include "wfs_common.h"
+
+struct WfsFilterImageJobs {
+    wfs_filter_image_job j[WFS_FILTER_IMAGE_JOBS_MAX];
+    int first_block[WFS_FILTER_IMAGE_JOBS_MAX + 1];
+    int n;
+};
+
+template <typename H, bool TRANSPOSE_W>
+__device__ __forceinline__ uint4 wfs_filter_fragment(const float *__restrict__ W, int u) {
+    const int k = u >> 7, s = (u >> 6) & 1, h = (u >> 5) & 1, col = u & 31;
+    const int c0 = 16 * h + 8 * s;
+    float w[8];
+    if (!TRANSPOSE_W) {
+#pragma unroll
+        for (int j = 0; j < 8; ++j) w[j] = W[((long long)k * 32 + c0 + j) * 32 + col];
+    } else {
+        const float4 *src = reinterpret_cast<const float4 *>(W + ((long long)k * 32 + col) * 32 + c0);
+        const float4 lo = src[0], hi = src[1];
+        w[0] = lo.x; w[1] = lo.y; w[2] = lo.z; w[3] = lo.w;
+        w[4] = hi.x; w[5] = hi.y; w[6] = hi.z; w[7] = hi.w;
+    }
+    uint4 v;
+    v.x = wfs_pack2<H>(w[0], w[1]);
+    v.y = wfs_pack2<H>(w[2], w[3]);
+    v.z = wfs_pack2<H>(w[4], w[5]);
+    v.w = wfs_pack2<H>(w[6], w[7]);
+    return v;
+}
+
+__device__ __forceinline__ void wfs_filter_images_block(const wfs_filter_image_job &job, int b) {
+    const int t = (int)threadIdx.x, u = b * 128 + (t & 127);
+    if (b >= job.K || t >= 256) return;
+    uint4 *dst = reinterpret_cast<uint4 *>(t < 128 ? job.img_fwd : job.img_t);
+    if (!dst) return;
+    if (job.dtype == WFS_F16)
+        dst[u] = t < 128 ? wfs_filter_fragment<wfs_f16, false>(job.W, u) : wfs_filter_fragment<wfs_f16, true>(job.W, u);
+    else
+        dst[u] = t < 128 ? wfs_filter_fragment<wfs_bf16, false>(job.W, u) : wfs_filter_fragment<wfs_bf16, true>(job.W, u);
+}
diff --git a/waveformml_amd/psd/graph.py b/waveformml_amd/psd/graph.py
--- a/waveformml_amd/psd/graph.py
+++ b/waveformml_amd/psd/graph.py
@@ -55,6 +55,7 @@
         dev = coords.device
         self.module, self.per_row = module, per_row
         self.graph, self._graphs = None, []
+        self._images = []
         self.n_cap = max(_round_up(headroom * coords.shape[0], granule), _round_up(min_rows, granule))
         self.coords = torch.zeros((self.n_cap, coords.shape[1]), dtype=coords.dtype, device=dev)
         self.feats = torch.zeros((self.n_cap, feats.shape[1]), dtype=feats.dtype, device=dev)
@@ -72,6 +73,51 @@
         self.events = None
         return net
 
+    def _make_filter_images(self, backward):
+        from ..spconv.conv import SparseConvolution
+        self._images = []
+        if not ops.FILTER_IMAGES or self.feats.dtype not in (torch.bfloat16, torch.float16):
+            return
+        lib = _lib.load()
+        for m in self.module.modules():
+            if (isinstance(m, SparseConvolution) and m.in_channels == 32 and m.out_channels == 32 and not m.conv1x1
+                    and not m.inverse and m.weight.is_cuda and m.weight.dtype == torch.float32
+                    and m.weight.is_contiguous() and len(self._images) < _lib.FILTER_IMAGE_JOBS_MAX):
+                K = m.weight.numel() // 1024
+                if K > 27:
+                    continue
+                nbytes = int(lib.wfs_filter_image_bytes(K))
+                fwd = torch.zeros((nbytes,), dtype=torch.uint8, device=m.weight.device)
+                t = torch.zeros_like(fwd) if backward else None
+                self._images.append((m, K, (self.feats.dtype, fwd, t)))
+
+    def _filter_image_jobs(self):
+        code = _lib.dtype_code(self.feats)
+        jobs = (_lib.FilterImageJob * max(1, len(self._images)))()
+        for job, (m, K, (_dt, fwd, t)) in zip(jobs, self._images):
+            w = m.weight
+            if not (w.is_cuda and w.dtype == torch.float32 and w.is_contiguous() and w.numel() == K * 1024):
+                raise RuntimeError("a conv weight changed its layout under a captured step (filter images)")
+            job.W, job.img_fwd, job.img_t, job.K, job.dtype = w.data_ptr(), _lib.ptr(fwd), _lib.ptr(t), K, code
+        return jobs
+
+    def _refresh_filter_images(self):
+        if not self._images:
+            return
+        lib = _lib.load()
+        for job in self._filter_image_jobs()[:len(self._images)]:
+            _lib.check(lib.wfs_conv_filter_images(job.W, job.K, job.dtype, job.img_fwd, job.img_t, _lib.stream_ptr()))
+
+    @contextlib.contextmanager
+    def _filter_images_live(self):
+        for m, _K, imgs in self._images:
+            m.filter_images = imgs
+        try:
+            yield
+        finally:
+            for m, _K, _imgs in self._images:
+                m.filter_images = None
+
     def _own_stream(self, dev):
         if torch.cuda.current_stream(dev) == torch.cuda.default_stream(dev):
             st = torch.cuda.Stream(dev)
@@ -148,6 +194,7 @@
             if self.indices is not None:
                 self.indices[:n].copy_(coords[:, self._perm], non_blocking=True)
             self._event_offsets()
+            self._refresh_filter_images()
             return
         if (coords.is_cuda and coords.dtype == torch.int32 and coords.is_contiguous() and feats.is_cuda
                 and feats.is_contiguous() and feats.dtype == self.feats.dtype and labels.is_cuda
@@ -155,11 +202,14 @@
             lib = _lib.load()
             perm = _lib.i32_array(self._perm) if self._perm is not None else None
             ev = self.events if (self.events is not None and perm is not None) else None
-            _lib.check(lib.wfs_load_batch(_lib.ptr(coords), n, coords.shape[1], perm, _lib.ptr(self.coords),
-                                          _lib.ptr(self.indices), _lib.ptr(feats), _lib.ptr(self.feats),
-                                          feats.numel() * feats.element_size(), _lib.ptr(labels), _lib.ptr(self.labels),
-                                          labels.numel(), _lib.ptr(self.n_valid), _lib.ptr(ev), self.n_events,
-                                          _lib.stream_ptr()))
+            args = (_lib.ptr(coords), n, coords.shape[1], perm, _lib.ptr(self.coords), _lib.ptr(self.indices),
+                    _lib.ptr(feats), _lib.ptr(self.feats), feats.numel() * feats.element_size(), _lib.ptr(labels),
+                    _lib.ptr(self.labels), labels.numel(), _lib.ptr(self.n_valid), _lib.ptr(ev), self.n_events)
+            if self._images:
+                _lib.check(lib.wfs_load_batch_images(*args, self._filter_image_jobs(), len(self._images),
+                                                     _lib.stream_ptr()))
+            else:
+                _lib.check(lib.wfs_load_batch(*args, _lib.stream_ptr()))
             if ev is None:
                 self._event_offsets()
             return
@@ -170,6 +220,7 @@
         if self.indices is not None:
             self.indices[:n].copy_(coords[:, self._perm], non_blocking=True)
         self._event_offsets()
+        self._refresh_filter_images()
 
     def _event_offsets(self):
         if self.events is None:
@@ -222,6 +273,7 @@
             reducer.remove()
         if self.indices is not None:
             net.batch_first_indices = (self.coords, self.indices)
+        self._make_filter_images(backward=True)
         self._load(example_batch)
         failed, err = 0, None
         try:
@@ -244,6 +296,7 @@
 
     def _warm_and_capture(self, warmup):
         for _ in range(warmup):
+            self._refresh_filter_images()
             self._body()
             if not self.in_graph_optimizer:
                 self._after()
@@ -260,6 +313,10 @@
         return ([self.coords, self.feats, self.n_valid], self.labels)
 
     def _body(self):
+        with self._filter_images_live():
+            return self._step_body()
+
+    def _step_body(self):
         self.reducer.reset()
         from ..spconv import functional as Fsp
         loss = self.module.training_step(self._static_batch(), 0)
@@ -452,6 +509,7 @@
                 self._calibrate(headroom, 1.0, granule)
                 if self.indices is not None:
                     net.batch_first_indices = (self.coords, self.indices)
+                self._make_filter_images(backward=False)
                 self._load(example_batch)
                 if sweep:
                     self._reuse = ops.reuse_rulebooks()
@@ -472,7 +530,8 @@
         net = self.module.model
         if hasattr(net, "batch_size_hint"):
             net.batch_size_hint = self.n_events
-        return net([self.coords, self.feats, self.n_valid]).float()
+        with self._filter_images_live():
+            return net([self.coords, self.feats, self.n_valid]).float()
 
     def __call__(self, batch, occlude_index=None):
         self._load(batch)
diff --git a/waveformml_amd/spconv/conv.py b/waveformml_amd/spconv/conv.py
--- a/waveformml_amd/spconv/conv.py
+++ b/waveformml_amd/spconv/conv.py
@@ -41,6 +41,7 @@
             self.bias = nn.Parameter(torch.Tensor(out_channels))
         else:
             self.register_parameter('bias', None)
+        self.filter_images = None
         self.reset_parameters()
 
     def calibration_count(self):
@@ -120,10 +121,10 @@
                 out_features = features
                 out_unique = input.unique if self.subm else True
             elif self.subm:
-                out_features = Fsp.indice_subm_conv(features, self.weight, self.bias, rb)
+                out_features = Fsp.indice_subm_conv(features, self.weight, self.bias, rb, getattr(self, "filter_images", None))
                 out_unique = input.unique
             else:
-                out_features = Fsp.indice_conv(features, self.weight, self.bias, rb)
+                out_features = Fsp.indice_conv(features, self.weight, self.bias, rb, getattr(self, "filter_images", None))
                 out_unique = True
             out_n_valid = rb.m_dev
         out_tensor = SparseConvTensor(out_features, out_indices, out_spatial_shape, batch_size)
diff --git a/waveformml_amd/spconv/functional.py b/waveformml_amd/spconv/functional.py
--- a/waveformml_amd/spconv/functional.py
+++ b/waveformml_amd/spconv/functional.py
@@ -84,15 +84,15 @@
     return Y
 
 
-def gather_conv(table, kmap, K, identity_k, R, X, W, transpose_w, bias, r_dev=None, w16=None, packed_kl=0):
+def gather_conv(table, kmap, K, identity_k, R, X, W, transpose_w, bias, r_dev=None, w16=None, packed_kl=0, image=None):
     lib = _lib.load()
     Cw_in, Cw_out = int(W.shape[-2]), int(W.shape[-1])
     if packed_kl:
         assert transpose_w and kmap is None and table.shape == (K // packed_kl, R), (table.shape, K, packed_kl, R)
         Y = _rows((R, Cw_in), X, r_dev)
-        _lib.check(lib.wfs_gather_conv(_lib.ptr(table), None, K, identity_k, R, _lib.ptr(X), X.shape[0], X.shape[1],
-                                       _lib.ptr(W), Cw_in, Cw_out, 1, None, _lib.ptr(Y), _lib.dtype_code(X),
-                                       _lib.ptr(r_dev), packed_kl, _lib.stream_ptr()))
+        _lib.check(lib.wfs_gather_conv_image(_lib.ptr(table), None, K, identity_k, R, _lib.ptr(X), X.shape[0], X.shape[1],
+                                             _lib.ptr(W), Cw_in, Cw_out, 1, None, _lib.ptr(Y), _lib.dtype_code(X),
+                                             _lib.ptr(r_dev), packed_kl, _lib.ptr(image), _lib.stream_ptr()))
         if ACCOUNT is not None:
             _account("gather_conv", (table >> 3).clamp_(min=-1), R, X.shape[0], X.shape[1], R, Cw_in, K, Cw_in, Cw_out,
                      X.element_size())
@@ -108,9 +108,10 @@
     assert X.dim() == 2 and X.shape[1] == (Cw_out if transpose_w else Cw_in), (X.shape, W.shape, transpose_w)
     assert table is None or (table.dtype == torch.int32 and table.shape == (K, R)), (None if table is None else table.shape, K, R)
     assert bias is None or (bias.dtype == torch.float32 and bias.numel() == Cy)
-    _lib.check(lib.wfs_gather_conv(_lib.ptr(table), kmap, K, identity_k, R, _lib.ptr(X), X.shape[0], X.shape[1],
-                                   _lib.ptr(W), Cw_in, Cw_out, 1 if transpose_w else 0, _lib.ptr(bias),
-                                   _lib.ptr(Y), _lib.dtype_code(X), _lib.ptr(r_dev), 0, _lib.stream_ptr()))
+    _lib.check(lib.wfs_gather_conv_image(_lib.ptr(table), kmap, K, identity_k, R, _lib.ptr(X), X.shape[0], X.shape[1],
+                                         _lib.ptr(W), Cw_in, Cw_out, 1 if transpose_w else 0, _lib.ptr(bias),
+                                         _lib.ptr(Y), _lib.dtype_code(X), _lib.ptr(r_dev), 0, _lib.ptr(image),
+                                         _lib.stream_ptr()))
     _account("gather_conv", table, R, X.shape[0], X.shape[1], R, Cy, K, Cw_in, Cw_out, X.element_size())
     return Y
 
@@ -234,7 +235,7 @@
     return dW
 
 
-def conv_backward(table, K, identity_k, R, X, dY, W, r_dev=None, like=None, packed_kl=0):
+def conv_backward(table, K, identity_k, R, X, dY, W, r_dev=None, like=None, packed_kl=0, image_t=None):
     lib = _lib.load()
     Cin, Cout = int(X.shape[1]), int(dY.shape[1])
     if like is not None and like.numel() == K * Cin * Cout:
@@ -244,9 +245,10 @@
     dX = _rows((R, Cin), dY, r_dev)
     ws = torch.empty((max(int(lib.wfs_gather_dw_workspace_bytes(K, R, Cin, Cout)), 1),), dtype=torch.uint8, device=X.device)
     job = _dw_job(dW)
-    _lib.check(lib.wfs_conv_backward(_lib.ptr(table), K, identity_k, R, _lib.ptr(X), _lib.ptr(dY), dY.shape[0], Cin, Cout,
-                                     _lib.ptr(W), _lib.ptr(dX), _lib.ptr(dW), _lib.dtype_code(X), _lib.ptr(ws), ws.numel(),
-                                     _lib.ptr(r_dev), job, packed_kl, _lib.stream_ptr()))
+    _lib.check(lib.wfs_conv_backward_image(_lib.ptr(table), K, identity_k, R, _lib.ptr(X), _lib.ptr(dY), dY.shape[0], Cin,
+                                           Cout, _lib.ptr(W), _lib.ptr(dX), _lib.ptr(dW), _lib.dtype_code(X), _lib.ptr(ws),
+                                           ws.numel(), _lib.ptr(r_dev), job, packed_kl, _lib.ptr(image_t),
+                                           _lib.stream_ptr()))
     _queue_dw_job(job, ws)
     if ACCOUNT is not None:
         dense = (table >> 3).clamp_(min=-1) if packed_kl else table
@@ -273,7 +275,7 @@
 class SparseConvFunction(Function):
 
     @staticmethod
-    def forward(ctx, features, filters, bias, rulebook, mode):
+    def forward(ctx, features, filters, bias, rulebook, mode, images=None):
         rb = rulebook
         features = _features_ok(features)
         K = rb.K
@@ -281,6 +283,11 @@
         b = None if bias is None else bias.detach().float().contiguous()
         ident = rb.centre_k if rb.subm else -1
         w16 = None
+        img_fwd = img_t = None
+        if (images is not None and mode != INVERSE and images[0] == features.dtype and tuple(W.shape) == (K, 32, 32)
+                and W.data_ptr() == filters.data_ptr() and K <= 27):
+            img_fwd, img_t = images[1], images[2]
+        ctx.img_t = img_t
         if mode == INVERSE:
             assert features.shape[0] == rb.M, "inverse conv input must be the coupled conv's output set"
             w16 = filters16(W, features) if takes_wide_path(K, rb.N, features, W.shape[2]) else None
@@ -291,7 +298,7 @@
             assert features.shape[0] == rb.N
             table, kmap = rb.table_by_out()
             w16 = filters16(W, features) if takes_wide_path(K, rb.M, features, W.shape[2]) else None
-            out = gather_conv(table, kmap, K, ident, rb.M, features, W, False, b, rb.m_dev, w16)
+            out = gather_conv(table, kmap, K, ident, rb.M, features, W, False, b, rb.m_dev, w16, image=img_fwd)
         ctx.save_for_backward(features, filters, bias)
         ctx.rb, ctx.mode = rb, mode
         ctx.w16 = w16 if ctx.needs_input_grad[0] else None
@@ -319,7 +326,7 @@
             table, pk = rb.table_by_in(32, 32, features, 3)
             if pk and rb.table_by_in(32, 32, dY, 1)[1] != pk:
                 table, pk = rb.nbr_out, 0
-            dX, dW = conv_backward(table, K, ident, rb.N, features, dY, W, rb.n_dev, filters, pk)
+            dX, dW = conv_backward(table, K, ident, rb.N, features, dY, W, rb.n_dev, filters, pk, ctx.img_t)
         else:
             if ctx.needs_input_grad[1]:
                 if features.shape[1] == 2 and dY.shape[1] == 32 and K <= 27 and not rb.has_dup:
@@ -330,12 +337,13 @@
                     dW = gather_dw(table, K, ident, rb.N, features, dY, False, None, rb.n_dev, filters, pk)
             if ctx.needs_input_grad[0]:
                 table, pk = rb.table_by_in(dY.shape[1], W.shape[1], dY, 1)
-                dX = gather_conv(table, None, K, ident, rb.N, dY, W, True, None, rb.n_dev, ctx.w16, pk)
+                dX = gather_conv(table, None, K, ident, rb.N, dY, W, True, None, rb.n_dev, ctx.w16, pk,
+                                 image=ctx.img_t if dY.dtype == features.dtype else None)
         if dW is not None:
             dW = dW.reshape(filters.shape).to(filters.dtype)
         if bias is not None and ctx.needs_input_grad[2]:
             db = _masked_column_sum(dY, rb.n_dev if mode == INVERSE else rb.m_dev).to(bias.dtype)
-        return dX, dW, db, None, None
+        return dX, dW, db, None, None, None
 
 
 def maxpool_fwd(table, kmap, K, R, X, r_dev=None):
@@ -960,12 +968,12 @@
     return CrossEntropyMeanFunction.apply(logits, target, ignore_index)
 
 
-def indice_conv(features, filters, bias, rulebook):
-    return SparseConvFunction.apply(features, filters, bias, rulebook, CONV)
-
-
-def indice_subm_conv(features, filters, bias, rulebook):
-    return SparseConvFunction.apply(features, filters, bias, rulebook, SUBM)
+def indice_conv(features, filters, bias, rulebook, images=None):
+    return SparseConvFunction.apply(features, filters, bias, rulebook, CONV, images)
+
+
+def indice_subm_conv(features, filters, bias, rulebook, images=None):
+    return SparseConvFunction.apply(features, filters, bias, rulebook, SUBM, images)
 
 
 def indice_inverse_conv(features, filters, bias, rulebook):
diff --git a/waveformml_amd/spconv/ops.py b/waveformml_amd/spconv/ops.py
--- a/waveformml_amd/spconv/ops.py
+++ b/waveformml_amd/spconv/ops.py
@@ -18,6 +18,8 @@
 
 EVENT_LOCAL_CONV = os.environ.get("WFS_EVENT_LOCAL_CONV", "1") != "0"
 PACKED_TABLES = os.environ.get("WFS_PACKED_TABLES", "1") != "0"
+
+FILTER_IMAGES = os.environ.get("WFS_FILTER_IMAGES", "1") != "0"
 
 _SIDE_STREAMS = {}
 
```

New measurement: 577,400 events/s (median of 6 runs). +2.6%, better.
